# boqian-li/GarmentDreamer

Hardware: AMD Instinct MI355X
Metric: SDS iters/sec (rasterize+UNet+bwd), 100k Gaussians ×8 views @512², 1/2/4/8 GPU (higher is better)
Workload: dtype bf16

## Files before the change

### garmentdreamer_amd/csrc/nn_elementwise.hip

```cpp
#include <hip/hip_runtime.h>
#include <stdint.h>
#include <stdio.h>

#include "../../include/gd_nn.h"
#include "nn_device.h"
#include "nn_host.h"
#include "nn_math.h"

namespace {

using namespace gdnn;


__device__ __forceinline__ float wave_sum(float v)
{
#pragma unroll
    for (int off = 32; off > 0; off >>= 1) v += __shfl_xor(v, off, 64);
    return v;
}

__global__ __launch_bounds__(256) void geglu_kernel(const bf16x8* __restrict__ x, bf16x8* __restrict__ y, int64_t nvec,
                                                    int vin )
{
    for (int64_t i = (int64_t)blockIdx.x * blockDim.x + threadIdx.x; i < nvec; i += (int64_t)gridDim.x * blockDim.x) {
        const int64_t row = i / vin;
        const int c = (int)(i - row * vin);
        const u32x4 h = __builtin_bit_cast(u32x4, x[row * 2 * vin + c]);
        const u32x4 g = __builtin_bit_cast(u32x4, x[row * 2 * vin + vin + c]);
        u32x4 o;
#pragma unroll
        for (int k = 0; k < 4; k++) o.w[k] = gdnn::geglu2(h.w[k], g.w[k]);
        y[i] = __builtin_bit_cast(bf16x8, o);
    }
}

template <int VPL>
__global__ __launch_bounds__(256) void add_layernorm_kernel(const bf16x8* __restrict__ x, const bf16x8* __restrict__ r,
                                                            const bf16x8* __restrict__ w, const bf16x8* __restrict__ b,
                                                            bf16x8* __restrict__ s_out, bf16x8* __restrict__ y,
                                                            int64_t rows, int vpr , float eps)
{
    const int lane = threadIdx.x & 63;
    const int64_t row = (int64_t)blockIdx.x * (blockDim.x >> 6) + (threadIdx.x >> 6);
    if (row >= rows) return;
    const bf16x8* xr = x + row * vpr;
    f2 v[VPL][4];
    f2 sum2 = {0.f, 0.f};
#pragma unroll
    for (int i = 0; i < VPL; i++) {
        const int c = lane + 64 * i;
        if (c < vpr) {
            const u32x4 a = __builtin_bit_cast(u32x4, xr[c]);
            if (r) {
                const u32x4 rr = __builtin_bit_cast(u32x4, r[row * vpr + c]);
                u32x4 so;
#pragma unroll
                for (int k = 0; k < 4; k++) {
                    so.w[k] = pack2(unpack2(a.w[k]) + unpack2(rr.w[k]));
                    v[i][k] = unpack2(so.w[k]);
                }
                if (s_out) s_out[row * vpr + c] = __builtin_bit_cast(bf16x8, so);
            } else {
#pragma unroll
                for (int k = 0; k < 4; k++) v[i][k] = unpack2(a.w[k]);
            }
#pragma unroll
            for (int k = 0; k < 4; k++) sum2 += v[i][k];
        } else {
#pragma unroll
            for (int k = 0; k < 4; k++) v[i][k] = f2{0.f, 0.f};
        }
    }
    const float inv_c = 1.0f / (float)(vpr * 8);
    const float mean = wave_sum(sum2.x + sum2.y) * inv_c;
    f2 sq2 = {0.f, 0.f};
#pragma unroll
    for (int i = 0; i < VPL; i++) {
        if (lane + 64 * i < vpr) {
#pragma unroll
            for (int k = 0; k < 4; k++) {
                const f2 d = v[i][k] - mean;
                sq2 += d * d;
            }
        }
    }
    const float rstd = rsqrtf(wave_sum(sq2.x + sq2.y) * inv_c + eps);
#pragma unroll
    for (int i = 0; i < VPL; i++) {
        const int c = lane + 64 * i;
        if (c < vpr) {
            const u32x4 ww = __builtin_bit_cast(u32x4, w[c]), bb = __builtin_bit_cast(u32x4, b[c]);
            u32x4 o;
#pragma unroll
            for (int k = 0; k < 4; k++) o.w[k] = pack2(((v[i][k] - mean) * rstd) * unpack2(ww.w[k]) + unpack2(bb.w[k]));
            y[row * vpr + c] = __builtin_bit_cast(bf16x8, o);
        }
    }
}

__global__ __launch_bounds__(256) void geglu_backward_kernel(const bf16x8* __restrict__ x, const bf16x8* __restrict__ dy,
                                                             bf16x8* __restrict__ dx, int64_t nvec, int vin)
{
    for (int64_t i = (int64_t)blockIdx.x * blockDim.x + threadIdx.x; i < nvec; i += (int64_t)gridDim.x * blockDim.x) {
        const int64_t row = i / vin;
        const int c = (int)(i - row * vin);
        const u32x4 h = __builtin_bit_cast(u32x4, x[row * 2 * vin + c]);
        const u32x4 g = __builtin_bit_cast(u32x4, x[row * 2 * vin + vin + c]);
        const u32x4 d = __builtin_bit_cast(u32x4, dy[i]);
        u32x4 oh, og;
#pragma unroll
        for (int k = 0; k < 4; k++) {
            const f2 gv = unpack2(g.w[k]), hv = unpack2(h.w[k]), dv = unpack2(d.w[k]);
            const f2 cdf = 0.5f * (1.0f + erf_as2(gv * 0.70710678118654752f));
            const f2 a = (gv * gv) * -0.72134752044448170f;
            const f2 pdf = 0.39894228040143268f * f2{__builtin_amdgcn_exp2f(a.x), __builtin_amdgcn_exp2f(a.y)};
            oh.w[k] = pack2(dv * (gv * cdf));
            og.w[k] = pack2((dv * hv) * (cdf + gv * pdf));
        }
        dx[row * 2 * vin + c] = __builtin_bit_cast(bf16x8, oh);
        dx[row * 2 * vin + vin + c] = __builtin_bit_cast(bf16x8, og);
    }
}

template <int VPL>
__global__ __launch_bounds__(256) void layernorm_backward_kernel(const bf16x8* __restrict__ s, const bf16x8* __restrict__ dy,
                                                                 const bf16x8* __restrict__ w, const bf16x8* __restrict__ ds,
                                                                 bf16x8* __restrict__ dx, int64_t rows, int vpr, float eps)
{
    const int lane = threadIdx.x & 63;
    const int64_t row = (int64_t)blockIdx.x * (blockDim.x >> 6) + (threadIdx.x >> 6);
    if (row >= rows) return;
    f2 v[VPL][4], a[VPL][4];
    f2 sum2 = {0.f, 0.f};
#pragma unroll
    for (int i = 0; i < VPL; i++) {
        const int c = lane + 64 * i;
        if (c < vpr) {
            const u32x4 q = __builtin_bit_cast(u32x4, s[row * vpr + c]);
#pragma unroll
            for (int k = 0; k < 4; k++) { v[i][k] = unpack2(q.w[k]); sum2 += v[i][k]; }
        } else {
#pragma unroll
            for (int k = 0; k < 4; k++) v[i][k] = f2{0.f, 0.f};
        }
    }
    const float inv_c = 1.0f / (float)(vpr * 8);
    const float mean = wave_sum(sum2.x + sum2.y) * inv_c;
    f2 sq2 = {0.f, 0.f};
#pragma unroll
    for (int i = 0; i < VPL; i++)
        if (lane + 64 * i < vpr) {
#pragma unroll
            for (int k = 0; k < 4; k++) { const f2 d = v[i][k] - mean; sq2 += d * d; }
        }
    const float rstd = rsqrtf(wave_sum(sq2.x + sq2.y) * inv_c + eps);
    f2 m1 = {0.f, 0.f}, m2 = {0.f, 0.f};
#pragma unroll
    for (int i = 0; i < VPL; i++) {
        const int c = lane + 64 * i;
        if (c < vpr) {
            const u32x4 g = __builtin_bit_cast(u32x4, dy[row * vpr + c]), ww = __builtin_bit_cast(u32x4, w[c]);
#pragma unroll
            for (int k = 0; k < 4; k++) {
                v[i][k] = (v[i][k] - mean) * rstd;
                a[i][k] = unpack2(g.w[k]) * unpack2(ww.w[k]);
                m1 += a[i][k];
                m2 += a[i][k] * v[i][k];
            }
        } else {
#pragma unroll
            for (int k = 0; k < 4; k++) a[i][k] = f2{0.f, 0.f};
        }
    }
    const float ma = wave_sum(m1.x + m1.y) * inv_c, mb = wave_sum(m2.x + m2.y) * inv_c;
#pragma unroll
    for (int i = 0; i < VPL; i++) {
        const int c = lane + 64 * i;
        if (c < vpr) {
            u32x4 o;
            u32x4 e = {{0u, 0u, 0u, 0u}};
            if (ds) e = __builtin_bit_cast(u32x4, ds[row * vpr + c]);
#pragma unroll
            for (int k = 0; k < 4; k++) o.w[k] = pack2((a[i][k] - ma - v[i][k] * mb) * rstd + unpack2(e.w[k]));
            dx[row * vpr + c] = __builtin_bit_cast(bf16x8, o);
        }
    }
}

template <int R>
__global__ __launch_bounds__(256) void softmax_rows_kernel(const u32x4* x, u32x4* y, int64_t rows, int L8)
{
    const int lane = threadIdx.x & 63;
    const int64_t row = (int64_t)blockIdx.x * 4 + (threadIdx.x >> 6);
    if (row >= rows) return;
    const u32x4* xr = x + row * L8;
    u32x4 v[R];
    float m = -INFINITY;
#pragma unroll
    for (int i = 0; i < R; i++) {
        const int c = lane + 64 * i;
        if (c < L8) {
            v[i] = xr[c];
#pragma unroll
            for (int e = 0; e < 4; e++) { const f2 f = unpack2(v[i].w[e]); m = fmaxf(m, fmaxf(f.x, f.y)); }
        }
    }
#pragma unroll
    for (int off = 32; off > 0; off >>= 1) m = fmaxf(m, __shfl_xor(m, off, 64));
    const float k = 1.4426950408889634f;
    const float mk = m == -INFINITY ? 0.f : m * k;
    float sum = 0.f;
    f2 ex[R][4];
#pragma unroll
    for (int i = 0; i < R; i++) {
        if (lane + 64 * i < L8) {
#pragma unroll
            for (int e = 0; e < 4; e++) {
                const f2 f = unpack2(v[i].w[e]);
                ex[i][e] = f2{__builtin_amdgcn_exp2f(f.x * k - mk), __builtin_amdgcn_exp2f(f.y * k - mk)};
                sum += ex[i][e].x + ex[i][e].y;
            }
        }
    }
    sum = wave_sum(sum);
    const float inv = 1.f / sum;
    u32x4* yr = y + row * L8;
#pragma unroll
    for (int i = 0; i < R; i++) {
        const int c = lane + 64 * i;
        if (c < L8) {
            u32x4 o;
#pragma unroll
            for (int e = 0; e < 4; e++) o.w[e] = pack2(ex[i][e] * inv);
            yr[c] = o;
        }
    }
}

template <int R>
__global__ __launch_bounds__(256) void softmax_rows_backward_kernel(const u32x4* __restrict__ p, const u32x4* dp,
                                                                    u32x4* ds, int64_t rows, int L8)
{
    const int lane = threadIdx.x & 63;
    const int64_t row = (int64_t)blockIdx.x * 4 + (threadIdx.x >> 6);
    if (row >= rows) return;
    const u32x4* pr = p + row * L8;
    const u32x4* gr = dp + row * L8;
    u32x4 vp[R], vg[R];
    f2 acc = f2{0.f, 0.f};
#pragma unroll
    for (int i = 0; i < R; i++) {
        const int c = lane + 64 * i;
        if (c < L8) {
            vp[i] = pr[c];
            vg[i] = gr[c];
        }
    }
#pragma unroll
    for (int i = 0; i < R; i++) {
        if (lane + 64 * i < L8) {
#pragma unroll
            for (int e = 0; e < 4; e++) acc += unpack2(vp[i].w[e]) * unpack2(vg[i].w[e]);
        }
    }
    const float s = wave_sum(acc.x + acc.y);
    u32x4* or_ = ds + row * L8;
#pragma unroll
    for (int i = 0; i < R; i++) {
        const int c = lane + 64 * i;
        if (c < L8) {
            u32x4 o;
#pragma unroll
            for (int e = 0; e < 4; e++) o.w[e] = pack2(unpack2(vp[i].w[e]) * (unpack2(vg[i].w[e]) - s));
            or_[c] = o;
        }
    }
}

template <bool TRANSPOSED>
__global__ __launch_bounds__(256) void conv1x1_c8_kernel(const u32x4* __restrict__ x, const uint16_t* __restrict__ w,
                                                         const uint16_t* __restrict__ bias, u32x4* __restrict__ y, int64_t npix)
{
    float wf[8][8], bf[8];
#pragma unroll
    for (int o = 0; o < 8; o++) {
        bf[o] = (!TRANSPOSED && bias) ? bf2f(bias[o]) : 0.f;
#pragma unroll
        for (int i = 0; i < 8; i++) wf[o][i] = bf2f(TRANSPOSED ? w[i * 8 + o] : w[o * 8 + i]);
    }
    for (int64_t p = (int64_t)blockIdx.x * blockDim.x + threadIdx.x; p < npix; p += (int64_t)gridDim.x * blockDim.x) {
        const u32x4 q = x[p];
        float v[8], o[8];
#pragma unroll
        for (int e = 0; e < 4; e++) { v[2 * e] = __uint_as_float(q.w[e] << 16); v[2 * e + 1] = __uint_as_float(q.w[e] & 0xffff0000u); }
#pragma unroll
        for (int c = 0; c < 8; c++) {
            float a = bf[c];
#pragma unroll
            for (int i = 0; i < 8; i++) a = fmaf(wf[c][i], v[i], a);
            o[c] = a;
        }
        u32x4 out;
#pragma unroll
        for (int e = 0; e < 4; e++) out.w[e] = pack2(f2{o[2 * e], o[2 * e + 1]});
        y[p] = out;
    }
}

}

extern "C" {

const char* gd_nn_elementwise_last_error(void) { return g_err; }

int gd_nn_geglu_forward(void* stream, const void* x, void* y, int64_t rows, int inner)
{
    if (!x || !y) return fail(GD_NN_ERR_INVALID_ARG, "geglu: null pointer");
    if (rows <= 0 || inner <= 0 || inner % 8) return fail(GD_NN_ERR_INVALID_ARG, "geglu: need inner % 8 == 0");
    const int64_t nvec = rows * (inner / 8);
    const int64_t blocks = (nvec + 255) / 256;
    const int grid = (int)(blocks < 16384 ? blocks : 16384);
    hipLaunchKernelGGL(geglu_kernel, dim3(grid), dim3(256), 0, (hipStream_t)stream, (const bf16x8*)x, (bf16x8*)y, nvec,
                       inner / 8);
    return launch_status("geglu: launch failed");
}

int gd_nn_add_layernorm_forward(void* stream, const void* x, const void* residual, const void* weight, const void* bias,
                                float eps, void* sum_out, void* y, int64_t rows, int C)
{
    if (!x || !weight || !bias || !y) return fail(GD_NN_ERR_INVALID_ARG, "add_layernorm: null pointer");
    if (rows <= 0 || C <= 0 || C % 8 || C > 64 * 8 * 4)
        return fail(GD_NN_ERR_INVALID_ARG, "add_layernorm: need C % 8 == 0 and C <= 2048");
    if (sum_out && !residual) return fail(GD_NN_ERR_INVALID_ARG, "add_layernorm: sum_out without residual");
    const int vpr = C / 8;
    const int vpl = (vpr + 63) / 64;
    const int64_t blocks = (rows + 3) / 4;
    if (blocks > 2147483647LL) return fail(GD_NN_ERR_INVALID_ARG, "add_layernorm: too many rows");
#define GD_LN(V_)                                                                                                      \
    hipLaunchKernelGGL(add_layernorm_kernel<V_>, dim3((unsigned)blocks), dim3(256), 0, (hipStream_t)stream,            \
                       (const bf16x8*)x, (const bf16x8*)residual, (const bf16x8*)weight, (const bf16x8*)bias,          \
                       (bf16x8*)sum_out, (bf16x8*)y, rows, vpr, eps)
    if (vpl == 1) GD_LN(1);
    else if (vpl == 2) GD_LN(2);
    else if (vpl == 3) GD_LN(3);
    else GD_LN(4);
#undef GD_LN
    return launch_status("add_layernorm: launch failed");
}

int gd_nn_geglu_backward(void* stream, const void* x, const void* dy, void* dx, int64_t rows, int inner)
{
    if (!x || !dy || !dx) return fail(GD_NN_ERR_INVALID_ARG, "geglu_backward: null pointer");
    if (rows <= 0 || inner <= 0 || inner % 8) return fail(GD_NN_ERR_INVALID_ARG, "geglu_backward: need inner % 8 == 0");
    const int64_t nvec = rows * (inner / 8);
    const int64_t blocks = (nvec + 255) / 256;
    const int grid = (int)(blocks < 16384 ? blocks : 16384);
    hipLaunchKernelGGL(geglu_backward_kernel, dim3(grid), dim3(256), 0, (hipStream_t)stream, (const bf16x8*)x, (const bf16x8*)dy,
                       (bf16x8*)dx, nvec, inner / 8);
    return launch_status("geglu_backward: launch failed");
}

int gd_nn_layernorm_backward(void* stream, const void* s, const void* dy, const void* weight, const void* ds, void* dx,
                             int64_t rows, int C, float eps)
{
    if (!s || !dy || !weight || !dx) return fail(GD_NN_ERR_INVALID_ARG, "layernorm_backward: null pointer");
    if (rows <= 0 || C <= 0 || C % 8 || C > 2048) return fail(GD_NN_ERR_INVALID_ARG, "layernorm_backward: need C % 8 == 0, C <= 2048");
    const int vpr = C / 8, vpl = (vpr + 63) / 64;
    const int64_t blocks = (rows + 3) / 4;
    if (blocks > 2147483647LL) return fail(GD_NN_ERR_INVALID_ARG, "layernorm_backward: too many rows");
#define GD_LNB(V_)                                                                                                     \
    hipLaunchKernelGGL(layernorm_backward_kernel<V_>, dim3((unsigned)blocks), dim3(256), 0, (hipStream_t)stream,       \
                       (const bf16x8*)s, (const bf16x8*)dy, (const bf16x8*)weight, (const bf16x8*)ds, (bf16x8*)dx, rows, vpr, eps)
    if (vpl == 1) GD_LNB(1);
    else if (vpl == 2) GD_LNB(2);
    else if (vpl == 3) GD_LNB(3);
    else GD_LNB(4);
#undef GD_LNB
    return launch_status("layernorm_backward: launch failed");
}

int gd_nn_conv1x1_c8(void* stream, const void* x, const void* weight, const void* bias, void* y, int64_t npix, int transposed)
{
    if (!x || !weight || !y) return fail(GD_NN_ERR_INVALID_ARG, "conv1x1_c8: null pointer");
    if (npix <= 0) return fail(GD_NN_ERR_INVALID_ARG, "conv1x1_c8: need npix > 0");
    const int64_t blocks = (npix + 255) / 256;
    const int grid = (int)(blocks < 16384 ? blocks : 16384);
    if (transposed)
        hipLaunchKernelGGL(conv1x1_c8_kernel<true>, dim3(grid), dim3(256), 0, (hipStream_t)stream, (const u32x4*)x,
                           (const uint16_t*)weight, (const uint16_t*)nullptr, (u32x4*)y, npix);
    else
        hipLaunchKernelGGL(conv1x1_c8_kernel<false>, dim3(grid), dim3(256), 0, (hipStream_t)stream, (const u32x4*)x,
                           (const uint16_t*)weight, (const uint16_t*)bias, (u32x4*)y, npix);
    return launch_status("conv1x1_c8: launch failed");
}

int gd_nn_softmax_rows_forward(void* stream, const void* x, void* y, int64_t rows, int L)
{
    if (!x || !y) return fail(GD_NN_ERR_INVALID_ARG, "softmax_rows: null pointer");
    if (rows <= 0 || L <= 0 || L % 8 || L > 8192) return fail(GD_NN_ERR_INVALID_ARG, "softmax_rows: need rows > 0, L % 8 == 0, L <= 8192");
    const int64_t blocks = (rows + 3) / 4;
    if (blocks > 2147483647LL) return fail(GD_NN_ERR_INVALID_ARG, "softmax_rows: too many rows");
    const int L8 = L / 8, R = (L8 + 63) / 64;
#define GD_SM(R_) hipLaunchKernelGGL(softmax_rows_kernel<R_>, dim3((unsigned)blocks), dim3(256), 0, (hipStream_t)stream, (const u32x4*)x, (u32x4*)y, rows, L8)
    if (R <= 2) GD_SM(2);
    else if (R <= 4) GD_SM(4);
    else if (R <= 8) GD_SM(8);
    else GD_SM(16);
#undef GD_SM
    return launch_status("softmax_rows: launch failed");
}

int gd_nn_softmax_rows_backward(void* stream, const void* p, const void* dp, void* ds, int64_t rows, int L)
{
    if (!p || !dp || !ds) return fail(GD_NN_ERR_INVALID_ARG, "softmax_rows_backward: null pointer");
    if (rows <= 0 || L <= 0 || L % 8 || L > 8192) return fail(GD_NN_ERR_INVALID_ARG, "softmax_rows_backward: need rows > 0, L % 8 == 0, L <= 8192");
    const int64_t blocks = (rows + 3) / 4;
    if (blocks > 2147483647LL) return fail(GD_NN_ERR_INVALID_ARG, "softmax_rows_backward: too many rows");
    const int L8 = L / 8, R = (L8 + 63) / 64;
#define GD_SMB(R_) hipLaunchKernelGGL(softmax_rows_backward_kernel<R_>, dim3((unsigned)blocks), dim3(256), 0, (hipStream_t)stream, (const u32x4*)p, (const u32x4*)dp, (u32x4*)ds, rows, L8)
    if (R <= 2) GD_SMB(2);
    else if (R <= 4) GD_SMB(4);
    else if (R <= 8) GD_SMB(8);
    else GD_SMB(16);
#undef GD_SMB
    return launch_status("softmax_rows_backward: launch failed");
}

}
```

### garmentdreamer_amd/guidance/sd21.py

```python
from __future__ import annotations

import math
from typing import Optional

import torch
import torch.nn as nn
import torch.nn.functional as F

from ..nn_ops import (add_layer_norm, attention_d64, attention_d64_supported, attention_d64_vt, conv1x1, conv3x3, conv3x3_s2, conv3x3_s2_supported, conv3x3_small_cin,
                      conv3x3_supported, geglu, gn_conv3x3, gn_conv3x3_supported, gn_conv_prefers_fused, group_norm_silu,
                      resnet_block_frozen, resnet_block_frozen_supported, upsample2x_conv3x3,
                      upsample2x_conv3x3_supported, linear_320, route_rows, route_scale,
                      linear_320_geglu, linear_320_supported, gemm_geglu, gemm_supported)


import os as _os

_FUSED_QKV = _os.environ.get("GD_FUSED_QKV", "1") != "0"
_VT_GEMM = _os.environ.get("GD_VT_GEMM", "1") != "0"
_LORA_FUSED = _os.environ.get("GD_LORA_FUSED", "1") != "0"
_VAE_ATTN_NODE = _os.environ.get("GD_VAE_ATTN_NODE", "1") != "0"
_CTX_VT = _os.environ.get("GD_CTX_VT", "1") != "0"
_LORA_LINEAR = _os.environ.get("GD_LORA_LINEAR", "1") != "0"
_CONV_BIAS_GRAD = _os.environ.get("GD_CONV_BIAS_GRAD", "1") != "0"
_PINNED_TABLES = _os.environ.get("GD_PAGEABLE_COPIES", "0") != "1"
_TEMB_TRAIN_CAT = _os.environ.get("GD_TEMB_TRAIN_CAT", "1") != "0"
from .. import nn_ops
_FP8_ACTIVE = [None]


def _gn(norm: nn.GroupNorm, x, silu: bool):
    return group_norm_silu(x, norm.weight, norm.bias, norm.num_groups, norm.eps, silu)


def _conv3(conv: nn.Conv2d, x, image_bias=None, residual=None):
    bias = conv.bias if image_bias is None else image_bias
    frozen = not conv.weight.requires_grad and (conv.bias is None or not conv.bias.requires_grad)
    if frozen and conv3x3_supported(x, conv.weight) and conv.stride == (1, 1) and conv.padding == (1, 1):
        if bias is not None and bias.requires_grad and not _CONV_BIAS_GRAD:
            y = conv3x3(x, conv.weight, None, None) + (bias[:, :, None, None] if bias.dim() == 2 else bias[None, :, None, None])
            return y if residual is None else y + residual
        return conv3x3(x, conv.weight, bias, residual)
    nn_ops._note_fallback("sd21._conv3", x, "needs frozen bf16 channels_last weights, stride 1, pad 1, Cin % 64 == 0")
    y = F.conv2d(x, conv.weight, None if image_bias is not None else conv.bias, conv.stride, conv.padding)
    if image_bias is not None:
        y = y + image_bias[:, :, None, None]
    return y if residual is None else y + residual


import os as _os0
_LIN320 = _os0.environ.get("GD_LINEAR320", "1") != "0"
_OWN_GEMM = _os0.environ.get("GD_OWN_GEMM", "1") != "0"
_OWN_GEMM_MIN_ROWS = 1024


def _lib_linear(x, w, b=None):
    if route_scale() > 1 and x.is_cuda:
        padded, take = route_rows(x.reshape(-1, x.shape[-1]))
        return take(F.linear(padded, w, b)).reshape(*x.shape[:-1], w.shape[0])
    return F.linear(x, w, b)


def _lib_addmm(c, a, w_t):
    if route_scale() > 1 and a.is_cuda:
        pa, take = route_rows(a)
        pc, _ = route_rows(c)
        return take(torch.addmm(pc, pa, w_t))
    return torch.addmm(c, a, w_t)


def _lin(mod: nn.Linear, x, bias=None):
    w = mod.weight
    b = mod.bias if bias is None else bias
    if _LIN320 and x.is_cuda and not torch.is_grad_enabled() and not w.requires_grad and w.shape[1] == 320 and \
            linear_320_supported(x, w, b):
        return linear_320(x, w, b)
    return _lib_linear(x, w, b)


def _gn_conv3(norm: nn.GroupNorm, conv: nn.Conv2d, x, image_bias=None, residual=None):
    frozen = not conv.weight.requires_grad and (conv.bias is None or not conv.bias.requires_grad)
    frozen = frozen and (image_bias is None or not image_bias.requires_grad)
    st = _FP8_ACTIVE[0]
    if st is not None and frozen and not torch.is_grad_enabled() and st.wants(conv, x):
        bias = conv.bias if image_bias is None else image_bias
        if st.mode == "run" and id(conv) in st.amax:
            return st.gn_conv(norm, conv, x, bias, residual)
        act = _gn(norm, x, True)
        if st.mode == "calibrate":
            st.observe(conv, act)
        return _conv3(conv, act, image_bias=image_bias, residual=residual)
    if x.is_cuda and frozen and gn_conv_prefers_fused(x, conv.out_channels) and \
            gn_conv3x3_supported(x, norm.weight, conv.weight):
        return gn_conv3x3(x, norm.weight, norm.bias, norm.num_groups, norm.eps, True, conv.weight,
                          conv.bias if image_bias is None else image_bias, residual)
    return _conv3(conv, _gn(norm, x, True), image_bias=image_bias, residual=residual)




class TembProjections:

    __slots__ = ("temb", "image_bias")

    def __init__(self, temb, image_bias):
        self.temb, self.image_bias = temb, image_bias


class ContextProjections:

    __slots__ = ("context", "kv", "vt")

    def __init__(self, context, kv, vt=None):
        self.context, self.kv, self.vt = context, kv, (vt or {})

    @property
    def shape(self):
        return self.context.shape


class ResnetBlock2D(nn.Module):
    def __init__(self, in_ch: int, out_ch: int, temb_ch: Optional[int], eps: float = 1e-5, groups: int = 32):
        super().__init__()
        self.norm1 = nn.GroupNorm(groups, in_ch, eps=eps)
        self.conv1 = nn.Conv2d(in_ch, out_ch, 3, padding=1)
        self.time_emb_proj = nn.Linear(temb_ch, out_ch) if temb_ch is not None else None
        self.norm2 = nn.GroupNorm(groups, out_ch, eps=eps)
        self.conv2 = nn.Conv2d(out_ch, out_ch, 3, padding=1)
        self.conv_shortcut = nn.Conv2d(in_ch, out_ch, 1) if in_ch != out_ch else None

    def forward(self, x, temb=None, next_norm=None):
        if resnet_block_frozen_supported(x, self):
            return resnet_block_frozen(x, self, next_norm)
        image_bias = None
        if isinstance(temb, TembProjections):
            image_bias = temb.image_bias.get(id(self))
            temb = temb.temb
        if image_bias is None and self.time_emb_proj is not None:
            image_bias = self.time_emb_proj(F.silu(temb)) + self.conv1.bias
        h = _gn_conv3(self.norm1, self.conv1, x, image_bias=image_bias)
        if self.conv_shortcut is not None:
            x = conv1x1(x, self.conv_shortcut.weight, self.conv_shortcut.bias)
        return _gn_conv3(self.norm2, self.conv2, h, residual=x)


class LoRALinearLayer(nn.Module):

    def __init__(self, in_features: int, out_features: int, rank: int = 4):
        super().__init__()
        self.down = nn.Linear(in_features, rank, bias=False)
        self.up = nn.Linear(rank, out_features, bias=False)
        nn.init.normal_(self.down.weight, std=1 / rank)
        nn.init.zeros_(self.up.weight)

    def forward(self, x):
        return self.up(self.down(x.to(self.down.weight.dtype))).to(x.dtype)


class Attention(nn.Module):

    def __init__(self, query_dim: int, heads: int, dim_head: int, cross_dim: Optional[int] = None,
                 qkv_bias: bool = False):
        super().__init__()
        inner = heads * dim_head
        self.heads = heads
        self.to_q = nn.Linear(query_dim, inner, bias=qkv_bias)
        self.to_k = nn.Linear(cross_dim or query_dim, inner, bias=qkv_bias)
        self.to_v = nn.Linear(cross_dim or query_dim, inner, bias=qkv_bias)
        self.to_out = nn.ModuleList([nn.Linear(inner, query_dim)])
        self.lora = None
        self.lora_scale = 1.0

    def add_lora(self, rank: int = 4):
        q_in, kv_in, inner = self.to_q.in_features, self.to_k.in_features, self.to_q.out_features
        self.lora = nn.ModuleDict({
            "to_q_lora": LoRALinearLayer(q_in, inner, rank), "to_k_lora": LoRALinearLayer(kv_in, inner, rank),
            "to_v_lora": LoRALinearLayer(kv_in, inner, rank),
            "to_out_lora": LoRALinearLayer(inner, self.to_out[0].out_features, rank)})
        return self.lora

    def forward(self, x, context=None):
        B, N, _ = x.shape
        kv = context_vt = None
        if isinstance(context, ContextProjections):
            kv = context.kv.get(id(self)) if self.lora is None else None
            context_vt = context.vt
            context = context.context
        ctx = x if context is None else context
        if kv is not None:
            q, (k, v) = _lin(self.to_q, x), kv
            vt = context_vt.get(id(self)) if context_vt is not None else None
            if vt is not None and N >= 256 and _CTX_VT and q.shape[-1] == 64 * self.heads and not torch.is_grad_enabled():
                q4, k4 = q.view(B, N, self.heads, 64), k.view(B, k.shape[1], self.heads, 64)
                if nn_ops._attention_d64_layout_ok(q4, k4, k4):
                    return _lin(self.to_out[0], nn_ops.attention_d64_vt_strided(q4, k4, vt, k.shape[1]))
        elif _FUSED_QKV and context is None and self.lora is None and x.is_cuda and self.to_q.bias is None and \
                not self.to_q.weight.requires_grad and not torch.is_grad_enabled():
            src = (self.to_q.weight.data_ptr(), self.to_q.weight._version, self.to_k.weight._version,
                   self.to_v.weight._version, x.dtype)
            if getattr(self, "_wqkv_src", None) != src:
                self._wqk = torch.cat([self.to_q.weight, self.to_k.weight], dim=0).detach().contiguous()
                self._wqkv_src = src
            q, k = (linear_320(x, self._wqk) if _LIN320 and linear_320_supported(x, self._wqk)
                    else _lib_linear(x, self._wqk)).chunk(2, dim=-1)
            q = q.view(B, N, self.heads, -1)
            k = k.view(B, N, self.heads, -1)
            if _VT_GEMM and N % 64 == 0 and N >= 256 and q.shape[-1] == 64 and x.dtype == torch.bfloat16:
                vt = torch.matmul(self.to_v.weight.detach(), x.transpose(1, 2))
                return _lin(self.to_out[0], attention_d64_vt(q, k, vt))
            v = _lin(self.to_v, x)
            q, k = q.reshape(B, N, -1), k.reshape(B, N, -1)
        elif self.lora is not None:
            q = self._lora_lin(self.to_q, x, "to_q_lora")
            k = self._lora_lin(self.to_k, ctx, "to_k_lora")
            v = self._lora_lin(self.to_v, ctx, "to_v_lora")
        else:
            q, k, v = _lin(self.to_q, x), _lin(self.to_k, ctx), _lin(self.to_v, ctx)
        q = q.view(B, N, self.heads, -1)
        k = k.view(B, ctx.shape[1], self.heads, -1)
        v = v.view(B, ctx.shape[1], self.heads, -1)
        if N >= 256 and q.shape[-1] == 64 and nn_ops.attention_d64_train_supported(q, k, v):
            o = nn_ops.attention_d64_train(q, k, v)
        elif N >= 256 and q.shape[-1] == 64 and attention_d64_supported(q, k, v):
            o = attention_d64(q, k, v)
        else:
            o = F.scaled_dot_product_attention(q.transpose(1, 2), k.transpose(1, 2), v.transpose(1, 2))
            o = o.transpose(1, 2).reshape(B, N, -1)
        if self.lora is not None:
            return self._lora_lin(self.to_out[0], o, "to_out_lora")
        return _lin(self.to_out[0], o)

    def _lora_lin(self, mod: nn.Linear, x, name):
        layer = self.lora[name]
        dw, uw = layer.down.weight, layer.up.weight
        w, b = mod.weight, mod.bias
        if _LORA_FUSED and _LORA_LINEAR and x.is_cuda and x.dtype == torch.bfloat16 and w.dtype == torch.bfloat16 and \
                not w.requires_grad and (b is None or not b.requires_grad) and dw.dtype == torch.float32 and \
                uw.dtype == torch.float32 and dw.shape[0] == 4 and uw.shape[1] == 4 and x.shape[-1] % 8 == 0 and \
                w.shape[0] % 8 == 0 and dw.is_contiguous() and uw.is_contiguous():
            return nn_ops.lora_linear(x, w, dw, uw, self.lora_scale, lambda t: _lin(mod, t))
        return self._lora_add(_lin(mod, x), x, name)

    def _lora_add(self, base, x, name):
        layer = self.lora[name]
        dw, uw = layer.down.weight, layer.up.weight
        if _LORA_FUSED and nn_ops.lora_branch_supported(x, base, dw, uw):
            return nn_ops.lora_branch(x, base, dw, uw, self.lora_scale)
        return base + self.lora_scale * layer(x)


class GEGLU(nn.Module):
    def __init__(self, dim_in: int, dim_out: int):
        super().__init__()
        self.proj = nn.Linear(dim_in, dim_out * 2)

    def forward(self, x):
        w = self.proj.weight
        if _LIN320 and x.is_cuda and not torch.is_grad_enabled() and not w.requires_grad and tuple(w.shape) == (2560, 320) and \
                linear_320_supported(x, w, self.proj.bias):
            return linear_320_geglu(x, w, self.proj.bias)
        if _OWN_GEMM and x.is_cuda and not torch.is_grad_enabled() and not w.requires_grad and w.shape[1] != 320 and \
                (x.numel() // x.shape[-1]) * route_scale() >= _OWN_GEMM_MIN_ROWS and gemm_supported(x, w, self.proj.bias, geglu=True):
            return gemm_geglu(x, w, self.proj.bias)
        return geglu(_lin(self.proj, x))


class FeedForward(nn.Module):
    def __init__(self, dim: int, mult: int = 4):
        super().__init__()
        self.net = nn.ModuleList([GEGLU(dim, dim * mult), nn.Identity(), nn.Linear(dim * mult, dim)])

    def forward(self, x):
        return _lin(self.net[2], self.net[0](x))


class BasicTransformerBlock(nn.Module):
    def __init__(self, dim: int, heads: int, dim_head: int, cross_dim: int):
        super().__init__()
        self.norm1 = nn.LayerNorm(dim)
        self.attn1 = Attention(dim, heads, dim_head)
        self.norm2 = nn.LayerNorm(dim)
        self.attn2 = Attention(dim, heads, dim_head, cross_dim=cross_dim)
        self.norm3 = nn.LayerNorm(dim)
        self.ff = FeedForward(dim)

    def forward(self, x, context, defer_ff_bias: bool = False):
        _, n = add_layer_norm(x, None, self.norm1)
        x, n = add_layer_norm(x, self.attn1(n), self.norm2)
        x, n = add_layer_norm(x, self.attn2(n, context), self.norm3)
        if defer_ff_bias:
            g = self.ff.net[0](n)
            return _lib_addmm(x.reshape(-1, x.shape[-1]), g.reshape(-1, g.shape[-1]), self.ff.net[2].weight.t()).view_as(x)
        return x + self.ff(n)


class Transformer2DModel(nn.Module):
    def __init__(self, channels: int, heads: int, dim_head: int, cross_dim: int, groups: int = 32):
        super().__init__()
        self.norm = nn.GroupNorm(groups, channels, eps=1e-6)
        self.proj_in = nn.Linear(channels, channels)
        self.transformer_blocks = nn.ModuleList([BasicTransformerBlock(channels, heads, dim_head, cross_dim)])
        self.proj_out = nn.Linear(channels, channels)

    def _folded_out_bias(self, dtype):
        w, b2 = self.proj_out.weight, self.transformer_blocks[0].ff.net[2].bias
        key = (w.data_ptr(), w._version, b2._version, self.proj_out.bias._version, dtype)
        if getattr(self, "_fold_key", None) != key:
            with torch.no_grad():
                self._fold_bias = (self.proj_out.bias.float() + w.float() @ b2.float()).to(dtype)
            self._fold_key = key
        return self._fold_bias

    def forward(self, x, context):
        B, C, H, W = x.shape
        h = _gn(self.norm, x, False)
        h = h.permute(0, 2, 3, 1).reshape(B, H * W, C)
        h = _lin(self.proj_in, h)
        if len(self.transformer_blocks) == 1 and h.is_cuda and not torch.is_grad_enabled() and \
                not self.proj_out.weight.requires_grad:
            h = self.transformer_blocks[0](h, context, defer_ff_bias=True)
            h = _lin(self.proj_out, h, self._folded_out_bias(h.dtype))
        else:
            for blk in self.transformer_blocks:
                h = blk(h, context)
            h = self.proj_out(h)
        h = h.reshape(B, H, W, C).permute(0, 3, 1, 2)
        return h + x


class Downsample2D(nn.Module):
    def __init__(self, ch: int, padding: int = 1):
        super().__init__()
        self.padding = padding
        self.conv = nn.Conv2d(ch, ch, 3, stride=2, padding=padding)

    def forward(self, x):
        if conv3x3_s2_supported(x, self.conv.weight):
            return conv3x3_s2(x, self.conv.weight, self.conv.bias, self.padding)
        nn_ops._note_fallback("sd21.Downsample2D", x, "needs frozen bf16 weights with Cin % 64 == 0 and Cout % 64 == 0")
        if self.padding == 0:
            x = F.pad(x, (0, 1, 0, 1))
        return self.conv(x)


class Upsample2D(nn.Module):
    def __init__(self, ch: int):
        super().__init__()
        self.conv = nn.Conv2d(ch, ch, 3, padding=1)

    def forward(self, x):
        if upsample2x_conv3x3_supported(x, self.conv.weight) and not self.conv.bias.requires_grad:
            return upsample2x_conv3x3(x, self.conv.weight, self.conv.bias)
        return _conv3(self.conv, F.interpolate(x, scale_factor=2.0, mode="nearest"))


class _DownBlock(nn.Module):
    def __init__(self, in_ch, out_ch, temb_ch, n_layers, heads, cross_dim, attn: bool, down: bool):
        super().__init__()
        self.resnets = nn.ModuleList(
            [ResnetBlock2D(in_ch if i == 0 else out_ch, out_ch, temb_ch) for i in range(n_layers)])
        self.attentions = nn.ModuleList(
            [Transformer2DModel(out_ch, heads, out_ch // heads, cross_dim) for _ in range(n_layers)]) if attn else None
        self.downsamplers = nn.ModuleList([Downsample2D(out_ch)]) if down else None

    def forward(self, x, temb, context, skips):
        for i, res in enumerate(self.resnets):
            x = res(x, temb)
            if self.attentions is not None:
                x = self.attentions[i](x, context)
            skips.append(x)
        if self.downsamplers is not None:
            x = self.downsamplers[0](x)
            skips.append(x)
        return x


class _UpBlock(nn.Module):
    def __init__(self, in_ch, prev_ch, out_ch, temb_ch, n_layers, heads, cross_dim, attn: bool, up: bool):
        super().__init__()
        res = []
        for i in range(n_layers):
            skip_ch = in_ch if i == n_layers - 1 else out_ch
            res_in = prev_ch if i == 0 else out_ch
            res.append(ResnetBlock2D(res_in + skip_ch, out_ch, temb_ch))
        self.resnets = nn.ModuleList(res)
        self.attentions = nn.ModuleList(
            [Transformer2DModel(out_ch, heads, out_ch // heads, cross_dim) for _ in range(n_layers)]) if attn else None
        self.upsamplers = nn.ModuleList([Upsample2D(out_ch)]) if up else None

    def forward(self, x, temb, context, skips):
        for i, res in enumerate(self.resnets):
            x = torch.cat([x, skips.pop()], dim=1)
            x = res(x, temb)
            if self.attentions is not None:
                x = self.attentions[i](x, context)
        if self.upsamplers is not None:
            x = self.upsamplers[0](x)
        return x


class _MidBlockCrossAttn(nn.Module):
    def __init__(self, ch, temb_ch, heads, cross_dim):
        super().__init__()
        self.resnets = nn.ModuleList([ResnetBlock2D(ch, ch, temb_ch), ResnetBlock2D(ch, ch, temb_ch)])
        self.attentions = nn.ModuleList([Transformer2DModel(ch, heads, ch // heads, cross_dim)])

    def forward(self, x, temb, context):
        x = self.resnets[0](x, temb)
        x = self.attentions[0](x, context)
        return self.resnets[1](x, temb)


class TimestepEmbedding(nn.Module):
    def __init__(self, in_ch, out_ch):
        super().__init__()
        self.linear_1 = nn.Linear(in_ch, out_ch)
        self.linear_2 = nn.Linear(out_ch, out_ch)

    def forward(self, x):
        return _lin(self.linear_2, F.silu(_lin(self.linear_1, x)))


def sinusoidal_timestep_embedding(t: torch.Tensor, dim: int) -> torch.Tensor:
    half = dim // 2
    exponent = -math.log(10000.0) * torch.arange(half, dtype=torch.float32, device=t.device) / half
    emb = t.float()[:, None] * torch.exp(exponent)[None, :]
    return torch.cat([torch.cos(emb), torch.sin(emb)], dim=-1)


class UNet2DConditionModel(nn.Module):

    def __init__(self, in_channels=4, out_channels=4, block_out_channels=(320, 640, 1280, 1280), layers_per_block=2,
                 cross_attention_dim=1024, attention_head_dim=(5, 10, 20, 20)):
        super().__init__()
        ch = block_out_channels
        temb_ch = ch[0] * 4
        self.block_out_channels = tuple(ch)
        self.conv_in = nn.Conv2d(in_channels, ch[0], 3, padding=1)
        self.time_embedding = TimestepEmbedding(ch[0], temb_ch)
        self.down_blocks = nn.ModuleList()
        out = ch[0]
        for i, c in enumerate(ch):
            inp, out = out, c
            last = i == len(ch) - 1
            self.down_blocks.append(_DownBlock(inp, out, temb_ch, layers_per_block, attention_head_dim[i],
                                               cross_attention_dim, attn=not last, down=not last))
        self.mid_block = _MidBlockCrossAttn(ch[-1], temb_ch, attention_head_dim[-1], cross_attention_dim)
        self.up_blocks = nn.ModuleList()
        rev = list(reversed(ch))
        rev_heads = list(reversed(attention_head_dim))
        out = rev[0]
        for i, c in enumerate(rev):
            prev, out = out, c
            inp = rev[min(i + 1, len(ch) - 1)]
            last = i == len(ch) - 1
            self.up_blocks.append(_UpBlock(inp, prev, out, temb_ch, layers_per_block + 1, rev_heads[i],
                                           cross_attention_dim, attn=i != 0, up=not last))
        self.conv_norm_out = nn.GroupNorm(32, ch[0], eps=1e-5)
        self.conv_out = nn.Conv2d(ch[0], out_channels, 3, padding=1)

    def extra_embedding(self, batch: int, **kwargs):
        return None

    def _project_context(self, ctx):
        if not ctx.is_cuda or torch.is_grad_enabled():
            return ctx
        atts = [m.attn2 for m in self.modules() if isinstance(m, BasicTransformerBlock)]
        if not atts or any(a.to_k.weight.requires_grad or a.to_k.bias is not None or a.lora is not None for a in atts):
            return ctx
        first = atts[0].to_k.weight
        key = (first.data_ptr(), ctx.dtype, len(atts)) + tuple(t._version for a in atts for t in (a.to_k.weight, a.to_v.weight))
        cache = getattr(self, "_ctx_cat", None)
        if cache is None or cache[0] != key:
            with torch.no_grad():
                w = torch.cat([t for a in atts for t in (a.to_k.weight, a.to_v.weight)], dim=0).to(ctx.dtype).contiguous()
                wv = torch.cat([a.to_v.weight for a in atts], dim=0).to(ctx.dtype).contiguous()
            cache = self._ctx_cat = (key, w, wv)
        with torch.no_grad():
            allp = _lib_linear(ctx, cache[1])
            vt_all = None
            if _CTX_VT and ctx.dtype == torch.bfloat16 and all(a.to_v.out_features == 64 * a.heads for a in atts):
                T = ctx.shape[1]
                Tp = (T + 63) // 64 * 64
                ctx_p = F.pad(ctx, (0, 0, 0, Tp - T)) if Tp != T else ctx
                vt_all = torch.matmul(cache[2], ctx_p.transpose(1, 2))
        kv, vt, off, voff = {}, {}, 0, 0
        for a in atts:
            c = a.to_k.out_features
            kv[id(a)] = (allp[..., off:off + c], allp[..., off + c:off + 2 * c])
            if vt_all is not None:
                vt[id(a)] = vt_all[:, voff:voff + c]
            off += 2 * c
            voff += c
        return ContextProjections(ctx, kv, vt)

    def _project_temb(self, temb):
        train = torch.is_grad_enabled() and temb.requires_grad
        if not temb.is_cuda or (train and not _TEMB_TRAIN_CAT):
            return temb
        blocks = [m for m in self.modules() if isinstance(m, ResnetBlock2D) and m.time_emb_proj is not None]
        if not blocks or any(b.time_emb_proj.weight.requires_grad or b.conv1.bias.requires_grad for b in blocks):
            return temb
        first = blocks[0].time_emb_proj.weight
        key = (first.data_ptr(), temb.dtype, len(blocks)) + tuple(
            t._version for b in blocks for t in (b.time_emb_proj.weight, b.time_emb_proj.bias, b.conv1.bias))
        cache = getattr(self, "_temb_cat", None)
        if cache is None or cache[0] != key:
            with torch.no_grad():
                w = torch.cat([b.time_emb_proj.weight for b in blocks], dim=0).to(temb.dtype).contiguous()
                bias = torch.cat([b.time_emb_proj.bias + b.conv1.bias for b in blocks], dim=0).to(temb.dtype)
            cache = self._temb_cat = (key, w, bias)
        if train:
            parts = torch.split(_lib_linear(F.silu(temb), cache[1], cache[2]), [b.time_emb_proj.out_features for b in blocks], dim=1)
            return TembProjections(temb, {id(b): p for b, p in zip(blocks, parts)})
        with torch.no_grad():
            allp = _lib_linear(F.silu(temb), cache[1], cache[2])
        out, off = {}, 0
        for b in blocks:
            c = b.time_emb_proj.out_features
            out[id(b)] = allp[:, off:off + c]
            off += c
        return TembProjections(temb, out)

    fp8 = None

    def enable_fp8(self, state=None):
        from ..nn_ops import Fp8State
        self.fp8 = state if state is not None else Fp8State()
        return self.fp8

    def forward(self, sample, timestep, encoder_hidden_states, **kwargs):
        if self.fp8 is not None and not torch.is_grad_enabled() and sample.is_cuda:
            _FP8_ACTIVE[0] = self.fp8
            try:
                return self._forward(sample, timestep, encoder_hidden_states, **kwargs)
            finally:
                _FP8_ACTIVE[0] = None
        return self._forward(sample, timestep, encoder_hidden_states, **kwargs)

    def _forward(self, sample, timestep, encoder_hidden_states, **kwargs):
        dtype = self.conv_in.weight.dtype
        if timestep.dim() == 0:
            timestep = timestep[None].expand(sample.shape[0])
        temb = self.time_embedding(sinusoidal_timestep_embedding(timestep, self.block_out_channels[0]).to(dtype))
        extra = self.extra_embedding(sample.shape[0], **kwargs)
        if extra is not None:
            temb = temb + extra.to(dtype)
        temb = self._project_temb(temb)
        x = conv3x3_small_cin(sample.to(dtype).contiguous(memory_format=torch.channels_last), self.conv_in.weight,
                              self.conv_in.bias)
        ctx = self._project_context(encoder_hidden_states.to(dtype))
        skips = [x]
        for blk in self.down_blocks:
            x = blk(x, temb, ctx, skips)
        x = self.mid_block(x, temb, ctx)
        for blk in self.up_blocks:
            x = blk(x, temb, ctx, skips)
        return _conv3(self.conv_out, _gn(self.conv_norm_out, x, True))


class LoraUNet2DConditionModel(UNet2DConditionModel):

    def __init__(self, rank: int = 4, **kw):
        super().__init__(**kw)
        temb_ch = self.block_out_channels[0] * 4
        self.camera_emb = nn.Sequential(nn.Linear(16, temb_ch), nn.SiLU(), nn.Linear(temb_ch, temb_ch))
        self.lambertian_emb = nn.Parameter(torch.randn(1, temb_ch))
        self.textureless_emb = nn.Parameter(torch.randn(1, temb_ch))
        self.normal_emb = nn.Parameter(torch.randn(1, temb_ch))
        self.lora_layers = nn.ModuleList()
        for m in self.modules():
            if isinstance(m, Attention):
                self.lora_layers.append(m.add_lora(rank))

    def adapters_to_fp32(self):
        self.lora_layers.float()
        return self

    def trainables_to_fp32(self):
        self.adapters_to_fp32()
        self.camera_emb.float()
        for p in (self.lambertian_emb, self.textureless_emb, self.normal_emb):
            p.data = p.data.float()
        return self

    def freeze_base(self):
        for p in self.parameters():
            p.requires_grad_(False)
        train = list(self.lora_layers.parameters()) + list(self.camera_emb.parameters()) + \
            [self.lambertian_emb, self.textureless_emb, self.normal_emb]
        for p in train:
            p.requires_grad_(True)
        return train

    def forward(self, sample, timestep, encoder_hidden_states, **kwargs):
        if torch.is_grad_enabled() and sample.is_cuda:
            with nn_ops.lora_grad_group():
                return super().forward(sample, timestep, encoder_hidden_states, **kwargs)
        return super().forward(sample, timestep, encoder_hidden_states, **kwargs)

    def extra_embedding(self, batch: int, c=None, shading: str = "albedo"):
        dev, dt = self.camera_emb[0].weight.device, self.camera_emb[0].weight.dtype
        if c is None:
            c = torch.zeros(batch, 16, device=dev)
        emb = self.camera_emb(c.to(device=dev, dtype=dt))
        if shading == "textureless":
            emb = emb + self.textureless_emb
        elif shading == "lambertian":
            emb = emb + self.lambertian_emb
        elif shading == "normal":
            emb = emb + self.normal_emb
        else:
            assert shading == "albedo"
        return emb




class _VAEAttention(nn.Module):

    def __init__(self, ch: int):
        super().__init__()
        self.group_norm = nn.GroupNorm(32, ch, eps=1e-6)
        self.to_q = nn.Linear(ch, ch)
        self.to_k = nn.Linear(ch, ch)
        self.to_v = nn.Linear(ch, ch)
        self.to_out = nn.ModuleList([nn.Linear(ch, ch)])

    def _qkv_scaled(self, dtype, scale):
        ws = (self.to_q.weight, self.to_k.weight, self.to_v.weight, self.to_q.bias, self.to_k.bias, self.to_v.bias)
        key = (ws[0].data_ptr(), dtype) + tuple(t._version for t in ws)
        if getattr(self, "_qkv_key", None) != key:
            with torch.no_grad():
                w = torch.cat([ws[0].float() * scale, ws[1].float(), ws[2].float()], dim=0).to(dtype).contiguous()
                b = torch.cat([ws[3].float() * scale, ws[4].float(), ws[5].float()], dim=0).to(dtype)
            self._qkv_cache, self._qkv_key = (w, b), key
        return self._qkv_cache

    def forward(self, x):
        B, C, H, W = x.shape
        h = _gn(self.group_norm, x, False).permute(0, 2, 3, 1).reshape(B, H * W, C)
        if x.is_cuda:
            o = None
            if _FUSED_QKV and not (self.to_q.weight.requires_grad or self.to_k.weight.requires_grad or self.to_v.weight.requires_grad):
                qkv = _lib_linear(h, *self._qkv_scaled(h.dtype, C ** -0.5))
                if _VAE_ATTN_NODE and nn_ops.single_head_attention_supported(qkv):
                    o = nn_ops.single_head_attention(qkv)
                else:
                    q, k, v = qkv.chunk(3, dim=-1)
            else:
                q, k, v = _lin(self.to_q, h) * (C ** -0.5), _lin(self.to_k, h), _lin(self.to_v, h)
            if o is None:
                p = torch.softmax(torch.bmm(q, k.transpose(1, 2)), dim=-1)
                o = torch.bmm(p, v)
        else:
            q, k, v = self.to_q(h), self.to_k(h), self.to_v(h)
            o = F.scaled_dot_product_attention(q[:, None], k[:, None], v[:, None])[:, 0]
        o = _lin(self.to_out[0], o).reshape(B, H, W, C).permute(0, 3, 1, 2)
        return x + o


class _VAEDownBlock(nn.Module):
    def __init__(self, in_ch, out_ch, n_layers, down: bool):
        super().__init__()
        self.resnets = nn.ModuleList(
            [ResnetBlock2D(in_ch if i == 0 else out_ch, out_ch, None, eps=1e-6) for i in range(n_layers)])
        self.downsamplers = nn.ModuleList([Downsample2D(out_ch, padding=0)]) if down else None

    def forward(self, x, next_norm=None):
        for i, r in enumerate(self.resnets):
            last = i + 1 == len(self.resnets)
            x = r(x, next_norm=(next_norm if self.downsamplers is None else None) if last else self.resnets[i + 1].norm1)
        if self.downsamplers is not None:
            x = self.downsamplers[0](x)
        return x


class _VAEMidBlock(nn.Module):
    def __init__(self, ch):
        super().__init__()
        self.resnets = nn.ModuleList([ResnetBlock2D(ch, ch, None, eps=1e-6), ResnetBlock2D(ch, ch, None, eps=1e-6)])
        self.attentions = nn.ModuleList([_VAEAttention(ch)])

    def forward(self, x):
        return self.resnets[1](self.attentions[0](self.resnets[0](x)))


class Encoder(nn.Module):
    def __init__(self, in_channels=3, block_out_channels=(128, 256, 512, 512), layers_per_block=2, latent_channels=4):
        super().__init__()
        ch = block_out_channels
        self.conv_in = nn.Conv2d(in_channels, ch[0], 3, padding=1)
        self.down_blocks = nn.ModuleList()
        out = ch[0]
        for i, c in enumerate(ch):
            inp, out = out, c
            self.down_blocks.append(_VAEDownBlock(inp, out, layers_per_block, down=i != len(ch) - 1))
        self.mid_block = _VAEMidBlock(ch[-1])
        self.conv_norm_out = nn.GroupNorm(32, ch[-1], eps=1e-6)
        self.conv_out = nn.Conv2d(ch[-1], 2 * latent_channels, 3, padding=1)

    def forward(self, x):
        x = conv3x3_small_cin(x.contiguous(memory_format=torch.channels_last), self.conv_in.weight, self.conv_in.bias,
                              next_norm=self.down_blocks[0].resnets[0].norm1)
        for i, b in enumerate(self.down_blocks):
            x = b(x, next_norm=self.mid_block.resnets[0].norm1 if i + 1 == len(self.down_blocks) else None)
        x = self.mid_block(x)
        return _conv3(self.conv_out, _gn(self.conv_norm_out, x, True))


# ... 247 lines not shown
```

### garmentdreamer_amd/guidance/stable_diffusion_guidance.py

```python
from __future__ import annotations

from dataclasses import dataclass, field
from typing import Any, Optional

import torch
import torch.nn as nn
import torch.nn.functional as F

from .. import _runtime_env, nn_ops
from . import sd21


def C(value: Any, epoch: int, global_step: int) -> float:
    if isinstance(value, (int, float)):
        return value
    value = list(value)
    if len(value) == 3:
        value = [0] + value
    assert len(value) == 4
    start_step, start_value, end_value, end_step = value
    current = global_step if isinstance(end_step, int) else epoch
    return start_value + (end_value - start_value) * max(min(1.0, (current - start_step) / (end_step - start_step)), 0.0)


class StableDiffusionGuidance(nn.Module):
    @dataclass
    class Config:
        pretrained_model_name_or_path: str = "stabilityai/stable-diffusion-2-1-base"
        enable_memory_efficient_attention: bool = False
        enable_sequential_cpu_offload: bool = False
        enable_attention_slicing: bool = False
        enable_channels_last_format: bool = True
        guidance_scale: float = 100.0
        grad_clip: Optional[Any] = None
        half_precision_weights: bool = True
        min_step_percent: float = 0.02
        max_step_percent: float = 0.98
        max_step_percent_annealed: float = 0.5
        anneal_start_step: Optional[int] = None
        use_sjc: bool = False
        var_red: bool = True
        weighting_strategy: str = "sds"
        token_merging: bool = False
        token_merging_params: Optional[dict] = field(default_factory=dict)
        view_dependent_prompting: bool = True
        max_items_eval: int = 4
        unet_weights: Optional[str] = None
        vae_weights: Optional[str] = None
        init_seed: int = 0
        use_hip_graphs: bool = False
        fp8_unet: bool = False
        fp8_calibration_steps: int = 3

    def __init__(self, cfg: Optional[dict] = None, device="cuda", unet: Optional[nn.Module] = None,
                 vae: Optional[nn.Module] = None):
        super().__init__()
        cfg = cfg or {}
        self.cfg = cfg if isinstance(cfg, self.Config) else self.Config(**cfg)
        self.device = torch.device(device)
        self.configure(unet, vae)

    def configure(self, unet=None, vae=None) -> None:
        self.weights_dtype = torch.bfloat16 if self.cfg.half_precision_weights else torch.float32
        if unet is None:
            with torch.device(self.device):
                unet = sd21.UNet2DConditionModel()
            if self.cfg.unet_weights:
                sd21.load_diffusers_weights(unet, self.cfg.unet_weights)
            else:
                sd21.init_random_(unet, self.cfg.init_seed)
        self._vae_self_built = vae is None
        self._own_decoder = ()
        if vae is None:
            with torch.device(self.device):
                vae = sd21.AutoencoderKLEncoder()
            if self.cfg.vae_weights:
                sd21.load_diffusers_weights(vae, self.cfg.vae_weights)
            else:
                sd21.init_random_(vae, self.cfg.init_seed + 1)
        fmt = torch.channels_last if self.cfg.enable_channels_last_format else torch.contiguous_format
        self.unet = unet.to(device=self.device, dtype=self.weights_dtype).to(memory_format=fmt).eval()
        self.vae = vae.to(device=self.device, dtype=self.weights_dtype).to(memory_format=fmt).eval()
        for p in self.vae.parameters():
            p.requires_grad_(False)
        for p in self.unet.parameters():
            p.requires_grad_(False)
        self.scheduler = sd21.DDIMScheduler()
        self.num_train_timesteps = self.scheduler.config.num_train_timesteps
        self.set_min_max_steps()
        self.alphas = self.scheduler.alphas_cumprod.to(self.device)
        if self.cfg.use_sjc:
            self.us = torch.sqrt((1 - self.alphas) / self.alphas)
        self.grad_clip_val: Optional[float] = None
        self._unet_graphs = {}
        self._vae_graphs = {}
        self._fp8_calibrated = False
        self._fp8_calib_done = 0
        if self.cfg.fp8_unet and self.weights_dtype == torch.bfloat16 and self.device.type == "cuda":
            self.unet.enable_fp8()
        if self.cfg.use_hip_graphs and not _runtime_env.graph_replay_safe():
            import warnings
            warnings.warn(f"{_runtime_env.FLAG}=0 was not in place before the HIP runtime started; hipGraph replay of "
                          "the UNet / VAE is off for this process (eager launches). Import garmentdreamer_amd before "
                          "the first torch.cuda call, or export the flag.")
            self.cfg.use_hip_graphs = False

    def set_min_max_steps(self, min_step_percent=0.02, max_step_percent=0.98):
        self.min_step = int(self.num_train_timesteps * min_step_percent)
        self.max_step = int(self.num_train_timesteps * max_step_percent)

    def forward_unet(self, latents, t, encoder_hidden_states):
        input_dtype = latents.dtype
        t_dtype = torch.float32 if self.weights_dtype == torch.bfloat16 else self.weights_dtype
        x, tt, ctx = latents.to(self.weights_dtype), t.to(t_dtype), encoder_hidden_states.to(self.weights_dtype)
        fp8 = getattr(self.unet, "fp8", None)
        if fp8 is not None and not self._fp8_calibrated and not torch.is_grad_enabled():
            out = self.unet(x, tt, encoder_hidden_states=ctx).to(input_dtype)
            self._fp8_calib_done += 1
            if self._fp8_calib_done >= max(1, int(self.cfg.fp8_calibration_steps)):
                fp8.mode = "run"
                self._fp8_calibrated = True
            return out
        if self.cfg.use_hip_graphs and x.is_cuda and not torch.is_grad_enabled():
            try:
                return self._graphed_unet(x, tt, ctx).to(input_dtype)
            except RuntimeError as e:
                self._graphs_failed(e)
        return self.unet(x, tt, encoder_hidden_states=ctx).to(input_dtype)

    def may_capture(self, batch_size: int) -> bool:
        if not self.cfg.use_hip_graphs:
            return False
        have_u = any(k[0][0] in (2 * batch_size, 4 * batch_size) for k in self._unet_graphs)
        have_v = any(k[0] == batch_size for k in self._vae_graphs)
        return not (have_u and have_v)

    def _graphs_failed(self, err):
        import warnings
        warnings.warn(f"hipGraph capture failed ({err}); continuing with eager kernel launches")
        self.cfg.use_hip_graphs = False
        self._unet_graphs.clear()
        self._vae_graphs.clear()
        torch.cuda.synchronize()
        from .. import nn_ops
        nn_ops.reset_workspaces()

    def _graphed_unet(self, x, t, ctx):
        key = (tuple(x.shape), tuple(ctx.shape))
        entry = self._unet_graphs.get(key)
        if entry is None:
            sx, st, sc = x.clone(), t.clone(), ctx.clone()
            side = torch.cuda.Stream(device=x.device)
            side.wait_stream(torch.cuda.current_stream(x.device))
            with torch.cuda.stream(side), torch.no_grad():
                for _ in range(2):
                    self.unet(sx, st, encoder_hidden_states=sc)
            torch.cuda.current_stream(x.device).wait_stream(side)
            g = torch.cuda.CUDAGraph()
            with _runtime_env.capture_guard(), torch.cuda.graph(g), torch.no_grad():
                out = self.unet(sx, st, encoder_hidden_states=sc)
            entry = self._unet_graphs[key] = (g, sx, st, sc, out)
        g, sx, st, sc, out = entry
        sx.copy_(x)
        st.copy_(t)
        sc.copy_(ctx)
        g.replay()
        return out.clone()

    def _graphed_vae_moments(self, imgs):
        key = tuple(imgs.shape)
        fn = self._vae_graphs.get(key)
        if fn is None:
            vae = self.vae

            class _Moments(nn.Module):
                def forward(self, x):
                    return vae.quant_conv(vae.encoder(x))

            sample = torch.rand(imgs.shape, device=imgs.device, dtype=imgs.dtype, requires_grad=True)
            with _runtime_env.capture_guard():
                fn = self._vae_graphs[key] = torch.cuda.make_graphed_callables(_Moments(), (sample,))
        return fn(imgs)

    def encode_images(self, imgs, vae_noise: Optional[torch.Tensor] = None):
        return self._encode_prepared((imgs * 2.0 - 1.0).to(self.weights_dtype), vae_noise, imgs.dtype)

    def _encode_prepared(self, x, vae_noise, out_dtype):
        with nn_ops.route_batch(1, x.shape[0]):
            if self.cfg.use_hip_graphs and x.is_cuda and torch.is_grad_enabled() and x.requires_grad:
                xc = x.contiguous(memory_format=torch.channels_last)
                try:
                    posterior = sd21.DiagonalGaussianDistribution(self._graphed_vae_moments(xc))
                except RuntimeError as e:
                    self._graphs_failed(e)
                    posterior = self.vae.encode(x).latent_dist
            else:
                posterior = self.vae.encode(x).latent_dist
        noise = None if vae_noise is None else vae_noise.to(self.weights_dtype)
        latents = posterior.sample(noise) * self.vae.config.scaling_factor
        return latents.to(out_dtype)

    def compute_grad_sds(self, latents, t, prompt_utils, elevation, azimuth, camera_distances,
                         noise: Optional[torch.Tensor] = None):
        use_perp_neg = bool(getattr(prompt_utils, "use_perp_neg", False))
        batch_size = elevation.shape[0]
        neg_guidance_weights = None
        if use_perp_neg:
            text_embeddings, neg_guidance_weights = prompt_utils.get_text_embeddings_perp_neg(
                elevation, azimuth, camera_distances, self.cfg.view_dependent_prompting)
            with torch.no_grad():
                if noise is None:
                    noise = torch.randn_like(latents)
                latents_noisy = self.scheduler.add_noise(latents, noise, t)
                with nn_ops.route_batch(4, 4 * batch_size):
                    noise_pred = self.forward_unet(torch.cat([latents_noisy] * 4, dim=0), torch.cat([t] * 4),
                                                   encoder_hidden_states=text_embeddings)
            noise_pred_text = noise_pred[:batch_size]
            noise_pred_uncond = noise_pred[batch_size:batch_size * 2]
            noise_pred_neg = noise_pred[batch_size * 2:]
            e_pos = noise_pred_text - noise_pred_uncond
            accum_grad = 0
            n_negative_prompts = neg_guidance_weights.shape[-1]
            for i in range(n_negative_prompts):
                e_i_neg = noise_pred_neg[i::n_negative_prompts] - noise_pred_uncond
                accum_grad = accum_grad + neg_guidance_weights[:, i].view(-1, 1, 1, 1).to(e_pos) * \
                    perpendicular_component(e_i_neg, e_pos)
            noise_pred = noise_pred_uncond + self.cfg.guidance_scale * (e_pos + accum_grad)
        else:
            text_embeddings = prompt_utils.get_text_embeddings(elevation, azimuth, camera_distances,
                                                               self.cfg.view_dependent_prompting)
            with torch.no_grad():
                if noise is None:
                    noise = torch.randn_like(latents)
                latents_noisy = self.scheduler.add_noise(latents, noise, t)
                latent_model_input = torch.cat([latents_noisy] * 2, dim=0)
                with nn_ops.route_batch(2, 2 * batch_size):
                    noise_pred = self.forward_unet(latent_model_input, torch.cat([t] * 2),
                                                   encoder_hidden_states=text_embeddings)
            noise_pred_text, noise_pred_uncond = noise_pred.chunk(2)
            noise_pred = noise_pred_text + self.cfg.guidance_scale * (noise_pred_text - noise_pred_uncond)

        if self.cfg.weighting_strategy == "sds":
            w = (1 - self.alphas[t]).view(-1, 1, 1, 1)
        elif self.cfg.weighting_strategy == "uniform":
            w = 1
        elif self.cfg.weighting_strategy == "fantasia3d":
            w = (self.alphas[t] ** 0.5 * (1 - self.alphas[t])).view(-1, 1, 1, 1)
        else:
            raise ValueError(f"Unknown weighting strategy: {self.cfg.weighting_strategy}")
        grad = w * (noise_pred - noise)
        guidance_eval_utils = {"use_perp_neg": use_perp_neg, "neg_guidance_weights": neg_guidance_weights,
                               "text_embeddings": text_embeddings, "t_orig": t, "latents_noisy": latents_noisy,
                               "noise_pred": noise_pred}
        return grad, guidance_eval_utils

    def compute_grad_sjc(self, latents, t, prompt_utils, elevation, azimuth, camera_distances,
                         noise: Optional[torch.Tensor] = None):
        use_perp_neg = bool(getattr(prompt_utils, "use_perp_neg", False))
        batch_size = elevation.shape[0]
        sigma = self.us[t].view(-1, 1, 1, 1)
        neg_guidance_weights = None
        if use_perp_neg:
            text_embeddings, neg_guidance_weights = prompt_utils.get_text_embeddings_perp_neg(
                elevation, azimuth, camera_distances, self.cfg.view_dependent_prompting)
            reps = 4
        else:
            text_embeddings = prompt_utils.get_text_embeddings(elevation, azimuth, camera_distances,
                                                               self.cfg.view_dependent_prompting)
            reps = 2
        with torch.no_grad():
            if noise is None:
                noise = torch.randn_like(latents)
            y = latents
            zs = y + sigma * noise
            scaled_zs = zs / torch.sqrt(1 + sigma ** 2)
            with nn_ops.route_batch(reps, reps * batch_size):
                noise_pred = self.forward_unet(torch.cat([scaled_zs] * reps, dim=0), torch.cat([t] * reps),
                                               encoder_hidden_states=text_embeddings)
        if use_perp_neg:
            noise_pred_text = noise_pred[:batch_size]
            noise_pred_uncond = noise_pred[batch_size:batch_size * 2]
            noise_pred_neg = noise_pred[batch_size * 2:]
            e_pos = noise_pred_text - noise_pred_uncond
            accum_grad = 0
            n_negative_prompts = neg_guidance_weights.shape[-1]
            for i in range(n_negative_prompts):
                e_i_neg = noise_pred_neg[i::n_negative_prompts] - noise_pred_uncond
                accum_grad = accum_grad + neg_guidance_weights[:, i].view(-1, 1, 1, 1).to(e_pos) * \
                    perpendicular_component(e_i_neg, e_pos)
            noise_pred = noise_pred_uncond + self.cfg.guidance_scale * (e_pos + accum_grad)
        else:
            noise_pred_text, noise_pred_uncond = noise_pred.chunk(2)
            noise_pred = noise_pred_text + self.cfg.guidance_scale * (noise_pred_text - noise_pred_uncond)
        Ds = zs - sigma * noise_pred
        grad = -(Ds - y) / sigma if self.cfg.var_red else -(Ds - zs) / sigma
        guidance_eval_utils = {"use_perp_neg": use_perp_neg, "neg_guidance_weights": neg_guidance_weights,
                               "text_embeddings": text_embeddings, "t_orig": t, "latents_noisy": scaled_zs,
                               "noise_pred": noise_pred}
        return grad, guidance_eval_utils

    def __call__(self, rgb, prompt_utils, elevation, azimuth, camera_distances, rgb_as_latents=False,
                 guidance_eval=False, noise: Optional[torch.Tensor] = None, timesteps: Optional[torch.Tensor] = None,
                 vae_noise: Optional[torch.Tensor] = None, **kwargs):
        batch_size = rgb.shape[0]
        rgb_BCHW = rgb.permute(0, 3, 1, 2)
        if rgb_as_latents:
            latents = F.interpolate(rgb_BCHW, (64, 64), mode="bilinear", align_corners=False)
        elif self.weights_dtype == torch.bfloat16 and nn_ops.vae_prologue_supported(rgb_BCHW):
            latents = self._encode_prepared(nn_ops.vae_prologue(rgb_BCHW, 512, 512), vae_noise, rgb.dtype)
        else:
            rgb_BCHW_512 = F.interpolate(rgb_BCHW, (512, 512), mode="bilinear", align_corners=False)
            latents = self.encode_images(rgb_BCHW_512, vae_noise)

        if timesteps is None:
            t = torch.randint(self.min_step, self.max_step + 1, [batch_size], dtype=torch.long, device=self.device)
        else:
            t = timesteps.to(device=self.device, dtype=torch.long)

        compute_grad = self.compute_grad_sjc if self.cfg.use_sjc else self.compute_grad_sds
        grad, guidance_eval_utils = compute_grad(latents, t, prompt_utils, elevation, azimuth, camera_distances, noise)
        grad = torch.nan_to_num(grad)
        if self.grad_clip_val is not None:
            grad = grad.clamp(-self.grad_clip_val, self.grad_clip_val)
        target = (latents - grad).detach()
        loss_sds = 0.5 * F.mse_loss(latents, target, reduction="sum") / batch_size
        guidance_out = {"loss_sds": loss_sds, "grad_norm": grad.norm(), "min_step": self.min_step,
                        "max_step": self.max_step}
        if guidance_eval:
            guidance_eval_out = self.guidance_eval(**guidance_eval_utils, generator=kwargs.get("eval_generator"))
            texts = []
            for n, e, a, c in zip(guidance_eval_out["noise_levels"], elevation, azimuth, camera_distances):
                texts.append(f"n{n:.02f}\ne{e.item():.01f}\na{a.item():.01f}\nc{c.item():.02f}")
            guidance_eval_out.update({"texts": texts})
            guidance_out.update({"eval": guidance_eval_out})
        return guidance_out

    def _decoder_vae(self):
        if hasattr(self.vae, "decode"):
            return self.vae
        if not self._vae_self_built:
            raise RuntimeError("guidance_eval needs a VAE with a decoder (pass vae=<object with .decode>); the supplied VAE "
                               "has the encoder half only")
        if not self._own_decoder:
            self._own_decoder = (_build_decoder(self.device, self.weights_dtype, self.cfg.vae_weights, self.cfg.init_seed + 2,
                                                self.cfg.enable_channels_last_format),)
        return self._own_decoder[0]

    def decode_latents(self, latents, latent_height: int = 64, latent_width: int = 64):
        vae = self._decoder_vae()
        input_dtype = latents.dtype
        latents = F.interpolate(latents, (latent_height, latent_width), mode="bilinear", align_corners=False)
        if isinstance(vae, sd21._VAEDecoderMixin):
            return vae.decode_to_image(latents).to(input_dtype)
        latents = 1 / vae.config.scaling_factor * latents
        image = vae.decode(latents.to(self.weights_dtype)).sample
        image = (image * 0.5 + 0.5).clamp(0, 1)
        return image.to(input_dtype)

    @torch.no_grad()
    def get_noise_pred(self, latents_noisy, t, text_embeddings, use_perp_neg=False, neg_guidance_weights=None):
        batch_size = latents_noisy.shape[0]
        reps = 4 if use_perp_neg else 2
        from .. import nn_ops
        with nn_ops.route_batch(reps, reps * batch_size):
            noise_pred = self.forward_unet(torch.cat([latents_noisy] * reps, dim=0),
                                           torch.cat([t.reshape(1)] * reps).to(self.device),
                                           encoder_hidden_states=text_embeddings)
        if use_perp_neg:
            noise_pred_text = noise_pred[:batch_size]
            noise_pred_uncond = noise_pred[batch_size:batch_size * 2]
            noise_pred_neg = noise_pred[batch_size * 2:]
            e_pos = noise_pred_text - noise_pred_uncond
            accum_grad = 0
            n_negative_prompts = neg_guidance_weights.shape[-1]
            for i in range(n_negative_prompts):
                e_i_neg = noise_pred_neg[i::n_negative_prompts] - noise_pred_uncond
                accum_grad = accum_grad + neg_guidance_weights[:, i].view(-1, 1, 1, 1).to(e_pos) * \
                    perpendicular_component(e_i_neg, e_pos)
            return noise_pred_uncond + self.cfg.guidance_scale * (e_pos + accum_grad)
        noise_pred_text, noise_pred_uncond = noise_pred.chunk(2)
        return noise_pred_text + self.cfg.guidance_scale * (noise_pred_text - noise_pred_uncond)

    @torch.no_grad()
    def guidance_eval(self, t_orig, text_embeddings, latents_noisy, noise_pred, use_perp_neg=False,
                      neg_guidance_weights=None, generator=None):
        self.scheduler.set_timesteps(50)
        timesteps_dev = self.scheduler.timesteps.to(self.device)
        bs = min(self.cfg.max_items_eval, latents_noisy.shape[0]) if self.cfg.max_items_eval > 0 else latents_noisy.shape[0]
        large_enough_idxs = timesteps_dev.expand([bs, -1]) > t_orig[:bs].unsqueeze(-1)
        idxs = torch.min(large_enough_idxs, dim=1)[1]
        t = timesteps_dev[idxs]
        fracs = list((t / self.scheduler.config.num_train_timesteps).cpu().numpy())
        imgs_noisy = self.decode_latents(latents_noisy[:bs]).permute(0, 2, 3, 1)
        latents_1step, pred_1orig = [], []
        for b in range(bs):
            step_output = self.scheduler.step(noise_pred[b:b + 1], t[b], latents_noisy[b:b + 1], eta=1, generator=generator)
            latents_1step.append(step_output["prev_sample"])
            pred_1orig.append(step_output["pred_original_sample"])
        latents_1step = torch.cat(latents_1step)
        pred_1orig = torch.cat(pred_1orig)
        imgs_1step = self.decode_latents(latents_1step).permute(0, 2, 3, 1)
        imgs_1orig = self.decode_latents(pred_1orig).permute(0, 2, 3, 1)
        latents_final = []
        for b, i in enumerate(idxs):
            latents = latents_1step[b:b + 1]
            sel = [b, b + len(idxs), b + 2 * len(idxs), b + 3 * len(idxs)] if use_perp_neg else [b, b + len(idxs)]
            text_emb = text_embeddings[sel, ...]
            neg_guid = neg_guidance_weights[b:b + 1] if use_perp_neg else None
            for tt in self.scheduler.timesteps[int(i) + 1:]:
                npred = self.get_noise_pred(latents, tt, text_emb, use_perp_neg, neg_guid)
                latents = self.scheduler.step(npred, tt, latents, eta=1, generator=generator)["prev_sample"]
            latents_final.append(latents)
        latents_final = torch.cat(latents_final)
        imgs_final = self.decode_latents(latents_final).permute(0, 2, 3, 1)
        return {"bs": bs, "noise_levels": fracs, "imgs_noisy": imgs_noisy, "imgs_1step": imgs_1step,
                "imgs_1orig": imgs_1orig, "imgs_final": imgs_final}

    def update_step(self, epoch: int, global_step: int, on_load_weights: bool = False):
        if self.cfg.grad_clip is not None:
            self.grad_clip_val = C(self.cfg.grad_clip, epoch, global_step)
        self.set_min_max_steps(min_step_percent=C(self.cfg.min_step_percent, epoch, global_step),
                               max_step_percent=C(self.cfg.max_step_percent, epoch, global_step))


def _build_decoder(device, dtype, weights: Optional[str], seed: int, channels_last: bool = True):
    with torch.device(device):
        dec = sd21.AutoencoderKLDecoder()
    if weights:
        sd21.load_diffusers_weights(dec, weights)
    else:
        sd21.init_random_(dec, seed)
    fmt = torch.channels_last if channels_last else torch.contiguous_format
    dec = dec.to(device=device, dtype=dtype).to(memory_format=fmt).eval()
    for p in dec.parameters():
        p.requires_grad_(False)
    return dec


def perpendicular_component(x, y):
    eps = torch.ones_like(x[:, 0, 0, 0]) * 1e-6
    return x - (torch.mul(x, y).sum(dim=[1, 2, 3]) / torch.maximum(torch.mul(y, y).sum(dim=[1, 2, 3]), eps)).view(-1, 1, 1, 1) * y


class PromptEmbeddings:

    use_perp_neg = False
    perp_neg_f_sb = (1, 0.5, -0.606)
    perp_neg_f_fsb = (1, 0.5, +0.967)
    perp_neg_f_fs = (4, 0.5, -2.426)
    perp_neg_f_sf = (4, 0.5, -2.426)

    def __init__(self, text_embeddings_vd, uncond_text_embeddings_vd, front_threshold=45.0, back_threshold=45.0,
                 overhead_threshold=60.0):
        self.text_embeddings_vd = text_embeddings_vd
        self.uncond_text_embeddings_vd = uncond_text_embeddings_vd
        self.text_embeddings = text_embeddings_vd[:1]
        self.uncond_text_embeddings = uncond_text_embeddings_vd[:1]
        self.front_threshold, self.back_threshold, self.overhead_threshold = front_threshold, back_threshold, \
            overhead_threshold

    @classmethod
    def random(cls, device, dtype=torch.float32, seed: int = 0):
        g = torch.Generator().manual_seed(seed)
        e = torch.randn(2, 4, 77, 1024, generator=g).to(device=device, dtype=dtype)
        return cls(e[0], e[1])

    def get_text_embeddings(self, elevation, azimuth, camera_distances, view_dependent_prompting=True):
        batch_size = elevation.shape[0]
        if view_dependent_prompting:
            azi = (azimuth + 180) % 360 - 180
            idx = torch.zeros_like(elevation, dtype=torch.long)
            idx[(azi > -self.front_threshold) & (azi < self.front_threshold)] = 1
            idx[(azi > 180 - self.back_threshold) | (azi < -180 + self.back_threshold)] = 2
            idx[elevation > self.overhead_threshold] = 3
            dev = self.text_embeddings_vd.device
            if idx.device != dev:
                if dev.type == "cuda" and not idx.is_cuda and sd21._PINNED_TABLES:
                    idx = idx.pin_memory()
                idx = idx.to(dev, non_blocking=True)
            text, uncond = self.text_embeddings_vd[idx], self.uncond_text_embeddings_vd[idx]
        else:
            text = self.text_embeddings.expand(batch_size, -1, -1)
            uncond = self.uncond_text_embeddings.expand(batch_size, -1, -1)
        return torch.cat([text, uncond], dim=0)

    def _direction_idx(self, elevation, azimuth):
        azi = (azimuth + 180) % 360 - 180
        idx = torch.zeros_like(elevation, dtype=torch.long)
        idx[(azi > -self.front_threshold) & (azi < self.front_threshold)] = 1
        idx[(azi > 180 - self.back_threshold) | (azi < -180 + self.back_threshold)] = 2
        idx[elevation > self.overhead_threshold] = 3
        return idx, azi

    def get_text_embeddings_perp_neg(self, elevation, azimuth, camera_distances, view_dependent_prompting=True):
        assert view_dependent_prompting, "Perp-Neg only works with view-dependent prompting"
        B = elevation.shape[0]
        idx, azi = self._direction_idx(elevation, azimuth)
        side, front, back, overhead = (self.text_embeddings_vd[i] for i in range(4))
        decay = lambda f, r: f[0] * torch.exp(-f[1] * r) + f[2]
        pos, neg, wts, unc = [], [], [], []
        for i in range(B):
            d, a = int(idx[i]), azi[i]
            u = self.uncond_text_embeddings_vd[d]
            unc.append(u)
            if d == 3:
                pos.append(overhead)
                neg += [u, u]
                wts += [torch.zeros((), device=elevation.device), torch.zeros((), device=elevation.device)]
            elif torch.abs(a) < 90:
                r = 1 - torch.abs(a) / 90
                pos.append(r * front + (1 - r) * side)
                neg += [front, side]
                wts += [-decay(self.perp_neg_f_fs, r), -decay(self.perp_neg_f_sf, 1 - r)]
            else:
                r = 2.0 - torch.abs(a) / 90
                pos.append(r * side + (1 - r) * back)
                neg += [side, front]
                wts += [-decay(self.perp_neg_f_sb, r), -decay(self.perp_neg_f_fsb, r)]
        emb = torch.cat([torch.stack(pos), torch.stack(unc), torch.stack(neg)], dim=0)
        w = torch.stack([torch.as_tensor(x, dtype=torch.float32) for x in wts]).to(elevation.device).reshape(B, 2)
# ... 2 lines not shown
```

### garmentdreamer_amd/nn_ops.py

```python
from __future__ import annotations

import ctypes as C
import os
import weakref

import torch
import torch.nn.functional as F

_HERE = os.path.dirname(os.path.abspath(__file__))
_LIB_PATH = os.path.join(_HERE, "libgd_nn.so")
_LIB_OVERRIDDEN = False
_lib = None


def use_library(path: str) -> None:
    global _LIB_PATH, _LIB_OVERRIDDEN
    if _lib is not None:
        raise RuntimeError("libgd_nn.so is already loaded")
    _LIB_PATH, _LIB_OVERRIDDEN = os.path.abspath(path), True


_vp, _i, _f = C.c_void_p, C.c_int, C.c_float
SIGNATURES = {
    "gd_nn_groupnorm_silu_forward": (_i, [_vp, _vp, _vp, _vp, _vp, _i, _i, _i, _i, _f, _i, _vp, _vp]),
    "gd_nn_groupnorm_silu_fused_supported": (_i, [_i, _i, _i, _i]),
    "gd_nn_groupnorm_silu_fused_forward": (_i, [_vp, _vp, _vp, _vp, _vp, _i, _i, _i, _i, _f, _i]),
    "gd_nn_groupnorm_silu_fused_forward_stats": (_i, [_vp, _vp, _vp, _vp, _vp, _i, _i, _i, _i, _f, _i, _vp]),
    "gd_nn_groupnorm_silu_fused_backward": (_i, [_vp, _vp, _vp, _vp, _vp, _vp, _vp, _i, _i, _i, _i, _i]),
    "gd_nn_groupnorm_silu_fused_backward_supported": (_i, [_i, _i, _i, _i]),
    "gd_nn_groupnorm_silu_backward": (_i, [_vp, _vp, _vp, _vp, _vp, _vp, _vp, _i, _i, _i, _i, _i, _vp, _vp, _vp]),
    "gd_nn_groupnorm_ws_bytes": (C.c_size_t, [_i, _i]),
    "gd_nn_conv3x3_forward": (_i, [_vp, _vp, _vp, _vp, _i, _vp, _vp, _i, _i, _i, _i, _i]),
    "gd_nn_conv3x3_ws_bytes": (C.c_size_t, [_i, _i, _i, _i, _i]),
    "gd_nn_conv3x3_forward_ws": (_i, [_vp, _vp, _vp, _vp, _i, _vp, _vp, _i, _i, _i, _i, _i, _vp, C.c_size_t]),
    "gd_nn_conv_force_split": (_i, [_i]),
    "gd_nn_conv_set_route_scale": (_i, [_i]),
    "gd_nn_conv3x3_flip_weights": (_i, [_vp, _vp, _vp, _i, _i]),
    "gd_nn_conv3x3_first_dgrad_supported": (_i, [_i, _i, _i, _i, _i]),
    "gd_nn_conv3x3_first_dgrad_weights": (_i, [_vp, _vp, _vp, _i, _i]),
    "gd_nn_conv3x3_first_dgrad": (_i, [_vp, _vp, _vp, _vp, _i, _i, _i, _i, _i]),
    "gd_nn_groupnorm_stats": (_i, [_vp, _vp, _i, _i, _i, _i, _f, _vp, _vp]),
    "gd_nn_groupnorm_silu_forward_fp8": (_i, [_vp, _vp, _vp, _vp, _vp, _i, _i, _i, _i, _f, _i, _vp, _vp, _f]),
    "gd_nn_conv3x3_gn_forward": (_i, [_vp, _vp, _vp, _vp, _vp, _i, _i, _vp, _vp, _i, _vp, _vp, _i, _i, _i, _i, _i]),
    "gd_nn_linear_320_supported": (_i, [C.c_int64, _i, _i]),
    "gd_nn_linear_320_forward": (_i, [_vp, _vp, _vp, _vp, _vp, C.c_int64]),
    "gd_nn_linear_k320_forward": (_i, [_vp, _vp, _vp, _vp, _vp, C.c_int64, _i]),
    "gd_nn_linear_k320_geglu_forward": (_i, [_vp, _vp, _vp, _vp, _vp, C.c_int64, _i]),
    "gd_nn_linear_320_last_error": (C.c_char_p, []),
    "gd_nn_conv3x3_stat_rows": (C.c_size_t, [_i, _i, _i, _i, _i]),
    "gd_nn_conv3x3_first_stat_rows": (C.c_size_t, [_i, _i, _i, _i, _i]),
    "gd_nn_conv3x3_first_forward_stats": (_i, [_vp, _vp, _vp, _vp, _vp, _i, _i, _i, _i, _i, _vp]),
    "gd_nn_conv3x3_gn_forward_stats": (_i, [_vp, _vp, _vp, _vp, _vp, _i, _i, _vp, _vp, _i, _vp, _vp, _i, _i, _i, _i, _i,
                                            _vp]),
    "gd_nn_conv3x3_forward_stats": (_i, [_vp, _vp, _vp, _vp, _i, _vp, _vp, _i, _i, _i, _i, _i, _vp]),
    "gd_nn_conv3x3_wino_supported": (_i, [_i, _i, _i, _i, _i]),
    "gd_nn_conv3x3_wino_weights": (_i, [_vp, _vp, _vp, _i, _i]),
    "gd_nn_conv3x3_wino_weights_bytes": (C.c_size_t, [_i, _i]),
    "gd_nn_conv3x3_wino_forward": (_i, [_vp, _vp, _vp, _vp, _i, _vp, _vp, _i, _i, _i, _i, _i, _vp]),
    "gd_nn_conv3x3_wino_gn_forward": (_i, [_vp, _vp, _vp, _vp, _vp, _i, _i, _vp, _vp, _i, _vp, _vp, _i, _i, _i, _i, _i, _vp]),
    "gd_nn_conv3x3_wide_supported": (_i, [_i, _i, _i, _i, _i]),
    "gd_nn_conv3x3_wide_weights": (_i, [_vp, _vp, _vp, _i, _i]),
    "gd_nn_conv3x3_wide_weights_bytes": (C.c_size_t, [_i, _i]),
    "gd_nn_conv3x3_wide_forward": (_i, [_vp, _vp, _vp, _vp, _i, _vp, _vp, _i, _i, _i, _i, _i, _vp]),
    "gd_nn_conv3x3_wide_gn_forward": (_i, [_vp, _vp, _vp, _vp, _vp, _i, _i, _vp, _vp, _i, _vp, _vp, _i, _i, _i, _i, _i, _vp]),
    "gd_nn_groupnorm_finish_partials": (_i, [_vp, _vp, _i, C.c_size_t, _i, _i, _i, _f, _vp]),
    "gd_nn_conv3x3_first_forward": (_i, [_vp, _vp, _vp, _vp, _vp, _i, _i, _i, _i, _i]),
    "gd_nn_conv3x3_s2_forward": (_i, [_vp, _vp, _vp, _vp, _vp, _i, _i, _i, _i, _i, _i]),
    "gd_nn_conv3x3_s2_dgrad": (_i, [_vp, _vp, _vp, _vp, _i, _i, _i, _i, _i, _i]),
    "gd_nn_conv3x3_s2_ws_bytes": (C.c_size_t, [_i, _i, _i, _i, _i, _i, _i]),
    "gd_nn_conv3x3_s2_forward_ws": (_i, [_vp, _vp, _vp, _vp, _vp, _i, _i, _i, _i, _i, _i, _vp, C.c_size_t]),
    "gd_nn_conv3x3_s2_dgrad_ws": (_i, [_vp, _vp, _vp, _vp, _i, _i, _i, _i, _i, _i, _vp, C.c_size_t]),
    "gd_nn_conv3x3_up2_forward": (_i, [_vp, _vp, _vp, _vp, _vp, _vp, _i, _i, _i, _i, _i]),
    "gd_nn_conv_force_variant": (_i, [_i]),
    "gd_nn_linear_forward": (_i, [_vp, _vp, _vp, _vp, _vp, _vp, C.c_int64, _i, _i]),
    "gd_nn_gemm_supported": (_i, [C.c_int64, _i, _i, _i]),
    "gd_nn_gemm_forward": (_i, [_vp, _vp, _vp, _vp, _vp, _vp, C.c_int64, _i, _i]),
    "gd_nn_gemm_geglu_forward": (_i, [_vp, _vp, _vp, _vp, _vp, C.c_int64, _i, _i]),
    "gd_nn_gemm_last_error": (C.c_char_p, []),
    "gd_nn_conv_profile_enable": (_i, [_i]),
    "gd_nn_conv_profile_reset": (_i, []),
    "gd_nn_conv_profile_read": (_i, [C.POINTER(C.c_double), C.POINTER(C.c_int64), C.POINTER(C.c_double)]),
    "gd_nn_conv_profile_read_bytes": (_i, [C.POINTER(C.c_double)]),
    "gd_nn_geglu_forward": (_i, [_vp, _vp, _vp, C.c_int64, _i]),
    "gd_nn_geglu_backward": (_i, [_vp, _vp, _vp, _vp, C.c_int64, _i]),
    "gd_nn_conv1x1_c8": (_i, [_vp, _vp, _vp, _vp, _vp, C.c_int64, _i]),
    "gd_nn_softmax_rows_forward": (_i, [_vp, _vp, _vp, C.c_int64, _i]),
    "gd_nn_softmax_rows_backward": (_i, [_vp, _vp, _vp, _vp, C.c_int64, _i]),
    "gd_nn_layernorm_backward": (_i, [_vp, _vp, _vp, _vp, _vp, _vp, C.c_int64, _i, C.c_float]),
    "gd_nn_add_layernorm_forward": (_i, [_vp, _vp, _vp, _vp, _vp, _f, _vp, _vp, C.c_int64, _i]),
    "gd_nn_attention_ws_bytes": (C.c_size_t, [_i, _i, _i]),
    "gd_nn_attention_d64_forward": (_i, [_vp, _vp, _vp, _vp, _vp, _vp, _i, _i, _i, _i, C.c_int64, _i, C.c_int64, _i,
                                         C.c_int64, _i, C.c_int64, _i, _f, _i]),
    "gd_nn_attention_d64_forward_lse": (_i, [_vp, _vp, _vp, _vp, _vp, _vp, _vp, _i, _i, _i, _i, C.c_int64, _i, C.c_int64, _i,
                                             C.c_int64, _i, C.c_int64, _i, _f, _i]),
    "gd_nn_attention_bwd_ws_bytes": (C.c_size_t, [_i, _i, _i, _i]),
    "gd_nn_attention_d64_backward": (_i, [_vp] * 11 + [_i, _i, _i, _i] + [C.c_int64, _i] * 8 + [_f, _i]),
    "gd_nn_attention_d64_forward_vt": (_i, [_vp, _vp, _vp, _vp, _vp, _i, _i, _i, _i, C.c_int64, _i, C.c_int64, _i, C.c_int64, _i,
                                            _f]),
    "gd_nn_attention_d64_forward_vt_strided": (_i, [_vp, _vp, _vp, _vp, _vp, _i, _i, _i, _i, C.c_int64, _i, C.c_int64, _i, C.c_int64,
                                                    C.c_int64, _i, _f, _i]),
    "gd_nn_attention_last_error": (C.c_char_p, []),
    "gd_nn_vae_prologue_forward": (_i, [_vp, _vp, _vp, _i, _i, _i, _i, _i]),
    "gd_nn_vae_prologue_backward": (_i, [_vp, _vp, _vp, _i, _i, _i, _i, _i, _i]),
    "gd_nn_sparsity_forward": (_i, [_vp, _vp, _vp, C.c_int64, _vp]),
    "gd_nn_sparsity_backward": (_i, [_vp, _vp, _vp, _vp, C.c_int64, _vp]),
    "gd_nn_prologue_last_error": (C.c_char_p, []),
    "gd_nn_fp8_quantize": (_i, [_vp, _vp, _vp, C.c_int64, _f]),
    "gd_nn_fp8_pack_weights": (_i, [_vp, _vp, _vp, C.c_int64, _i, _i, _f]),
    "gd_nn_fp8_linear_forward": (_i, [_vp, _vp, _vp, _vp, _vp, _vp, C.c_int64, _i, _i, _i, _f]),
    "gd_nn_fp8_conv3x3_forward": (_i, [_vp, _vp, _vp, _vp, _i, _vp, _vp, _i, _i, _i, _i, _i, _i, _f]),
    "gd_nn_fp8_last_error": (C.c_char_p, []),
    "gd_nn_conv_last_error": (C.c_char_p, []),
    "gd_nn_elementwise_last_error": (C.c_char_p, []),
    "gd_nn_lora_rowdot": (_i, [_vp, _vp, _vp, _vp, C.c_int64, _i, C.c_float, _i]),
    "gd_nn_lora_rank4_add": (_i, [_vp, _vp, _vp, _vp, _vp, C.c_int64, _i, _i]),
    "gd_nn_lora_row_fused": (_i, [_vp, _vp, _vp, _vp, _vp, _vp, _vp, C.c_int64, _i, _i, C.c_float, _i]),
    "gd_nn_lora_colreduce_scratch_floats": (C.c_size_t, [C.c_int64, _i]),
    "gd_nn_lora_colreduce": (_i, [_vp, _vp, _vp, _vp, _vp, C.c_int64, _i, C.c_float, _i]),
    "gd_nn_lora_colreduce_pair_scratch_floats": (C.c_size_t, [C.c_int64, _i, _i]),
    "gd_nn_lora_colreduce_pair": (_i, [_vp, _vp, _vp, _vp, _vp, _vp, _vp, _vp, C.c_int64, _i, _i]),
    "gd_nn_lora_colreduce_pair_into": (_i, [_vp, _vp, _vp, _vp, _vp, _vp, _vp, _vp, C.c_int64, _i, _i, _i]),
    "gd_nn_lora_colreduce_group_entry_bytes": (C.c_size_t, []),
    "gd_nn_lora_colreduce_group_desc": (_i, [_vp, _vp, _vp, _vp, _vp, _vp, _vp, _vp, C.c_int64, _i, _i, _i, C.POINTER(C.c_int)]),
    "gd_nn_lora_colreduce_group_launch": (_i, [_vp, _vp, _i, _i, _i, _i]),
    "gd_nn_lora_last_error": (C.c_char_p, []),
    "gd_nn_vae_decoder_stem_supported": (_i, [_i, _i, _i, _i]),
    "gd_nn_vae_decoder_stem": (_i, [_vp, _vp, _i, _f, _vp, _vp, _vp, _vp, _vp, _i, _i, _i, _i]),
    "gd_nn_vae_decoder_head_supported": (_i, [_i, _i, _i, _i, _i]),
    "gd_nn_vae_decoder_head": (_i, [_vp, _vp, _vp, _vp, _vp, _i, _vp, _vp, _vp, _i, _i, _i, _i, _i]),
    "gd_nn_vae_decoder_last_error": (C.c_char_p, []),
    "gd_nn_last_error": (C.c_char_p, []),
}


def lib():
    global _lib
    if _lib is None:
        if not os.path.exists(_LIB_PATH):
            raise RuntimeError(f"{_LIB_PATH} not found: build with `python -m garmentdreamer_amd._build`; "
                               "the HIP guidance kernels have no fallback on GPU tensors")
        L = C.CDLL(_LIB_PATH)
        for name, (res, args) in SIGNATURES.items():
            try:
                fn = getattr(L, name)
            except AttributeError:
                if _LIB_OVERRIDDEN:
                    continue
                raise
            fn.restype, fn.argtypes = res, args
        _lib = L
    return _lib


def _check(ret, what, err="gd_nn_last_error"):
    if ret < 0:
        raise RuntimeError(f"{what} failed ({ret}): {getattr(lib(), err)().decode()}")


_gn_ws_cache = {}
_WS_TAG = [None]


class workspace_tag:

    def __init__(self, tag):
        self.tag = tag

    def __enter__(self):
        self.prev, _WS_TAG[0] = _WS_TAG[0], self.tag
        return self

    def __exit__(self, *exc):
        _WS_TAG[0] = self.prev
        return False


def _gn_workspace(x, N, groups):
    stream = torch.cuda.current_stream(x.device)
    key = (x.device.index, stream.cuda_stream, _WS_TAG[0])
    need = lib().gd_nn_groupnorm_ws_bytes(N, groups)
    ws = _gn_ws_cache.get(key)
    if ws is None or ws.numel() < need:
        ws = _gn_ws_cache[key] = torch.zeros(max(need, 1 << 16), dtype=torch.uint8, device=x.device)
    return ws


def reset_workspaces():
    _gn_ws_cache.clear()


_FALLBACKS = {}
_STRICT = False


def set_strict_library(on: bool) -> None:
    global _STRICT
    _STRICT = bool(on)


def library_fallbacks(reset: bool = False) -> dict:
    out = dict(_FALLBACKS)
    if reset:
        _FALLBACKS.clear()
    return out


def _note_fallback(op: str, x, why: str) -> None:
    if not (torch.is_tensor(x) and x.is_cuda and x.dtype == torch.bfloat16):
        return
    key = f"{op}: {why}"
    if _STRICT:
        raise RuntimeError(f"nn_ops strict mode: {key} on a bf16 GPU tensor of shape {tuple(x.shape)} would run on the PyTorch library op")
    _FALLBACKS[key] = _FALLBACKS.get(key, 0) + 1


def _is_nhwc_bf16(x):
    return x.is_cuda and x.dtype == torch.bfloat16 and x.dim() == 4 and x.is_contiguous(memory_format=torch.channels_last)


class _GroupNormSiLU(torch.autograd.Function):
    @staticmethod
    def forward(ctx, x, weight, bias, groups, eps, silu):
        N, Cc, H, W = x.shape
        L = lib()
        y = torch.empty_like(x, memory_format=torch.channels_last)
        ws = _gn_workspace(x, N, groups)
        mr = torch.empty(N * groups * 2, dtype=torch.float32, device=x.device)
        w, b = weight.contiguous(), bias.contiguous()
        with torch.cuda.device(x.device):
            stream = torch.cuda.current_stream(x.device).cuda_stream
            _check(L.gd_nn_groupnorm_silu_forward(stream, x.data_ptr(), y.data_ptr(), w.data_ptr(), b.data_ptr(), N,
                                                  H * W, Cc, groups, float(eps), int(silu), ws.data_ptr(),
                                                  mr.data_ptr()), "gd_nn_groupnorm_silu_forward")
        ctx.save_for_backward(x, w, b, mr)
        ctx.groups, ctx.silu = groups, silu
        return y

    @staticmethod
    def backward(ctx, dy):
        x, w, b, mr = ctx.saved_tensors
        N, Cc, H, W = x.shape
        L = lib()
        dy = dy.contiguous(memory_format=torch.channels_last)
        if dy.dtype != torch.bfloat16:
            dy = dy.to(torch.bfloat16)
        dx = torch.empty_like(x, memory_format=torch.channels_last)
        ws = _gn_workspace(x, N, ctx.groups)
        sums = torch.empty(N * ctx.groups * 2, dtype=torch.float32, device=x.device)
        with torch.cuda.device(x.device):
            stream = torch.cuda.current_stream(x.device).cuda_stream
            _check(L.gd_nn_groupnorm_silu_backward(stream, x.data_ptr(), dy.data_ptr(), w.data_ptr(), b.data_ptr(),
                                                   mr.data_ptr(), dx.data_ptr(), N, H * W, Cc, ctx.groups,
                                                   int(ctx.silu), ws.data_ptr(), sums.data_ptr(), None),
                   "gd_nn_groupnorm_silu_backward")
        return dx, None, None, None, None, None


_GN_FUSED_SMALL = os.environ.get("GD_NN_GN_SMALL", "1") != "0"


def _gn_fused_small(x, weight, bias, groups, eps, silu):
    N, Cc, H, W = x.shape
    y = torch.empty_like(x, memory_format=torch.channels_last)
    w, b = weight.contiguous(), bias.contiguous()
    with torch.cuda.device(x.device):
        _check(lib().gd_nn_groupnorm_silu_fused_forward(torch.cuda.current_stream(x.device).cuda_stream, x.data_ptr(),
                                                        y.data_ptr(), w.data_ptr(), b.data_ptr(), N, H * W, Cc, groups,
                                                        float(eps), int(silu)), "gd_nn_groupnorm_silu_fused_forward")
    return y


_GN_FUSED_TRAIN = os.environ.get("GD_NN_GN_SMALL_TRAIN", "1") != "0"


class _GroupNormSiLUSmall(torch.autograd.Function):

    @staticmethod
    def forward(ctx, x, weight, bias, groups, eps, silu):
        N, Cc, H, W = x.shape
        y = torch.empty_like(x, memory_format=torch.channels_last)
        mr = torch.empty(N * groups * 2, dtype=torch.float32, device=x.device)
        w, b = weight.contiguous(), bias.contiguous()
        with torch.cuda.device(x.device):
            _check(lib().gd_nn_groupnorm_silu_fused_forward_stats(
                torch.cuda.current_stream(x.device).cuda_stream, x.data_ptr(), y.data_ptr(), w.data_ptr(), b.data_ptr(), N,
                H * W, Cc, groups, float(eps), int(silu), mr.data_ptr()), "gd_nn_groupnorm_silu_fused_forward_stats")
        ctx.save_for_backward(x, w, b, mr)
        ctx.groups, ctx.silu = groups, silu
        return y

    @staticmethod
    def backward(ctx, dy):
        x, w, b, mr = ctx.saved_tensors
        N, Cc, H, W = x.shape
        dy = dy.contiguous(memory_format=torch.channels_last)
        if dy.dtype != torch.bfloat16:
            dy = dy.to(torch.bfloat16)
        dx = torch.empty_like(x, memory_format=torch.channels_last)
        L = lib()
        with torch.cuda.device(x.device):
            stream = torch.cuda.current_stream(x.device).cuda_stream
            if L.gd_nn_groupnorm_silu_fused_backward_supported(N, H * W, Cc, ctx.groups):
                _check(L.gd_nn_groupnorm_silu_fused_backward(stream, x.data_ptr(), dy.data_ptr(), w.data_ptr(), b.data_ptr(),
                                                             mr.data_ptr(), dx.data_ptr(), N, H * W, Cc, ctx.groups,
                                                             int(ctx.silu)), "gd_nn_groupnorm_silu_fused_backward")
            else:
                ws = _gn_workspace(x, N, ctx.groups)
                sums = torch.empty(N * ctx.groups * 2, dtype=torch.float32, device=x.device)
                _check(L.gd_nn_groupnorm_silu_backward(stream, x.data_ptr(), dy.data_ptr(), w.data_ptr(), b.data_ptr(),
                                                       mr.data_ptr(), dx.data_ptr(), N, H * W, Cc, ctx.groups,
                                                       int(ctx.silu), ws.data_ptr(), sums.data_ptr(), None),
                       "gd_nn_groupnorm_silu_backward")
        return dx, None, None, None, None, None


def group_norm_silu(x, weight, bias, groups: int, eps: float, silu: bool = True):
    if x.is_cuda:
        if weight.requires_grad or bias.requires_grad:
            raise RuntimeError("group_norm_silu HIP kernel computes input gradients only (frozen weights)")
        if x.dtype == torch.bfloat16 and x.dim() == 4 and x.shape[1] % 8 == 0:
            if not x.is_contiguous(memory_format=torch.channels_last):
                x = x.contiguous(memory_format=torch.channels_last)
            small = lib().gd_nn_groupnorm_silu_fused_supported(x.shape[0], x.shape[2] * x.shape[3], x.shape[1], groups)
            if torch.is_grad_enabled() and x.requires_grad:
                if small and _GN_FUSED_TRAIN:
                    return _GroupNormSiLUSmall.apply(x, weight, bias, groups, eps, silu)
            elif small and _GN_FUSED_SMALL:
                return _gn_fused_small(x, weight, bias, groups, eps, silu)
            return _GroupNormSiLU.apply(x, weight, bias, groups, eps, silu)
        _note_fallback("group_norm_silu", x, "needs a 4-D tensor with C % 8 == 0")
    y = F.group_norm(x, groups, weight, bias, eps)
    return F.silu(y) if silu else y



def _bias_and_stride(bias):
    if bias is None:
        return None, 0
    if bias.dim() == 1:
        return bias.contiguous(), 0
    if bias.stride(1) != 1 or bias.stride(0) % 8 or bias.storage_offset() % 8:
        bias = bias.contiguous()
    return bias, bias.stride(0)


_WINO = os.environ.get("GD_NN_WINO", "1") != "0"

_ROUTE_SCALE = 1
_ROUTE_RANK = 0
_ROUTE_BATCH = None
_ROUTE_OWNER = None


def set_route_scale(k: int, rank: int = 0, owner=None) -> None:
    global _ROUTE_SCALE, _ROUTE_RANK, _ROUTE_OWNER
    k, rank = int(k), int(rank)
    if not 0 <= rank < max(k, 1):
        raise ValueError(f"rank {rank} outside 0..{k - 1}")
    if lib().gd_nn_conv_set_route_scale(k) != 0:
        raise ValueError(f"route scale must be >= 1, got {k}")
    _ROUTE_SCALE, _ROUTE_RANK = k, rank
    _ROUTE_OWNER = weakref.ref(owner) if owner is not None else None


def release_route_scale(owner) -> None:
    cur = _ROUTE_OWNER() if _ROUTE_OWNER is not None else None
    if cur is owner:
        set_route_scale(1, 0)


def route_scale() -> int:
    return _ROUTE_SCALE


class route_batch:

    def __init__(self, groups: int, samples: int):
        self.value = (int(groups), int(samples))

    def __enter__(self):
        global _ROUTE_BATCH
        self.prev, _ROUTE_BATCH = _ROUTE_BATCH, self.value
        return self

    def __exit__(self, *exc):
        global _ROUTE_BATCH
        _ROUTE_BATCH = self.prev
        return False


def route_rows(rows):
    k, r = _ROUTE_SCALE, _ROUTE_RANK
    M, K = rows.shape
    G, B = _ROUTE_BATCH if _ROUTE_BATCH is not None else (1, 0)
    if B <= 0 or B % G or M % B:
        G, B = 1, 1
    c, T = B // G, M // B
    padded = rows.new_zeros((G, c, k, T, K))
    padded[:, :, r] = rows.view(G, c, T, K)

    def take(out):
        return out.view(G, c, k, T, out.shape[-1])[:, :, r].reshape(M, out.shape[-1])
    return padded.view(k * M, K), take


def _conv_route(N, H, W, Cin, Cout, gn=False):
    if not _WINO or Cin % 32 or Cout % 8 or Cout < 64 or H < 16 or W < 16:
        return None
    tiles_n = (Cout + 127) // 128
    if Cout <= 128 and (not gn or Cin <= 128) or (not gn and Cout == 640 and W == 32 and Cin >= 320):
        if N * _ROUTE_SCALE * ((H + 15) // 16) * ((W + 31) // 32) * tiles_n >= (256 if Cout <= 128 else 160) and \
                lib().gd_nn_conv3x3_wide_supported(N, H, W, Cin, Cout):
            return "wide"
    if gn or (Cin < 320 and Cout > 128):
        return None
    if N * _ROUTE_SCALE * ((H + 15) // 16) * ((W + 15) // 16) * tiles_n >= 128 and lib().gd_nn_conv3x3_wino_supported(N, H, W, Cin, Cout):
        return "wino"
    return None


def _conv_launch(x, w_khwc, bias, residual, out_channels):
    N, Cin, H, W = x.shape
    route = _conv_route(N, H, W, Cin, out_channels)
    if route == "wino":
        return _wino_launch(x, w_khwc, bias, residual, out_channels)
    if route == "wide":
        return _wide_launch(x, w_khwc, bias, residual, out_channels)
    L = lib()
    y = torch.empty((N, out_channels, H, W), dtype=torch.bfloat16, device=x.device,
                    memory_format=torch.channels_last)
    bias, stride = _bias_and_stride(bias)
    ws_bytes = L.gd_nn_conv3x3_ws_bytes(N, H, W, Cin, out_channels)
    ws = torch.empty(ws_bytes, dtype=torch.uint8, device=x.device) if ws_bytes else None
    with torch.cuda.device(x.device):
        stream = torch.cuda.current_stream(x.device).cuda_stream
        ret = L.gd_nn_conv3x3_forward_ws(stream, x.data_ptr(), w_khwc.data_ptr(),
                                         None if bias is None else bias.data_ptr(), stride,
                                         None if residual is None else residual.data_ptr(), y.data_ptr(), N, H, W, Cin,
                                         out_channels, None if ws is None else ws.data_ptr(), ws_bytes)
    if ret < 0:
        raise RuntimeError(f"gd_nn_conv3x3_forward failed ({ret}): {L.gd_nn_conv_last_error().decode()}")
    return y


def _patch_launch(x, w_khwc, bias, residual, out_channels):
    N, Cin, H, W = x.shape
    L = lib()
    y = torch.empty((N, out_channels, H, W), dtype=torch.bfloat16, device=x.device, memory_format=torch.channels_last)
    bias, stride = _bias_and_stride(bias)
    with torch.cuda.device(x.device):
        ret = L.gd_nn_conv3x3_gn_forward(torch.cuda.current_stream(x.device).cuda_stream, x.data_ptr(), None, None, None,
                                         0, 0, w_khwc.data_ptr(), None if bias is None else bias.data_ptr(), stride,
                                         None if residual is None else residual.data_ptr(), y.data_ptr(), N, H, W, Cin,
                                         out_channels)
    if ret < 0:
        raise RuntimeError(f"gd_nn_conv3x3_gn_forward failed ({ret}): {L.gd_nn_conv_last_error().decode()}")
    return y


def _wino(weight):
    u = getattr(weight, "_gd_wino", None)
    key = (weight.data_ptr(), weight._version)
    if u is None or u.device != weight.device or getattr(weight, "_gd_wino_key", None) != key:
        Cout, Cin = weight.shape[0], weight.shape[1]
        u = torch.empty(lib().gd_nn_conv3x3_wino_weights_bytes(Cout, Cin) // 2, dtype=torch.bfloat16, device=weight.device)
        with torch.cuda.device(weight.device):
            ret = lib().gd_nn_conv3x3_wino_weights(torch.cuda.current_stream(weight.device).cuda_stream,
                                                   weight.data_ptr(), u.data_ptr(), Cout, Cin)
        _check(ret, "gd_nn_conv3x3_wino_weights", "gd_nn_conv_last_error")
        weight._gd_wino, weight._gd_wino_key = u, key
    return u


def _wino_launch(x, w_khwc, bias, residual, out_channels, stat_part=None):
    N, Cin, H, W = x.shape
    L = lib()
    y = torch.empty((N, out_channels, H, W), dtype=torch.bfloat16, device=x.device, memory_format=torch.channels_last)
    bias, stride = _bias_and_stride(bias)
    u = _wino(w_khwc)
    with torch.cuda.device(x.device):
        ret = L.gd_nn_conv3x3_wino_forward(torch.cuda.current_stream(x.device).cuda_stream, x.data_ptr(), u.data_ptr(),
                                           None if bias is None else bias.data_ptr(), stride,
                                           None if residual is None else residual.data_ptr(), y.data_ptr(), N, H, W, Cin,
                                           out_channels, None if stat_part is None else stat_part.data_ptr())
    _check(ret, "gd_nn_conv3x3_wino_forward", "gd_nn_conv_last_error")
    return y


def _wide(weight):
    u = getattr(weight, "_gd_wide", None)
    key = (weight.data_ptr(), weight._version)
    if u is None or u.device != weight.device or getattr(weight, "_gd_wide_key", None) != key:
        Cout, Cin = weight.shape[0], weight.shape[1]
        u = torch.empty(lib().gd_nn_conv3x3_wide_weights_bytes(Cout, Cin) // 2, dtype=torch.bfloat16, device=weight.device)
        with torch.cuda.device(weight.device):
            ret = lib().gd_nn_conv3x3_wide_weights(torch.cuda.current_stream(weight.device).cuda_stream,
                                                   weight.data_ptr(), u.data_ptr(), Cout, Cin)
        _check(ret, "gd_nn_conv3x3_wide_weights", "gd_nn_conv_last_error")
        weight._gd_wide, weight._gd_wide_key = u, key
    return u


def _wide_launch(x, w_khwc, bias, residual, out_channels, stat_part=None, gn=None):
    N, Cin, H, W = x.shape
    L = lib()
    y = torch.empty((N, out_channels, H, W), dtype=torch.bfloat16, device=x.device, memory_format=torch.channels_last)
    bias, stride = _bias_and_stride(bias)
    u = _wide(w_khwc)
    with torch.cuda.device(x.device):
        st = torch.cuda.current_stream(x.device).cuda_stream
        tail = (u.data_ptr(), None if bias is None else bias.data_ptr(), stride, None if residual is None else residual.data_ptr(),
                y.data_ptr(), N, H, W, Cin, out_channels, None if stat_part is None else stat_part.data_ptr())
        if gn is None:
            ret = L.gd_nn_conv3x3_wide_forward(st, x.data_ptr(), *tail)
        else:
            mr, gw, gb, groups, silu = gn
            ret = L.gd_nn_conv3x3_wide_gn_forward(st, x.data_ptr(), mr.data_ptr(), gw.data_ptr(), gb.data_ptr(), groups,
                                                  int(silu), *tail)
    _check(ret, "gd_nn_conv3x3_wide_forward", "gd_nn_conv_last_error")
    return y


def _wino_gn_launch(x, mean_rstd, gn_weight, gn_bias, groups, silu, w_khwc, bias, residual, out_channels, stat_part=None):
    N, Cin, H, W = x.shape
    L = lib()
    y = torch.empty((N, out_channels, H, W), dtype=torch.bfloat16, device=x.device, memory_format=torch.channels_last)
    bias, stride = _bias_and_stride(bias)
    u = _wino(w_khwc)
    with torch.cuda.device(x.device):
        ret = L.gd_nn_conv3x3_wino_gn_forward(torch.cuda.current_stream(x.device).cuda_stream, x.data_ptr(),
                                              mean_rstd.data_ptr(), gn_weight.data_ptr(), gn_bias.data_ptr(), groups,
                                              int(silu), u.data_ptr(), None if bias is None else bias.data_ptr(), stride,
                                              None if residual is None else residual.data_ptr(), y.data_ptr(), N, H, W, Cin,
                                              out_channels, None if stat_part is None else stat_part.data_ptr())
    _check(ret, "gd_nn_conv3x3_wino_gn_forward", "gd_nn_conv_last_error")
# ... 545 lines not shown
        raise RuntimeError(f"gd_nn_geglu_forward failed ({ret}): {L.gd_nn_elementwise_last_error().decode()}")
    return x, y


class _GegluTrain(torch.autograd.Function):

    @staticmethod
    def forward(ctx, x):
        inner = x.shape[-1] // 2
        xc, y = _geglu_fwd(x, inner)
        ctx.save_for_backward(xc)
        return y

    @staticmethod
    def backward(ctx, dy):
        (x,) = ctx.saved_tensors
        inner = x.shape[-1] // 2
        dy = dy.contiguous()
        dx = torch.empty_like(x)
        L = lib()
        with torch.cuda.device(x.device):
            ret = L.gd_nn_geglu_backward(torch.cuda.current_stream(x.device).cuda_stream, x.data_ptr(), dy.data_ptr(),
                                         dx.data_ptr(), x.numel() // (2 * inner), inner)
        if ret < 0:
            raise RuntimeError(f"gd_nn_geglu_backward failed ({ret}): {L.gd_nn_elementwise_last_error().decode()}")
        return dx


def softmax_rows_(s):
    L = s.shape[-1]
    with torch.cuda.device(s.device):
        ret = lib().gd_nn_softmax_rows_forward(torch.cuda.current_stream(s.device).cuda_stream, s.data_ptr(), s.data_ptr(),
                                               s.numel() // L, L)
    if ret < 0:
        raise RuntimeError(f"gd_nn_softmax_rows_forward failed ({ret}): {lib().gd_nn_elementwise_last_error().decode()}")
    return s


def softmax_rows_backward_(p, dp):
    L = p.shape[-1]
    with torch.cuda.device(p.device):
        ret = lib().gd_nn_softmax_rows_backward(torch.cuda.current_stream(p.device).cuda_stream, p.data_ptr(), dp.data_ptr(),
                                                dp.data_ptr(), p.numel() // L, L)
    if ret < 0:
        raise RuntimeError(f"gd_nn_softmax_rows_backward failed ({ret}): {lib().gd_nn_elementwise_last_error().decode()}")
    return dp


class _SingleHeadAttention(torch.autograd.Function):

    @staticmethod
    def forward(ctx, qkv):
        Cc = qkv.shape[-1] // 3
        q, k, v = qkv[..., :Cc], qkv[..., Cc:2 * Cc], qkv[..., 2 * Cc:]
        p = softmax_rows_(torch.bmm(q, k.transpose(1, 2)))
        ctx.save_for_backward(qkv, p)
        return torch.bmm(p, v)

    @staticmethod
    def backward(ctx, do):
        qkv, p = ctx.saved_tensors
        Cc = qkv.shape[-1] // 3
        q, k, v = qkv[..., :Cc], qkv[..., Cc:2 * Cc], qkv[..., 2 * Cc:]
        do = do.contiguous()
        ds = softmax_rows_backward_(p, torch.bmm(do, v.transpose(1, 2)))
        dqkv = torch.empty_like(qkv)
        torch.bmm(ds, k, out=dqkv[..., :Cc])
        torch.bmm(ds.transpose(1, 2), q, out=dqkv[..., Cc:2 * Cc])
        torch.bmm(p.transpose(1, 2), do, out=dqkv[..., 2 * Cc:])
        return dqkv


def single_head_attention_supported(qkv) -> bool:
    return (qkv.is_cuda and qkv.dtype == torch.bfloat16 and qkv.dim() == 3 and qkv.is_contiguous() and qkv.shape[-1] % 24 == 0
            and qkv.shape[1] % 8 == 0 and qkv.shape[1] <= 8192)


def single_head_attention(qkv):
    return _SingleHeadAttention.apply(qkv)


def _conv1x1_c8_launch(x, weight, bias, transposed):
    y = torch.empty_like(x, memory_format=torch.channels_last)
    L = lib()
    with torch.cuda.device(x.device):
        ret = L.gd_nn_conv1x1_c8(torch.cuda.current_stream(x.device).cuda_stream, x.data_ptr(), weight.data_ptr(),
                                 None if bias is None else bias.data_ptr(), y.data_ptr(), x.numel() // 8, int(transposed))
    if ret < 0:
        raise RuntimeError(f"gd_nn_conv1x1_c8 failed ({ret}): {L.gd_nn_elementwise_last_error().decode()}")
    return y


class _Conv1x1C8(torch.autograd.Function):

    @staticmethod
    def forward(ctx, x, weight, bias):
        ctx.save_for_backward(weight)
        return _conv1x1_c8_launch(x, weight, bias, False)

    @staticmethod
    def backward(ctx, dy):
        (weight,) = ctx.saved_tensors
        return _conv1x1_c8_launch(dy.contiguous(memory_format=torch.channels_last), weight, None, True), None, None


def conv1x1_c8_supported(x, weight, bias) -> bool:
    return (x.is_cuda and x.dim() == 4 and x.shape[1] == 8 and x.dtype == torch.bfloat16 and tuple(weight.shape) == (8, 8, 1, 1)
            and weight.dtype == torch.bfloat16 and weight.is_contiguous() and not weight.requires_grad
            and (bias is None or (bias.dtype == torch.bfloat16 and bias.is_contiguous() and not bias.requires_grad))
            and x.data_ptr() % 16 == 0 and x.numel() > 0)


def conv1x1_c8(x, weight, bias=None):
    if not x.is_contiguous(memory_format=torch.channels_last):
        x = x.contiguous(memory_format=torch.channels_last)
    return _Conv1x1C8.apply(x, weight, bias)


_ATTN_TRAIN = os.environ.get("GD_ATTN_TRAIN", "1") != "0"
_ATTN_BWD = os.environ.get("GD_ATTN_BWD", "1") != "0"
_ATTN_BWD_MIN_KEYS = int(os.environ.get("GD_ATTN_BWD_MIN_KEYS", "1"))
_ROW_TRAIN = os.environ.get("GD_ROW_TRAIN", "1") != "0"


def geglu(x):
    inner = x.shape[-1] // 2
    if x.is_cuda and x.dtype == torch.bfloat16 and inner % 8 == 0 and x.shape[-1] == 2 * inner:
        if _rowwise_ok(x):
            return _geglu_fwd(x, inner)[1]
        if _ROW_TRAIN:
            return _GegluTrain.apply(x)
    h, gate = x.chunk(2, dim=-1)
    return h * F.gelu(gate)


def _ln_backward(s, dy, weight, ds, eps):
    Cc = s.shape[-1]
    dx = torch.empty_like(s)
    L = lib()
    with torch.cuda.device(s.device):
        ret = L.gd_nn_layernorm_backward(torch.cuda.current_stream(s.device).cuda_stream, s.data_ptr(), dy.data_ptr(),
                                         weight.data_ptr(), None if ds is None else ds.data_ptr(), dx.data_ptr(),
                                         s.numel() // Cc, Cc, float(eps))
    if ret < 0:
        raise RuntimeError(f"gd_nn_layernorm_backward failed ({ret}): {L.gd_nn_elementwise_last_error().decode()}")
    return dx


def _add_ln_fwd(x, residual, weight, bias, eps, want_sum):
    Cc = x.shape[-1]
    x = x.contiguous()
    if residual is not None:
        residual = residual.contiguous()
    s = torch.empty_like(x) if (residual is not None and want_sum) else None
    y = torch.empty_like(x)
    L = lib()
    with torch.cuda.device(x.device):
        ret = L.gd_nn_add_layernorm_forward(
            torch.cuda.current_stream(x.device).cuda_stream, x.data_ptr(),
            None if residual is None else residual.data_ptr(), weight.data_ptr(), bias.data_ptr(),
            float(eps), None if s is None else s.data_ptr(), y.data_ptr(), x.numel() // Cc, Cc)
    if ret < 0:
        raise RuntimeError(f"gd_nn_add_layernorm_forward failed ({ret}): {L.gd_nn_elementwise_last_error().decode()}")
    return (x if residual is None else s), y


class _AddLayerNormTrain(torch.autograd.Function):

    @staticmethod
    def forward(ctx, x, residual, weight, bias, eps):
        s, y = _add_ln_fwd(x, residual, weight, bias, eps, True)
        ctx.save_for_backward(s, weight)
        ctx.eps = eps
        ctx.has_res = residual is not None
        ctx.set_materialize_grads(False)
        if residual is None:
            return y
        return s, y

    @staticmethod
    def backward(ctx, *grads):
        s, weight = ctx.saved_tensors
        gs, gy = (None, grads[0]) if not ctx.has_res else grads
        if gy is None:
            d = gs
        else:
            d = _ln_backward(s, gy.contiguous(), weight, None if gs is None else gs.contiguous(), ctx.eps)
        return d, (d if ctx.has_res else None), None, None, None


def add_layer_norm(x, residual, norm, want_sum: bool = True):
    Cc = x.shape[-1]
    ok = Cc % 8 == 0 and Cc <= 2048 and norm.weight.dtype == torch.bfloat16 and x.is_cuda and x.dtype == torch.bfloat16 and \
        (residual is None or (residual.is_cuda and residual.dtype == torch.bfloat16))
    if ok and _rowwise_ok(x, residual, norm.weight, norm.bias):
        return _add_ln_fwd(x, residual, norm.weight, norm.bias, norm.eps, want_sum)
    if ok and _ROW_TRAIN and torch.is_grad_enabled() and not norm.weight.requires_grad and not norm.bias.requires_grad:
        if residual is None:
            return x, _AddLayerNormTrain.apply(x, None, norm.weight, norm.bias, float(norm.eps))
        return _AddLayerNormTrain.apply(x, residual, norm.weight, norm.bias, float(norm.eps))
    s = x if residual is None else x + residual
    return s, norm(s)



def _attention_d64_layout_ok(q, k, v) -> bool:
    ok = lambda t: (t.is_cuda and t.dtype == torch.bfloat16 and t.dim() == 4 and t.shape[-1] == 64 and t.stride(-1) == 1
                    and t.stride(2) == 64 and t.stride(1) % 8 == 0)
    return ok(q) and ok(k) and ok(v) and k.shape == v.shape and q.shape[0] == k.shape[0] and q.shape[2] == k.shape[2]


def attention_d64_supported(q, k, v) -> bool:
    return _attention_d64_layout_ok(q, k, v) and \
        not (torch.is_grad_enabled() and (q.requires_grad or k.requires_grad or v.requires_grad))


def attention_d64_train_supported(q, k, v) -> bool:
    return _ATTN_TRAIN and torch.is_grad_enabled() and (q.requires_grad or k.requires_grad or v.requires_grad) and \
        _attention_d64_layout_ok(q, k, v)


def attention_d64(q, k, v):
    B, S, H, _ = q.shape
    kv_len = k.shape[1]
    Skv = (kv_len + 63) // 64 * 64
    L = lib()
    o = torch.empty((B, S, H * 64), dtype=torch.bfloat16, device=q.device)
    ws = torch.empty(L.gd_nn_attention_ws_bytes(B, Skv, H), dtype=torch.uint8, device=q.device)
    with torch.cuda.device(q.device):
        ret = L.gd_nn_attention_d64_forward(torch.cuda.current_stream(q.device).cuda_stream, q.data_ptr(), k.data_ptr(),
                                            v.data_ptr(), o.data_ptr(), ws.data_ptr(), B, S, Skv, H, q.stride(0), q.stride(1),
                                            k.stride(0), k.stride(1), v.stride(0), v.stride(1), o.stride(0), o.stride(1),
                                            64 ** -0.5, kv_len)
    if ret < 0:
        raise RuntimeError(f"gd_nn_attention_d64_forward failed ({ret}): {L.gd_nn_attention_last_error().decode()}")
    return o


class _AttentionD64Train(torch.autograd.Function):

    @staticmethod
    def forward(ctx, q, k, v):
        B, S, H, _ = q.shape
        kv_len = k.shape[1]
        Skv = (kv_len + 63) // 64 * 64
        L = lib()
        o = torch.empty((B, S, H * 64), dtype=torch.bfloat16, device=q.device)
        lse = torch.empty((B, H, S), dtype=torch.float32, device=q.device)
        ws = torch.empty(L.gd_nn_attention_ws_bytes(B, Skv, H), dtype=torch.uint8, device=q.device)
        with torch.cuda.device(q.device):
            ret = L.gd_nn_attention_d64_forward_lse(torch.cuda.current_stream(q.device).cuda_stream, q.data_ptr(), k.data_ptr(),
                                                    v.data_ptr(), o.data_ptr(), lse.data_ptr(), ws.data_ptr(), B, S, Skv, H,
                                                    q.stride(0), q.stride(1), k.stride(0), k.stride(1), v.stride(0), v.stride(1),
                                                    o.stride(0), o.stride(1), 64 ** -0.5, kv_len)
        if ret < 0:
            raise RuntimeError(f"gd_nn_attention_d64_forward_lse failed ({ret}): {L.gd_nn_attention_last_error().decode()}")
        ctx.save_for_backward(q, k, v, o, lse)
        return o

    @staticmethod
    def backward(ctx, do):
        q, k, v, o, lse = ctx.saved_tensors
        B, S, H, _ = q.shape
        kv_len = k.shape[1]
        if _ATTN_BWD and S % 64 == 0 and kv_len >= _ATTN_BWD_MIN_KEYS:
            Skv = (kv_len + 63) // 64 * 64
            do = do.contiguous()
            L = lib()
            dq = torch.empty((B, S, H, 64), dtype=torch.bfloat16, device=q.device)
            dk = torch.empty((B, kv_len, H, 64), dtype=torch.bfloat16, device=q.device)
            dv = torch.empty((B, kv_len, H, 64), dtype=torch.bfloat16, device=q.device)
            ws = torch.empty(L.gd_nn_attention_bwd_ws_bytes(B, S, Skv, H), dtype=torch.uint8, device=q.device)
            with torch.cuda.device(q.device):
                ret = L.gd_nn_attention_d64_backward(
                    torch.cuda.current_stream(q.device).cuda_stream, q.data_ptr(), k.data_ptr(), v.data_ptr(), o.data_ptr(),
                    do.data_ptr(), lse.data_ptr(), dq.data_ptr(), dk.data_ptr(), dv.data_ptr(), ws.data_ptr(), B, S, Skv, H,
                    q.stride(0), q.stride(1), k.stride(0), k.stride(1), v.stride(0), v.stride(1), o.stride(0), o.stride(1),
                    do.stride(0), do.stride(1), dq.stride(0), dq.stride(1), dk.stride(0), dk.stride(1), dv.stride(0),
                    dv.stride(1), 64 ** -0.5, kv_len)
            if ret < 0:
                raise RuntimeError(f"gd_nn_attention_d64_backward failed ({ret}): {L.gd_nn_attention_last_error().decode()}")
            return dq, dk, dv
        z = torch.zeros((), dtype=torch.long, device=q.device)
        dq, dk, dv = torch.ops.aten._scaled_dot_product_flash_attention_backward(
            do.reshape(B, S, H, 64).transpose(1, 2), q.transpose(1, 2), k.transpose(1, 2), v.transpose(1, 2),
            o.view(B, S, H, 64).transpose(1, 2), lse, None, None, S, k.shape[1], 0.0, False, z, z, scale=64 ** -0.5)
        return dq.transpose(1, 2), dk.transpose(1, 2), dv.transpose(1, 2)


def attention_d64_train(q, k, v):
    return _AttentionD64Train.apply(q, k, v)


def attention_d64_vt(q, k, vt):
    B, S, H, _ = q.shape
    Skv = k.shape[1]
    assert vt.shape == (B, H * 64, Skv) and vt.is_contiguous() and vt.dtype == torch.bfloat16 and Skv % 64 == 0
    L = lib()
    o = torch.empty((B, S, H * 64), dtype=torch.bfloat16, device=q.device)
    with torch.cuda.device(q.device):
        ret = L.gd_nn_attention_d64_forward_vt(torch.cuda.current_stream(q.device).cuda_stream, q.data_ptr(), k.data_ptr(),
                                               vt.data_ptr(), o.data_ptr(), B, S, Skv, H, q.stride(0), q.stride(1),
                                               k.stride(0), k.stride(1), o.stride(0), o.stride(1), 64 ** -0.5)
    if ret < 0:
        raise RuntimeError(f"gd_nn_attention_d64_forward_vt failed ({ret}): {L.gd_nn_attention_last_error().decode()}")
    return o


def attention_d64_vt_strided(q, k, vt, kv_len: int):
    B, S, H, _ = q.shape
    Skv = vt.shape[2]
    assert vt.shape[:2] == (B, H * 64) and vt.stride(2) == 1 and vt.stride(1) == Skv and vt.dtype == torch.bfloat16 and Skv % 64 == 0
    L = lib()
    o = torch.empty((B, S, H * 64), dtype=torch.bfloat16, device=q.device)
    with torch.cuda.device(q.device):
        ret = L.gd_nn_attention_d64_forward_vt_strided(torch.cuda.current_stream(q.device).cuda_stream, q.data_ptr(), k.data_ptr(),
                                                       vt.data_ptr(), o.data_ptr(), B, S, Skv, H, q.stride(0), q.stride(1),
                                                       k.stride(0), k.stride(1), vt.stride(0), o.stride(0), o.stride(1),
                                                       64 ** -0.5, int(kv_len))
    if ret < 0:
        raise RuntimeError(f"gd_nn_attention_d64_forward_vt_strided failed ({ret}): {L.gd_nn_attention_last_error().decode()}")
    return o


class _VaePrologue(torch.autograd.Function):

    @staticmethod
    def forward(ctx, x, OH, OW):
        N, Cc, H, W = x.shape
        y = torch.empty((N, 3, OH, OW), dtype=torch.bfloat16, device=x.device, memory_format=torch.channels_last)
        L = lib()
        with torch.cuda.device(x.device):
            _check(L.gd_nn_vae_prologue_forward(torch.cuda.current_stream(x.device).cuda_stream, x.data_ptr(), y.data_ptr(),
                                                N, H, W, OH, OW), "gd_nn_vae_prologue_forward", "gd_nn_prologue_last_error")
        ctx.shape = (N, H, W, OH, OW)
        return y

    @staticmethod
    def backward(ctx, dy):
        N, H, W, OH, OW = ctx.shape
        if dy.dtype != torch.bfloat16:
            dy = dy.to(torch.bfloat16)
        base = dy._base if dy._base is not None and dy.storage_offset() == 0 else None
        if (base is not None and base.dtype == torch.bfloat16 and base.dim() == 4 and dy.shape[1] == 3
                and base.shape[0] == N and base.shape[1] >= 3 and base.shape[2:] == dy.shape[2:]
                and base.is_contiguous(memory_format=torch.channels_last) and dy.stride() == base.stride()
                and dy.data_ptr() == base.data_ptr()):
            src, CG = base, base.shape[1]
        else:
            src, CG = dy.contiguous(memory_format=torch.channels_last), 3
        dx = torch.empty((N, 3, H, W), dtype=torch.float32, device=dy.device)
        L = lib()
        with torch.cuda.device(dy.device):
            _check(L.gd_nn_vae_prologue_backward(torch.cuda.current_stream(dy.device).cuda_stream, src.data_ptr(),
                                                 dx.data_ptr(), N, H, W, OH, OW, CG), "gd_nn_vae_prologue_backward", "gd_nn_prologue_last_error")
        return dx, None, None


def vae_prologue_supported(x) -> bool:
    return x.is_cuda and x.dtype == torch.float32 and x.dim() == 4 and x.shape[1] == 3 and x.is_contiguous()


def vae_prologue(x, OH: int = 512, OW: int = 512):
    return _VaePrologue.apply(x, OH, OW)


VAE_HEAD_RAW, VAE_HEAD_IMAGE = 0, 1
_HEAD_MODES = {"raw": VAE_HEAD_RAW, "image": VAE_HEAD_IMAGE}


def _frozen_bf16(*ts) -> bool:
    return all(t is None or (t.is_cuda and t.dtype == torch.bfloat16 and not t.requires_grad) for t in ts)


def vae_decode_stem_supported(latents, pq_weight, pq_bias, weight, bias) -> bool:
    if not (latents.is_cuda and latents.dim() == 4 and latents.shape[1] == 4 and latents.dtype in (torch.float32, torch.bfloat16)):
        return False
    if torch.is_grad_enabled() and latents.requires_grad:
        return False
    if not (_frozen_bf16(pq_weight, pq_bias, weight, bias) and tuple(pq_weight.shape) == (4, 4, 1, 1)
            and weight.dim() == 4 and tuple(weight.shape[1:]) == (4, 3, 3)):
        return False
    N, _, h, w = latents.shape
    return bool(lib().gd_nn_vae_decoder_stem_supported(N, h, w, weight.shape[0]))


def vae_decode_stem(latents, inv_scale: float, pq_weight, pq_bias, weight, bias):
    if vae_decode_stem_supported(latents, pq_weight, pq_bias, weight, bias):
        lat = latents.contiguous()
        N, _, h, w = lat.shape
        Cout = weight.shape[0]
        wc = weight.contiguous(memory_format=torch.channels_last)
        y = torch.empty((N, Cout, h, w), dtype=torch.bfloat16, device=lat.device, memory_format=torch.channels_last)
        with torch.cuda.device(lat.device):
            _check(lib().gd_nn_vae_decoder_stem(torch.cuda.current_stream(lat.device).cuda_stream, lat.data_ptr(),
                                                int(lat.dtype == torch.bfloat16), float(inv_scale),
                                                pq_weight.contiguous().data_ptr(),
                                                None if pq_bias is None else pq_bias.contiguous().data_ptr(), wc.data_ptr(),
                                                None if bias is None else bias.contiguous().data_ptr(), y.data_ptr(), N, h, w,
                                                Cout), "gd_nn_vae_decoder_stem", "gd_nn_vae_decoder_last_error")
        return y
    _note_fallback("vae_decode_stem", weight, "needs [N, 4, h, w] fp32/bf16 GPU latents, frozen bf16 weights, Cout % 64 == 0 <= 512")
    z = (latents * inv_scale).to(weight.dtype)
    return F.conv2d(F.conv2d(z, pq_weight, pq_bias), weight, bias, padding=1)


def vae_decode_head_supported(x, norm_weight, norm_bias, groups: int, weight, bias) -> bool:
    if not (x.is_cuda and x.dtype == torch.bfloat16 and x.dim() == 4) or (torch.is_grad_enabled() and x.requires_grad):
        return False
    if not (_frozen_bf16(norm_weight, norm_bias, weight, bias) and weight.dim() == 4
            and tuple(weight.shape) == (3, x.shape[1], 3, 3) and norm_weight.numel() == x.shape[1]):
        return False
    N, C, H, W = x.shape
    return bool(lib().gd_nn_vae_decoder_head_supported(N, H, W, C, int(groups)))


def vae_decode_head(x, norm_weight, norm_bias, groups: int, eps: float, weight, bias, mode: str = "image", mean_rstd=None):
    m = _HEAD_MODES[mode]
    if vae_decode_head_supported(x, norm_weight, norm_bias, groups, weight, bias):
        x = x.contiguous(memory_format=torch.channels_last)
        N, C, H, W = x.shape
        L = lib()
        out = torch.empty((N, 3, H, W), dtype=torch.bfloat16 if m == VAE_HEAD_RAW else torch.float32, device=x.device,
                          memory_format=torch.channels_last)
        wc = weight.contiguous(memory_format=torch.channels_last)
        with torch.cuda.device(x.device):
            stream = torch.cuda.current_stream(x.device).cuda_stream
            if mean_rstd is None:
                mean_rstd = torch.empty(N * groups * 2, dtype=torch.float32, device=x.device)
                _check(L.gd_nn_groupnorm_stats(stream, x.data_ptr(), N, H * W, C, groups, float(eps),
                                               _gn_workspace(x, N, groups).data_ptr(), mean_rstd.data_ptr()),
                       "gd_nn_groupnorm_stats")
            elif mean_rstd.dtype != torch.float32 or mean_rstd.numel() != N * groups * 2 or not mean_rstd.is_contiguous():
                raise ValueError("vae_decode_head: mean_rstd must be contiguous fp32 [N * groups * 2]")
            _check(L.gd_nn_vae_decoder_head(stream, x.data_ptr(), mean_rstd.data_ptr(), norm_weight.contiguous().data_ptr(),
                                            norm_bias.contiguous().data_ptr(), int(groups), wc.data_ptr(),
                                            None if bias is None else bias.contiguous().data_ptr(), out.data_ptr(), m, N, H,
                                            W, C), "gd_nn_vae_decoder_head", "gd_nn_vae_decoder_last_error")
        return out
    _note_fallback("vae_decode_head", x, "needs bf16 GPU activations with C % 64 == 0 <= 256 and frozen bf16 C -> 3 weights")
    r = F.conv2d(F.silu(F.group_norm(x, groups, norm_weight, norm_bias, eps)), weight, bias, padding=1)
    if m == VAE_HEAD_RAW:
        return r
    return (r.float() * 0.5 + 0.5).clamp(0, 1).contiguous(memory_format=torch.channels_last)


class _SparsityHead(torch.autograd.Function):

    @staticmethod
    def forward(ctx, depth, dmax):
        d = depth.contiguous()
        m = dmax.detach().reshape(1).to(torch.float32)
        sums = torch.empty(2, dtype=torch.float64, device=d.device)
        n = d.numel()
        L = lib()
        with torch.cuda.device(d.device):
            _check(L.gd_nn_sparsity_forward(torch.cuda.current_stream(d.device).cuda_stream, d.data_ptr(), m.data_ptr(), n,
                                            sums.data_ptr()), "gd_nn_sparsity_forward", "gd_nn_prologue_last_error")
        ctx.save_for_backward(d, m, sums)
        return (sums[0] / n).to(torch.float32)

    @staticmethod
    def backward(ctx, g):
        d, m, sums = ctx.saved_tensors
        n = d.numel()
        g32 = g.reshape(1).to(torch.float32).contiguous()
        dd = torch.empty_like(d)
        L = lib()
        with torch.cuda.device(d.device):
            _check(L.gd_nn_sparsity_backward(torch.cuda.current_stream(d.device).cuda_stream, d.data_ptr(), m.data_ptr(),
                                             g32.data_ptr(), n, dd.data_ptr()), "gd_nn_sparsity_backward", "gd_nn_prologue_last_error")
        dmax_grad = (-(sums[1] / n).to(torch.float32) / (m[0] + 1e-5)) * g32[0]
        return dd, dmax_grad.reshape(())

# ... 449 lines not shown
```

### include/gd_nn.h

```cpp
#ifndef GD_NN_H_INCLUDED
#define GD_NN_H_INCLUDED

#include <stddef.h>
#include <stdint.h>

#ifdef __cplusplus
extern "C" {
#endif

#define GD_NN_OK 0
#define GD_NN_ERR_INVALID_ARG (-1)
#define GD_NN_ERR_HIP (-2)

int gd_nn_groupnorm_silu_forward(void* stream, const void* x, void* y, const void* gamma, const void* beta, int N,
                                 int HW, int C, int G, float eps, int apply_silu, double* stats_ws,
                                 float* mean_rstd);

int gd_nn_groupnorm_silu_backward(void* stream, const void* x, const void* dy, const void* gamma,
                                  const void* beta, const float* mean_rstd, void* dx, int N, int HW, int C, int G,
                                  int apply_silu, double* stats_ws, float* group_sums ,
                                  const void* add);

size_t gd_nn_groupnorm_ws_bytes(int N, int G);

int gd_nn_conv3x3_forward(void* stream, const void* x, const void* weight, const void* bias, int bias_img_stride,
                          const void* residual, void* y, int N, int H, int W, int Cin, int Cout);

int gd_nn_conv3x3_flip_weights(void* stream, const void* weight, void* flipped, int Cout, int Cin);

int gd_nn_conv3x3_first_dgrad_supported(int N, int H, int W, int Cin, int Cout);
int gd_nn_conv3x3_first_dgrad_weights(void* stream, const void* weight, void* wpack, int Cout, int Cin);
int gd_nn_conv3x3_first_dgrad(void* stream, const void* dy, const void* wpack, void* dx4, int N, int H, int W, int Cin, int Cout);

int gd_nn_conv_force_variant(int v);

int gd_nn_linear_forward(void* stream, const void* x, const void* weight, const void* bias, const void* residual, void* y,
                         int64_t M, int K, int Nout);
int gd_nn_gemm_supported(int64_t M, int K, int N, int geglu);
int gd_nn_gemm_forward(void* stream, const void* x, const void* weight, const void* bias, const void* residual, void* y,
                       int64_t M, int K, int N);
int gd_nn_gemm_geglu_forward(void* stream, const void* x, const void* weight, const void* bias, void* y, int64_t M, int K,
                             int inner);
const char* gd_nn_gemm_last_error(void);
int gd_nn_conv_profile_enable(int on);
int gd_nn_conv_profile_reset(void);
int gd_nn_conv_profile_read(double* total_ms, int64_t* launches, double* total_flops);
int gd_nn_conv_profile_read_bytes(double* total_bytes);

size_t gd_nn_conv3x3_ws_bytes(int N, int H, int W, int Cin, int Cout);
int gd_nn_conv3x3_forward_ws(void* stream, const void* x, const void* weight, const void* bias, int bias_img_stride,
                             const void* residual, void* y, int N, int H, int W, int Cin, int Cout, void* ws,
                             size_t ws_bytes);
int gd_nn_conv_force_split(int s);
int gd_nn_conv_set_route_scale(int k);

int gd_nn_groupnorm_silu_fused_supported(int N, int HW, int C, int G);
int gd_nn_groupnorm_silu_fused_forward(void* stream, const void* x, void* y, const void* gamma, const void* beta, int N,
                                       int HW, int C, int G, float eps, int apply_silu);
int gd_nn_groupnorm_silu_fused_forward_stats(void* stream, const void* x, void* y, const void* gamma, const void* beta, int N,
                                             int HW, int C, int G, float eps, int apply_silu, float* mean_rstd);
int gd_nn_groupnorm_silu_fused_backward_supported(int N, int HW, int C, int G);
int gd_nn_groupnorm_silu_fused_backward(void* stream, const void* x, const void* dy, const void* gamma, const void* beta,
                                        const float* mean_rstd, void* dx, int N, int HW, int C, int G, int apply_silu);

int gd_nn_groupnorm_stats(void* stream, const void* x, int N, int HW, int C, int G, float eps, double* stats_ws,
                          float* mean_rstd);

int gd_nn_conv3x3_gn_forward(void* stream, const void* x, const float* mean_rstd, const void* gamma, const void* beta,
                             int groups, int apply_silu, const void* weight, const void* bias, int bias_img_stride,
                             const void* residual, void* y, int N, int H, int W, int Cin, int Cout);

size_t gd_nn_conv3x3_stat_rows(int N, int H, int W, int Cout, int gn_entry);
int gd_nn_conv3x3_gn_forward_stats(void* stream, const void* x, const float* mean_rstd, const void* gamma,
                                   const void* beta, int groups, int apply_silu, const void* weight, const void* bias,
                                   int bias_img_stride, const void* residual, void* y, int N, int H, int W, int Cin,
                                   int Cout, float* stat_part);
int gd_nn_conv3x3_forward_stats(void* stream, const void* x, const void* weight, const void* bias, int bias_img_stride,
                                const void* residual, void* y, int N, int H, int W, int Cin, int Cout, float* stat_part);
int gd_nn_conv3x3_wino_supported(int N, int H, int W, int Cin, int Cout);
size_t gd_nn_conv3x3_wino_weights_bytes(int Cout, int Cin);
int gd_nn_conv3x3_wino_weights(void* stream, const void* weight, void* u, int Cout, int Cin);
int gd_nn_conv3x3_wino_forward(void* stream, const void* x, const void* u, const void* bias, int bias_img_stride,
                               const void* residual, void* y, int N, int H, int W, int Cin, int Cout, float* stat_part);
int gd_nn_conv3x3_wino_gn_forward(void* stream, const void* x, const float* mean_rstd, const void* gamma, const void* beta,
                                  int groups, int apply_silu, const void* u, const void* bias, int bias_img_stride,
                                  const void* residual, void* y, int N, int H, int W, int Cin, int Cout, float* stat_part);
int gd_nn_conv3x3_wide_supported(int N, int H, int W, int Cin, int Cout);
size_t gd_nn_conv3x3_wide_weights_bytes(int Cout, int Cin);
int gd_nn_conv3x3_wide_weights(void* stream, const void* weight, void* u, int Cout, int Cin);
int gd_nn_conv3x3_wide_forward(void* stream, const void* x, const void* u, const void* bias, int bias_img_stride,
                               const void* residual, void* y, int N, int H, int W, int Cin, int Cout, float* stat_part);
int gd_nn_conv3x3_wide_gn_forward(void* stream, const void* x, const float* mean_rstd, const void* gamma, const void* beta,
                                  int groups, int apply_silu, const void* u, const void* bias, int bias_img_stride,
                                  const void* residual, void* y, int N, int H, int W, int Cin, int Cout, float* stat_part);
size_t gd_nn_conv3x3_first_stat_rows(int N, int H, int W, int Cin, int Cout);
int gd_nn_conv3x3_first_forward_stats(void* stream, const void* x, const void* weight, const void* bias, void* y, int N,
                                      int H, int W, int Cin, int Cout, float* stat_part);
int gd_nn_groupnorm_finish_partials(void* stream, const float* stat_part, int N, size_t rows, int C, int G, int HW,
                                    float eps, float* mean_rstd);

int gd_nn_linear_320_supported(int64_t M, int K, int N);
int gd_nn_linear_k320_forward(void* stream, const void* x, const void* weight, const void* bias, void* y, int64_t M, int N);
int gd_nn_linear_320_forward(void* stream, const void* x, const void* weight, const void* bias, void* y, int64_t M);
int gd_nn_linear_k320_geglu_forward(void* stream, const void* x, const void* weight, const void* bias, void* y, int64_t M,
                                    int inner);
const char* gd_nn_linear_320_last_error(void);

int gd_nn_conv3x3_first_forward(void* stream, const void* x, const void* weight, const void* bias, void* y, int N, int H,
                                int W, int Cin, int Cout);

int gd_nn_conv3x3_s2_forward(void* stream, const void* x, const void* weight, const void* bias, void* y, int N, int Hin,
                             int Win, int Cin, int Cout, int pad_lo);

int gd_nn_conv3x3_up2_forward(void* stream, const void* x, const void* w_even_rows, const void* w_odd_rows,
                              const void* bias, void* y, int N, int H, int W, int Cin, int Cout);

int gd_nn_conv3x3_s2_dgrad(void* stream, const void* dy, const void* weight_flipped, void* dx, int N, int Hin, int Win,
                           int Cin, int Cout, int pad_lo);

size_t gd_nn_conv3x3_s2_ws_bytes(int N, int Hin, int Win, int Cin, int Cout, int pad_lo, int dgrad);
int gd_nn_conv3x3_s2_forward_ws(void* stream, const void* x, const void* weight, const void* bias, void* y, int N,
                                int Hin, int Win, int Cin, int Cout, int pad_lo, void* ws, size_t ws_bytes);
int gd_nn_conv3x3_s2_dgrad_ws(void* stream, const void* dy, const void* weight_flipped, void* dx, int N, int Hin, int Win,
                              int Cin, int Cout, int pad_lo, void* ws, size_t ws_bytes);

int gd_nn_geglu_forward(void* stream, const void* x, void* y, int64_t rows, int inner);
int gd_nn_geglu_backward(void* stream, const void* x, const void* dy, void* dx, int64_t rows, int inner);
int gd_nn_layernorm_backward(void* stream, const void* s, const void* dy, const void* weight, const void* ds, void* dx,
                             int64_t rows, int C, float eps);

int gd_nn_add_layernorm_forward(void* stream, const void* x, const void* residual, const void* weight, const void* bias,
                                float eps, void* sum_out, void* y, int64_t rows, int C);

size_t gd_nn_attention_ws_bytes(int B, int Skv, int H);
int gd_nn_attention_d64_forward(void* stream, const void* q, const void* k, const void* v, void* o, void* vt_ws, int B, int S,
                                int Skv, int H, int64_t q_bs, int q_rs, int64_t k_bs, int k_rs, int64_t v_bs, int v_rs,
                                int64_t o_bs, int o_rs, float scale, int kv_len);
int gd_nn_attention_d64_forward_lse(void* stream, const void* q, const void* k, const void* v, void* o, float* lse, void* vt_ws,
                                    int B, int S, int Skv, int H, int64_t q_bs, int q_rs, int64_t k_bs, int k_rs, int64_t v_bs,
                                    int v_rs, int64_t o_bs, int o_rs, float scale, int kv_len);
size_t gd_nn_attention_bwd_ws_bytes(int B, int S, int Skv, int H);
int gd_nn_attention_d64_backward(void* stream, const void* q, const void* k, const void* v, const void* o, const void* dout,
                                 const float* lse, void* dq, void* dk, void* dv, void* ws, int B, int S, int Skv, int H,
                                 int64_t q_bs, int q_rs, int64_t k_bs, int k_rs, int64_t v_bs, int v_rs, int64_t o_bs, int o_rs,
                                 int64_t do_bs, int do_rs, int64_t dq_bs, int dq_rs, int64_t dk_bs, int dk_rs, int64_t dv_bs,
                                 int dv_rs, float scale, int kv_len);
int gd_nn_attention_d64_forward_vt(void* stream, const void* q, const void* k, const void* vt, void* o, int B, int S, int Skv,
                                   int H, int64_t q_bs, int q_rs, int64_t k_bs, int k_rs, int64_t o_bs, int o_rs, float scale);
int gd_nn_attention_d64_forward_vt_strided(void* stream, const void* q, const void* k, const void* vt, void* o, int B, int S,
                                           int Skv, int H, int64_t q_bs, int q_rs, int64_t k_bs, int k_rs, int64_t vt_bs,
                                           int64_t o_bs, int o_rs, float scale, int kv_len);
const char* gd_nn_attention_last_error(void);

int gd_nn_vae_prologue_forward(void* stream, const float* x, void* y, int N, int H, int W, int OH, int OW);
int gd_nn_vae_prologue_backward(void* stream, const void* dy, float* dx, int N, int H, int W, int OH, int OW, int CG);

int gd_nn_sparsity_forward(void* stream, const float* depth, const float* dmax, int64_t n, double* sums2);
int gd_nn_sparsity_backward(void* stream, const float* depth, const float* dmax, const float* grad_out, int64_t n,
                            float* d_depth);
const char* gd_nn_prologue_last_error(void);

int gd_nn_fp8_quantize(void* stream, const void* x_bf16, void* y_fp8, int64_t n, float inv_scale);
int gd_nn_groupnorm_silu_forward_fp8(void* stream, const void* x, void* y_fp8, const void* gamma, const void* beta, int N,
                                     int HW, int C, int G, float eps, int apply_silu, double* stats_ws, float* mean_rstd,
                                     float inv_scale);
int gd_nn_fp8_pack_weights(void* stream, const void* w_bf16, void* w_fp8, int64_t rows, int K, int Kp, float inv_scale);
int gd_nn_fp8_linear_forward(void* stream, const void* x_fp8, const void* w_fp8, const void* bias, const void* residual,
                             void* y, int64_t M, int K, int Kp, int Nout, float dq);
int gd_nn_fp8_conv3x3_forward(void* stream, const void* x_fp8, const void* w_fp8, const void* bias, int bias_img_stride,
                              const void* residual, void* y, int N, int H, int W, int Cin, int CinP, int Cout, float dq);
const char* gd_nn_fp8_last_error(void);

const char* gd_nn_conv_last_error(void);
int gd_nn_conv1x1_c8(void* stream, const void* x, const void* weight, const void* bias, void* y, int64_t npix, int transposed);
int gd_nn_softmax_rows_forward(void* stream, const void* x, void* y, int64_t rows, int L);
int gd_nn_softmax_rows_backward(void* stream, const void* p, const void* dp, void* ds, int64_t rows, int L);
const char* gd_nn_elementwise_last_error(void);
int gd_nn_lora_rowdot(void* stream, const void* a, const float* w, float* h, int64_t M, int K, float scale, int w_is_k_by_4);
int gd_nn_lora_rank4_add(void* stream, const float* h, const float* w, const void* base, void* y, int64_t M, int N, int w_is_n_by_4);
int gd_nn_lora_row_fused(void* stream, const void* a, const float* w1, const float* w2, const void* base, float* h, void* y,
                         int64_t M, int K, int N, float scale, int backward);
size_t gd_nn_lora_colreduce_scratch_floats(int64_t M, int J);
int gd_nn_lora_colreduce(void* stream, const void* a, const float* v, float* scratch, float* g, int64_t M, int J, float scale,
                         int g_is_j_by_4);
size_t gd_nn_lora_colreduce_pair_scratch_floats(int64_t M, int N, int K);
int gd_nn_lora_colreduce_pair(void* stream, const void* dy, const float* hs, const void* x, const float* dh, float* scratch,
                              float* d_up, float* d_down, int64_t M, int N, int K);
int gd_nn_lora_colreduce_pair_into(void* stream, const void* dy, const float* hs, const void* x, const float* dh, float* scratch,
                                   float* d_up, float* d_down, int64_t M, int N, int K, int accumulate);
size_t gd_nn_lora_colreduce_group_entry_bytes(void);
int gd_nn_lora_colreduce_group_desc(void* entry, const void* dy, const float* hs, const void* x, const float* dh, float* scratch,
                                    float* d_up, float* d_down, int64_t M, int N, int K, int accumulate, int* grid_xyz);
int gd_nn_lora_colreduce_group_launch(void* stream, const void* table_host, int n_entries, int grid1_x, int grid1_y, int grid2_x);
const char* gd_nn_lora_last_error(void);

int gd_nn_vae_decoder_stem_supported(int N, int h, int w, int Cout);
int gd_nn_vae_decoder_stem(void* stream, const void* latents, int latents_bf16, float inv_scale, const void* pq_weight,
                           const void* pq_bias, const void* weight, const void* bias, void* y, int N, int h, int w, int Cout);

#define GD_NN_VAE_HEAD_RAW 0
#define GD_NN_VAE_HEAD_IMAGE 1
int gd_nn_vae_decoder_head_supported(int N, int H, int W, int C, int G);
int gd_nn_vae_decoder_head(void* stream, const void* x, const float* mean_rstd, const void* gamma, const void* beta, int G,
                           const void* weight, const void* bias, void* out, int mode, int N, int H, int W, int C);
const char* gd_nn_vae_decoder_last_error(void);

const char* gd_nn_last_error(void);

#ifdef __cplusplus
}
#endif
#endif
```

Baseline: 22.74.

## Share batch-identical UNet work across CFG reps and fuse joins with GroupNorm stats

Adds a reps mechanism so the first resnet, norm, proj_in and self-attention of a down block run once on shared images and are then broadcast across classifier-free-guidance copies. A broadcasting add-layernorm kernel reads the shared input per row. New join kernels fuse residual add or skip concat with per-block GroupNorm partial statistics, so the next GroupNorm can skip its stats pass. This cuts duplicated compute and memory passes, but adds complex broadcasting bookkeeping and extra repeat/launch calls where the sharing does not apply.

New measurement: 23.00, median of 6. 1.01x the previous value.

```diff
diff --git a/garmentdreamer_amd/csrc/nn_elementwise.hip b/garmentdreamer_amd/csrc/nn_elementwise.hip
--- a/garmentdreamer_amd/csrc/nn_elementwise.hip
+++ b/garmentdreamer_amd/csrc/nn_elementwise.hip
@@ -38,12 +38,13 @@
 __global__ __launch_bounds__(256) void add_layernorm_kernel(const bf16x8* __restrict__ x, const bf16x8* __restrict__ r,
                                                             const bf16x8* __restrict__ w, const bf16x8* __restrict__ b,
                                                             bf16x8* __restrict__ s_out, bf16x8* __restrict__ y,
-                                                            int64_t rows, int vpr , float eps)
+                                                            int64_t rows, int vpr , float eps,
+                                                            int64_t x_rows )
 {
     const int lane = threadIdx.x & 63;
     const int64_t row = (int64_t)blockIdx.x * (blockDim.x >> 6) + (threadIdx.x >> 6);
     if (row >= rows) return;
-    const bf16x8* xr = x + row * vpr;
+    const bf16x8* xr = x + (row < x_rows ? row : row % x_rows) * vpr;
     f2 v[VPL][4];
     f2 sum2 = {0.f, 0.f};
 #pragma unroll
@@ -305,6 +306,108 @@
         for (int e = 0; e < 4; e++) out.w[e] = pack2(f2{o[2 * e], o[2 * e + 1]});
         y[p] = out;
     }
+}
+
+constexpr int kJoinUnroll = 4;
+constexpr int kJoinMaxThreads = 320;
+
+template <bool CONCAT, bool STATS>
+__global__ __launch_bounds__(kJoinMaxThreads) void join_gn_partials_kernel(const bf16x8* __restrict__ a,
+                                                                           const bf16x8* __restrict__ b,
+                                                                           bf16x8* __restrict__ out, float2* __restrict__ part,
+                                                                           int HW, int vpa, int vpp, int rows, int ppb, int Nb)
+{
+    __shared__ float4 s_red[kJoinMaxThreads];
+    const int n = blockIdx.y, nb = n % Nb;
+    const int tv = threadIdx.x % vpp, tr = threadIdx.x / vpp;
+    const int p0 = blockIdx.x * ppb, p1 = min(HW, p0 + ppb);
+    const bool from_b = CONCAT && tv >= vpa;
+    const int vps = CONCAT ? (from_b ? vpp - vpa : vpa) : vpp;
+    const int sv = from_b ? tv - vpa : tv;
+    const bf16x8* src = from_b ? b + (size_t)nb * HW * vps : a + (size_t)n * HW * vps;
+    const bf16x8* bn = b + (size_t)nb * HW * vpp;
+    bf16x8* on = out + (size_t)n * HW * vpp;
+    f2 s[2] = {f2{0.f, 0.f}, f2{0.f, 0.f}}, ss[2] = {f2{0.f, 0.f}, f2{0.f, 0.f}};
+    auto body = [&](const bf16x8& va, const bf16x8& vb, int p) {
+        u32x4 o = __builtin_bit_cast(u32x4, va);
+        if (!CONCAT) {
+            const u32x4 wb = __builtin_bit_cast(u32x4, vb);
+#pragma unroll
+            for (int k = 0; k < 4; k++) o.w[k] = pack2(unpack2(o.w[k]) + unpack2(wb.w[k]));
+        }
+        on[(size_t)p * vpp + tv] = __builtin_bit_cast(bf16x8, o);
+        if (STATS) {
+#pragma unroll
+            for (int k = 0; k < 4; k++) {
+                const f2 f = unpack2(o.w[k]);
+                s[k >> 1] += f;
+                ss[k >> 1] += f * f;
+            }
+        }
+    };
+    int p = p0 + tr;
+    for (; p + (kJoinUnroll - 1) * rows < p1; p += kJoinUnroll * rows) {
+        bf16x8 va[kJoinUnroll], vb[kJoinUnroll];
+#pragma unroll
+        for (int u = 0; u < kJoinUnroll; u++) {
+            va[u] = src[(size_t)(p + u * rows) * vps + sv];
+            if (!CONCAT) vb[u] = bn[(size_t)(p + u * rows) * vpp + tv];
+        }
+#pragma unroll
+        for (int u = 0; u < kJoinUnroll; u++) body(va[u], CONCAT ? va[u] : vb[u], p + u * rows);
+    }
+    for (; p < p1; p += rows) {
+        const bf16x8 va = src[(size_t)p * vps + sv];
+        body(va, CONCAT ? va : bn[(size_t)p * vpp + tv], p);
+    }
+    if (!STATS) return;
+    s_red[threadIdx.x] = float4{s[0].x + s[0].y, ss[0].x + ss[0].y, s[1].x + s[1].y, ss[1].x + ss[1].y};
+    __syncthreads();
+    for (int q = threadIdx.x; q < 2 * vpp; q += blockDim.x) {
+        float sa = 0.f, sb = 0.f;
+        for (int r = 0; r < rows; r++) {
+            const float4 v = s_red[r * vpp + (q >> 1)];
+            sa += (q & 1) ? v.z : v.x;
+            sb += (q & 1) ? v.w : v.y;
+        }
+        part[((size_t)n * (2 * vpp) + q) * gridDim.x + blockIdx.x] = float2{sa, sb};
+    }
+}
+
+bool join_geo(int N, int HW, int C, int* vpp, int* rows, int* ppb, int* nblk)
+{
+    if (N <= 0 || N > 65535 || HW <= 0 || C <= 0 || C % 8 || C / 8 > kJoinMaxThreads) return false;
+    *vpp = C / 8;
+    *rows = *vpp >= 256 ? 1 : 256 / *vpp;
+    int p = 128;
+    while (p > *rows && (long)((HW + p - 1) / p) * N < 2048) p >>= 1;
+    if (p < *rows) p = *rows;
+    *ppb = p;
+    *nblk = (HW + p - 1) / p;
+    return true;
+}
+
+bool aligned16(const void* p) { return ((uintptr_t)p & 15) == 0; }
+
+template <bool CONCAT>
+int join_launch(void* stream, const void* a, const void* b, void* out, float* part, int N, int Nb, int HW, int C0, int C1)
+{
+    const int C = CONCAT ? C0 + C1 : C0;
+    int vpp, rows, ppb, nblk;
+    if (!a || !b || !out) return fail(GD_NN_ERR_INVALID_ARG, "join: null pointer");
+    if (!aligned16(a) || !aligned16(b) || !aligned16(out)) return fail(GD_NN_ERR_INVALID_ARG, "join: tensors must be 16-byte aligned");
+    if (C0 <= 0 || C0 % 8 || (CONCAT && (C1 <= 0 || C1 % 8)) || !join_geo(N, HW, C, &vpp, &rows, &ppb, &nblk))
+        return fail(GD_NN_ERR_INVALID_ARG, "join: need channel counts that are multiples of 8, C <= 2560, N <= 65535");
+    if (Nb <= 0 || Nb > N || N % Nb) return fail(GD_NN_ERR_INVALID_ARG, "join: the images of b must divide N");
+    if ((int64_t)N * HW * C >= (int64_t)1 << 40) return fail(GD_NN_ERR_INVALID_ARG, "join: tensor too large");
+    const dim3 grid(nblk, N), block(rows * vpp);
+    if (part)
+        hipLaunchKernelGGL((join_gn_partials_kernel<CONCAT, true>), grid, block, 0, (hipStream_t)stream, (const bf16x8*)a,
+                           (const bf16x8*)b, (bf16x8*)out, (float2*)part, HW, C0 / 8, vpp, rows, ppb, Nb);
+    else
+        hipLaunchKernelGGL((join_gn_partials_kernel<CONCAT, false>), grid, block, 0, (hipStream_t)stream, (const bf16x8*)a,
+                           (const bf16x8*)b, (bf16x8*)out, (float2*)nullptr, HW, C0 / 8, vpp, rows, ppb, Nb);
+    return launch_status("join: launch failed");
 }
 
 }
@@ -328,10 +431,19 @@
 int gd_nn_add_layernorm_forward(void* stream, const void* x, const void* residual, const void* weight, const void* bias,
                                 float eps, void* sum_out, void* y, int64_t rows, int C)
 {
+    return gd_nn_add_layernorm_forward_bcast(stream, x, residual, weight, bias, eps, sum_out, y, rows, C, rows);
+}
+
+int gd_nn_add_layernorm_forward_bcast(void* stream, const void* x, const void* residual, const void* weight,
+                                      const void* bias, float eps, void* sum_out, void* y, int64_t rows, int C,
+                                      int64_t x_rows)
+{
     if (!x || !weight || !bias || !y) return fail(GD_NN_ERR_INVALID_ARG, "add_layernorm: null pointer");
     if (rows <= 0 || C <= 0 || C % 8 || C > 64 * 8 * 4)
         return fail(GD_NN_ERR_INVALID_ARG, "add_layernorm: need C % 8 == 0 and C <= 2048");
     if (sum_out && !residual) return fail(GD_NN_ERR_INVALID_ARG, "add_layernorm: sum_out without residual");
+    if (x_rows <= 0 || x_rows > rows || rows % x_rows || (x_rows != rows && !residual))
+        return fail(GD_NN_ERR_INVALID_ARG, "add_layernorm: x_rows must divide rows (and a shared x needs a residual)");
     const int vpr = C / 8;
     const int vpl = (vpr + 63) / 64;
     const int64_t blocks = (rows + 3) / 4;
@@ -339,13 +451,31 @@
 #define GD_LN(V_)                                                                                                      \
     hipLaunchKernelGGL(add_layernorm_kernel<V_>, dim3((unsigned)blocks), dim3(256), 0, (hipStream_t)stream,            \
                        (const bf16x8*)x, (const bf16x8*)residual, (const bf16x8*)weight, (const bf16x8*)bias,          \
-                       (bf16x8*)sum_out, (bf16x8*)y, rows, vpr, eps)
+                       (bf16x8*)sum_out, (bf16x8*)y, rows, vpr, eps, x_rows)
     if (vpl == 1) GD_LN(1);
     else if (vpl == 2) GD_LN(2);
     else if (vpl == 3) GD_LN(3);
     else GD_LN(4);
 #undef GD_LN
     return launch_status("add_layernorm: launch failed");
+}
+
+size_t gd_nn_join_stat_rows(int N, int HW, int C)
+{
+    int vpp, rows, ppb, nblk;
+    return join_geo(N, HW, C, &vpp, &rows, &ppb, &nblk) ? (size_t)nblk : 0;
+}
+
+int gd_nn_add_gn_partials(void* stream, const void* a, const void* b, void* out, float* stat_part, int N, int Nb, int HW,
+                          int C)
+{
+    return join_launch<false>(stream, a, b, out, stat_part, N, Nb, HW, C, 0);
+}
+
+int gd_nn_concat_gn_partials(void* stream, const void* a, const void* b, void* out, float* stat_part, int N, int Nb, int HW,
+                             int C0, int C1)
+{
+    return join_launch<true>(stream, a, b, out, stat_part, N, Nb, HW, C0, C1);
 }
 
 int gd_nn_geglu_backward(void* stream, const void* x, const void* dy, void* dx, int64_t rows, int inner)
diff --git a/garmentdreamer_amd/guidance/sd21.py b/garmentdreamer_amd/guidance/sd21.py
--- a/garmentdreamer_amd/guidance/sd21.py
+++ b/garmentdreamer_amd/guidance/sd21.py
@@ -30,7 +30,8 @@
 
 
 def _gn(norm: nn.GroupNorm, x, silu: bool):
-    return group_norm_silu(x, norm.weight, norm.bias, norm.num_groups, norm.eps, silu)
+    mr = nn_ops.gn_stats_of(x, norm.num_groups, norm.eps) if x.is_cuda else None
+    return group_norm_silu(x, norm.weight, norm.bias, norm.num_groups, norm.eps, silu, mean_rstd=mr)
 
 
 def _conv3(conv: nn.Conv2d, x, image_bias=None, residual=None):
@@ -179,21 +180,29 @@
             "to_out_lora": LoRALinearLayer(inner, self.to_out[0].out_features, rank)})
         return self.lora
 
-    def forward(self, x, context=None):
+    def forward(self, x, context=None, reps: int = 1):
         B, N, _ = x.shape
         kv = context_vt = None
         if isinstance(context, ContextProjections):
             kv = context.kv.get(id(self)) if self.lora is None else None
             context_vt = context.vt
             context = context.context
+        if reps > 1 and kv is None:
+            x = x.repeat(reps, 1, 1)
+            B, reps = B * reps, 1
         ctx = x if context is None else context
         if kv is not None:
-            q, (k, v) = _lin(self.to_q, x), kv
+            with nn_ops.route_batch_shared(reps):
+                q = _lin(self.to_q, x)
+            k, v = kv
             vt = context_vt.get(id(self)) if context_vt is not None else None
             if vt is not None and N >= 256 and _CTX_VT and q.shape[-1] == 64 * self.heads and not torch.is_grad_enabled():
-                q4, k4 = q.view(B, N, self.heads, 64), k.view(B, k.shape[1], self.heads, 64)
-                if nn_ops._attention_d64_layout_ok(q4, k4, k4):
+                q4, k4 = q.view(B, N, self.heads, 64), k.view(B * reps, k.shape[1], self.heads, 64)
+                if nn_ops._attention_d64_layout_ok(q4, k4[:B], k4[:B]):
                     return _lin(self.to_out[0], nn_ops.attention_d64_vt_strided(q4, k4, vt, k.shape[1]))
+            if reps > 1:
+                q = q.repeat(reps, 1, 1)
+                B = B * reps
         elif _FUSED_QKV and context is None and self.lora is None and x.is_cuda and self.to_q.bias is None and \
                 not self.to_q.weight.requires_grad and not torch.is_grad_enabled():
             src = (self.to_q.weight.data_ptr(), self.to_q.weight._version, self.to_k.weight._version,
@@ -284,10 +293,11 @@
         self.norm3 = nn.LayerNorm(dim)
         self.ff = FeedForward(dim)
 
-    def forward(self, x, context, defer_ff_bias: bool = False):
-        _, n = add_layer_norm(x, None, self.norm1)
-        x, n = add_layer_norm(x, self.attn1(n), self.norm2)
-        x, n = add_layer_norm(x, self.attn2(n, context), self.norm3)
+    def forward(self, x, context, defer_ff_bias: bool = False, reps: int = 1):
+        with nn_ops.route_batch_shared(reps):
+            _, n = add_layer_norm(x, None, self.norm1)
+            x, n = add_layer_norm(x, self.attn1(n), self.norm2)
+        x, n = add_layer_norm(x, self.attn2(n, context, reps=reps), self.norm3)
         if defer_ff_bias:
             g = self.ff.net[0](n)
             return _lib_addmm(x.reshape(-1, x.shape[-1]), g.reshape(-1, g.shape[-1]), self.ff.net[2].weight.t()).view_as(x)
@@ -311,21 +321,24 @@
             self._fold_key = key
         return self._fold_bias
 
-    def forward(self, x, context):
+    def forward(self, x, context, next_norm=None, reps: int = 1):
         B, C, H, W = x.shape
-        h = _gn(self.norm, x, False)
-        h = h.permute(0, 2, 3, 1).reshape(B, H * W, C)
-        h = _lin(self.proj_in, h)
+        with nn_ops.route_batch_shared(reps):
+            h = _gn(self.norm, x, False)
+            h = h.permute(0, 2, 3, 1).reshape(B, H * W, C)
+            h = _lin(self.proj_in, h)
         if len(self.transformer_blocks) == 1 and h.is_cuda and not torch.is_grad_enabled() and \
                 not self.proj_out.weight.requires_grad:
-            h = self.transformer_blocks[0](h, context, defer_ff_bias=True)
+            h = self.transformer_blocks[0](h, context, defer_ff_bias=True, reps=reps)
             h = _lin(self.proj_out, h, self._folded_out_bias(h.dtype))
         else:
-            for blk in self.transformer_blocks:
-                h = blk(h, context)
+            for i, blk in enumerate(self.transformer_blocks):
+                h = blk(h, context, reps=reps if i == 0 else 1)
             h = self.proj_out(h)
-        h = h.reshape(B, H, W, C).permute(0, 3, 1, 2)
-        return h + x
+        h = h.reshape(B * reps, H, W, C).permute(0, 3, 1, 2)
+        if h.is_cuda and not torch.is_grad_enabled():
+            return nn_ops.add_join(h, x, next_norm)
+        return h + (x if reps == 1 else x.repeat(reps, 1, 1, 1))
 
 
 class Downsample2D(nn.Module):
@@ -363,11 +376,19 @@
             [Transformer2DModel(out_ch, heads, out_ch // heads, cross_dim) for _ in range(n_layers)]) if attn else None
         self.downsamplers = nn.ModuleList([Downsample2D(out_ch)]) if down else None
 
-    def forward(self, x, temb, context, skips):
+    def forward(self, x, temb, context, skips, reps: int = 1, temb_shared=None):
+        n = len(self.resnets)
         for i, res in enumerate(self.resnets):
-            x = res(x, temb)
+            if reps > 1 and i == 0:
+                with nn_ops.route_batch_shared(reps):
+                    x = res(x, temb_shared)
+                if self.attentions is None:
+                    x = x.repeat(reps, 1, 1, 1)
+            else:
+                x = res(x, temb)
             if self.attentions is not None:
-                x = self.attentions[i](x, context)
+                x = self.attentions[i](x, context, next_norm=self.resnets[i + 1].norm1 if i + 1 < n else None,
+                                       reps=reps if i == 0 else 1)
             skips.append(x)
         if self.downsamplers is not None:
             x = self.downsamplers[0](x)
@@ -388,12 +409,19 @@
             [Transformer2DModel(out_ch, heads, out_ch // heads, cross_dim) for _ in range(n_layers)]) if attn else None
         self.upsamplers = nn.ModuleList([Upsample2D(out_ch)]) if up else None
 
-    def forward(self, x, temb, context, skips):
+    def forward(self, x, temb, context, skips, next_norm=None):
+        n = len(self.resnets)
         for i, res in enumerate(self.resnets):
-            x = torch.cat([x, skips.pop()], dim=1)
+            skip = skips.pop()
+            if x.is_cuda and not torch.is_grad_enabled():
+                x = nn_ops.concat_join(x, skip, res.norm1)
+            else:
+                x = torch.cat([x, skip if skip.shape[0] == x.shape[0] else skip.repeat(x.shape[0] // skip.shape[0], 1, 1, 1)],
+                              dim=1)
             x = res(x, temb)
             if self.attentions is not None:
-                x = self.attentions[i](x, context)
+                x = self.attentions[i](x, context,
+                                       next_norm=next_norm if i + 1 == n and self.upsamplers is None else None)
         if self.upsamplers is not None:
             x = self.upsamplers[0](x)
         return x
@@ -494,13 +522,14 @@
             voff += c
         return ContextProjections(ctx, kv, vt)
 
-    def _project_temb(self, temb):
+    def _project_temb(self, temb, reps: int = 1):
         train = torch.is_grad_enabled() and temb.requires_grad
+        plain = (temb, temb.repeat(reps, 1)) if reps > 1 else temb
         if not temb.is_cuda or (train and not _TEMB_TRAIN_CAT):
-            return temb
+            return plain
         blocks = [m for m in self.modules() if isinstance(m, ResnetBlock2D) and m.time_emb_proj is not None]
         if not blocks or any(b.time_emb_proj.weight.requires_grad or b.conv1.bias.requires_grad for b in blocks):
-            return temb
+            return plain
         first = blocks[0].time_emb_proj.weight
         key = (first.data_ptr(), temb.dtype, len(blocks)) + tuple(
             t._version for b in blocks for t in (b.time_emb_proj.weight, b.time_emb_proj.bias, b.conv1.bias))
@@ -515,12 +544,17 @@
             return TembProjections(temb, {id(b): p for b, p in zip(blocks, parts)})
         with torch.no_grad():
             allp = _lib_linear(F.silu(temb), cache[1], cache[2])
-        out, off = {}, 0
-        for b in blocks:
-            c = b.time_emb_proj.out_features
-            out[id(b)] = allp[:, off:off + c]
-            off += c
-        return TembProjections(temb, out)
+
+        def slices(t, allp):
+            out, off = {}, 0
+            for b in blocks:
+                c = b.time_emb_proj.out_features
+                out[id(b)] = allp[:, off:off + c]
+                off += c
+            return TembProjections(t, out)
+        if reps > 1:
+            return slices(temb, allp), slices(temb.repeat(reps, 1), allp.repeat(reps, 1))
+        return slices(temb, allp)
 
     fp8 = None
 
@@ -529,33 +563,58 @@
         self.fp8 = state if state is not None else Fp8State()
         return self.fp8
 
-    def forward(self, sample, timestep, encoder_hidden_states, **kwargs):
+    supports_shared_reps = True
+
+    def forward(self, sample, timestep, encoder_hidden_states, shared_reps: int = 1, **kwargs):
         if self.fp8 is not None and not torch.is_grad_enabled() and sample.is_cuda:
             _FP8_ACTIVE[0] = self.fp8
             try:
-                return self._forward(sample, timestep, encoder_hidden_states, **kwargs)
+                return self._forward(sample, timestep, encoder_hidden_states, shared_reps, **kwargs)
             finally:
                 _FP8_ACTIVE[0] = None
-        return self._forward(sample, timestep, encoder_hidden_states, **kwargs)
-
-    def _forward(self, sample, timestep, encoder_hidden_states, **kwargs):
+        return self._forward(sample, timestep, encoder_hidden_states, shared_reps, **kwargs)
+
+    def _shared_prefix_ok(self, sample) -> bool:
+        return (sample.is_cuda and not torch.is_grad_enabled() and not self.conv_in.weight.requires_grad
+                and type(self).extra_embedding is UNet2DConditionModel.extra_embedding
+                and self.down_blocks[0].attentions is not None)
+
+    def _forward(self, sample, timestep, encoder_hidden_states, shared_reps: int = 1, **kwargs):
         dtype = self.conv_in.weight.dtype
+        reps = int(shared_reps)
+        if reps < 1 or encoder_hidden_states.shape[0] != sample.shape[0] * reps:
+            raise ValueError(f"shared_reps={reps}: {sample.shape[0]} samples need {sample.shape[0] * max(reps, 1)} contexts, "
+                             f"got {encoder_hidden_states.shape[0]}")
+        if reps > 1 and not self._shared_prefix_ok(sample):
+            sample = torch.cat([sample] * reps, dim=0)
+            if timestep.dim() > 0:
+                timestep = torch.cat([timestep] * reps)
+            reps = 1
         if timestep.dim() == 0:
             timestep = timestep[None].expand(sample.shape[0])
-        temb = self.time_embedding(sinusoidal_timestep_embedding(timestep, self.block_out_channels[0]).to(dtype))
-        extra = self.extra_embedding(sample.shape[0], **kwargs)
-        if extra is not None:
-            temb = temb + extra.to(dtype)
-        temb = self._project_temb(temb)
-        x = conv3x3_small_cin(sample.to(dtype).contiguous(memory_format=torch.channels_last), self.conv_in.weight,
-                              self.conv_in.bias)
+        with nn_ops.route_batch_shared(reps):
+            temb = self.time_embedding(sinusoidal_timestep_embedding(timestep, self.block_out_channels[0]).to(dtype))
+            extra = self.extra_embedding(sample.shape[0], **kwargs)
+            if extra is not None:
+                temb = temb + extra.to(dtype)
+            temb_shared = None
+            if reps > 1:
+                temb_shared, temb = self._project_temb(temb, reps)
+            else:
+                temb = self._project_temb(temb)
+            x = conv3x3_small_cin(sample.to(dtype).contiguous(memory_format=torch.channels_last), self.conv_in.weight,
+                                  self.conv_in.bias)
         ctx = self._project_context(encoder_hidden_states.to(dtype))
         skips = [x]
-        for blk in self.down_blocks:
-            x = blk(x, temb, ctx, skips)
+        for i, blk in enumerate(self.down_blocks):
+            if i == 0 and reps > 1:
+                x = blk(x, temb, ctx, skips, reps=reps, temb_shared=temb_shared)
+            else:
+                x = blk(x, temb, ctx, skips)
         x = self.mid_block(x, temb, ctx)
-        for blk in self.up_blocks:
-            x = blk(x, temb, ctx, skips)
+        last = len(self.up_blocks) - 1
+        for i, blk in enumerate(self.up_blocks):
+            x = blk(x, temb, ctx, skips, next_norm=self.conv_norm_out if i == last else None)
         return _conv3(self.conv_out, _gn(self.conv_norm_out, x, True))
 
 
diff --git a/garmentdreamer_amd/guidance/stable_diffusion_guidance.py b/garmentdreamer_amd/guidance/stable_diffusion_guidance.py
--- a/garmentdreamer_amd/guidance/stable_diffusion_guidance.py
+++ b/garmentdreamer_amd/guidance/stable_diffusion_guidance.py
@@ -9,6 +9,9 @@
 
 from .. import _runtime_env, nn_ops
 from . import sd21
+
+import os as _os
+_SHARED_PREFIX = _os.environ.get("GD_SHARED_PREFIX", "1") != "0"
 
 
 def C(value: Any, epoch: int, global_step: int) -> float:
@@ -109,13 +112,17 @@
         self.min_step = int(self.num_train_timesteps * min_step_percent)
         self.max_step = int(self.num_train_timesteps * max_step_percent)
 
-    def forward_unet(self, latents, t, encoder_hidden_states):
+    def _shared_reps(self, reps: int) -> dict:
+        return {"shared_reps": reps} if _SHARED_PREFIX and reps > 1 and getattr(self.unet, "supports_shared_reps", False) else {}
+
+    def forward_unet(self, latents, t, encoder_hidden_states, shared_reps: int = 1):
+        kw = {"shared_reps": int(shared_reps)} if shared_reps > 1 else {}
         input_dtype = latents.dtype
         t_dtype = torch.float32 if self.weights_dtype == torch.bfloat16 else self.weights_dtype
         x, tt, ctx = latents.to(self.weights_dtype), t.to(t_dtype), encoder_hidden_states.to(self.weights_dtype)
         fp8 = getattr(self.unet, "fp8", None)
         if fp8 is not None and not self._fp8_calibrated and not torch.is_grad_enabled():
-            out = self.unet(x, tt, encoder_hidden_states=ctx).to(input_dtype)
+            out = self.unet(x, tt, encoder_hidden_states=ctx, **kw).to(input_dtype)
             self._fp8_calib_done += 1
             if self._fp8_calib_done >= max(1, int(self.cfg.fp8_calibration_steps)):
                 fp8.mode = "run"
@@ -123,15 +130,15 @@
             return out
         if self.cfg.use_hip_graphs and x.is_cuda and not torch.is_grad_enabled():
             try:
-                return self._graphed_unet(x, tt, ctx).to(input_dtype)
+                return self._graphed_unet(x, tt, ctx, **kw).to(input_dtype)
             except RuntimeError as e:
                 self._graphs_failed(e)
-        return self.unet(x, tt, encoder_hidden_states=ctx).to(input_dtype)
+        return self.unet(x, tt, encoder_hidden_states=ctx, **kw).to(input_dtype)
 
     def may_capture(self, batch_size: int) -> bool:
         if not self.cfg.use_hip_graphs:
             return False
-        have_u = any(k[0][0] in (2 * batch_size, 4 * batch_size) for k in self._unet_graphs)
+        have_u = any(k[1][0] in (2 * batch_size, 4 * batch_size) for k in self._unet_graphs)
         have_v = any(k[0] == batch_size for k in self._vae_graphs)
         return not (have_u and have_v)
 
@@ -145,8 +152,8 @@
         from .. import nn_ops
         nn_ops.reset_workspaces()
 
-    def _graphed_unet(self, x, t, ctx):
-        key = (tuple(x.shape), tuple(ctx.shape))
+    def _graphed_unet(self, x, t, ctx, **kw):
+        key = (tuple(x.shape), tuple(ctx.shape)) + tuple(sorted(kw.items()))
         entry = self._unet_graphs.get(key)
         if entry is None:
             sx, st, sc = x.clone(), t.clone(), ctx.clone()
@@ -154,11 +161,11 @@
             side.wait_stream(torch.cuda.current_stream(x.device))
             with torch.cuda.stream(side), torch.no_grad():
                 for _ in range(2):
-                    self.unet(sx, st, encoder_hidden_states=sc)
+                    self.unet(sx, st, encoder_hidden_states=sc, **kw)
             torch.cuda.current_stream(x.device).wait_stream(side)
             g = torch.cuda.CUDAGraph()
             with _runtime_env.capture_guard(), torch.cuda.graph(g), torch.no_grad():
-                out = self.unet(sx, st, encoder_hidden_states=sc)
+                out = self.unet(sx, st, encoder_hidden_states=sc, **kw)
             entry = self._unet_graphs[key] = (g, sx, st, sc, out)
         g, sx, st, sc, out = entry
         sx.copy_(x)
@@ -212,9 +219,13 @@
                 if noise is None:
                     noise = torch.randn_like(latents)
                 latents_noisy = self.scheduler.add_noise(latents, noise, t)
+                share = self._shared_reps(4)
                 with nn_ops.route_batch(4, 4 * batch_size):
-                    noise_pred = self.forward_unet(torch.cat([latents_noisy] * 4, dim=0), torch.cat([t] * 4),
-                                                   encoder_hidden_states=text_embeddings)
+                    if share:
+                        noise_pred = self.forward_unet(latents_noisy, t, encoder_hidden_states=text_embeddings, **share)
+                    else:
+                        noise_pred = self.forward_unet(torch.cat([latents_noisy] * 4, dim=0), torch.cat([t] * 4),
+                                                       encoder_hidden_states=text_embeddings)
             noise_pred_text = noise_pred[:batch_size]
             noise_pred_uncond = noise_pred[batch_size:batch_size * 2]
             noise_pred_neg = noise_pred[batch_size * 2:]
@@ -233,10 +244,13 @@
                 if noise is None:
                     noise = torch.randn_like(latents)
                 latents_noisy = self.scheduler.add_noise(latents, noise, t)
-                latent_model_input = torch.cat([latents_noisy] * 2, dim=0)
+                share = self._shared_reps(2)
                 with nn_ops.route_batch(2, 2 * batch_size):
-                    noise_pred = self.forward_unet(latent_model_input, torch.cat([t] * 2),
-                                                   encoder_hidden_states=text_embeddings)
+                    if share:
+                        noise_pred = self.forward_unet(latents_noisy, t, encoder_hidden_states=text_embeddings, **share)
+                    else:
+                        noise_pred = self.forward_unet(torch.cat([latents_noisy] * 2, dim=0), torch.cat([t] * 2),
+                                                       encoder_hidden_states=text_embeddings)
             noise_pred_text, noise_pred_uncond = noise_pred.chunk(2)
             noise_pred = noise_pred_text + self.cfg.guidance_scale * (noise_pred_text - noise_pred_uncond)
 
@@ -274,9 +288,13 @@
             y = latents
             zs = y + sigma * noise
             scaled_zs = zs / torch.sqrt(1 + sigma ** 2)
+            share = self._shared_reps(reps)
             with nn_ops.route_batch(reps, reps * batch_size):
-                noise_pred = self.forward_unet(torch.cat([scaled_zs] * reps, dim=0), torch.cat([t] * reps),
-                                               encoder_hidden_states=text_embeddings)
+                if share:
+                    noise_pred = self.forward_unet(scaled_zs, t, encoder_hidden_states=text_embeddings, **share)
+                else:
+                    noise_pred = self.forward_unet(torch.cat([scaled_zs] * reps, dim=0), torch.cat([t] * reps),
+                                                   encoder_hidden_states=text_embeddings)
         if use_perp_neg:
             noise_pred_text = noise_pred[:batch_size]
             noise_pred_uncond = noise_pred[batch_size:batch_size * 2]
@@ -362,10 +380,15 @@
         batch_size = latents_noisy.shape[0]
         reps = 4 if use_perp_neg else 2
         from .. import nn_ops
+        share = self._shared_reps(reps)
         with nn_ops.route_batch(reps, reps * batch_size):
-            noise_pred = self.forward_unet(torch.cat([latents_noisy] * reps, dim=0),
-                                           torch.cat([t.reshape(1)] * reps).to(self.device),
-                                           encoder_hidden_states=text_embeddings)
+            if share:
+                noise_pred = self.forward_unet(latents_noisy, t.reshape(1).to(self.device),
+                                               encoder_hidden_states=text_embeddings, **share)
+            else:
+                noise_pred = self.forward_unet(torch.cat([latents_noisy] * reps, dim=0),
+                                               torch.cat([t.reshape(1)] * reps).to(self.device),
+                                               encoder_hidden_states=text_embeddings)
         if use_perp_neg:
             noise_pred_text = noise_pred[:batch_size]
             noise_pred_uncond = noise_pred[batch_size:batch_size * 2]
diff --git a/garmentdreamer_amd/nn_ops.py b/garmentdreamer_amd/nn_ops.py
--- a/garmentdreamer_amd/nn_ops.py
+++ b/garmentdreamer_amd/nn_ops.py
@@ -88,6 +88,10 @@
     "gd_nn_softmax_rows_backward": (_i, [_vp, _vp, _vp, _vp, C.c_int64, _i]),
     "gd_nn_layernorm_backward": (_i, [_vp, _vp, _vp, _vp, _vp, _vp, C.c_int64, _i, C.c_float]),
     "gd_nn_add_layernorm_forward": (_i, [_vp, _vp, _vp, _vp, _vp, _f, _vp, _vp, C.c_int64, _i]),
+    "gd_nn_add_layernorm_forward_bcast": (_i, [_vp, _vp, _vp, _vp, _vp, _f, _vp, _vp, C.c_int64, _i, C.c_int64]),
+    "gd_nn_join_stat_rows": (C.c_size_t, [_i, _i, _i]),
+    "gd_nn_add_gn_partials": (_i, [_vp, _vp, _vp, _vp, _vp, _i, _i, _i, _i]),
+    "gd_nn_concat_gn_partials": (_i, [_vp, _vp, _vp, _vp, _vp, _i, _i, _i, _i, _i]),
     "gd_nn_attention_ws_bytes": (C.c_size_t, [_i, _i, _i]),
     "gd_nn_attention_d64_forward": (_i, [_vp, _vp, _vp, _vp, _vp, _vp, _i, _i, _i, _i, C.c_int64, _i, C.c_int64, _i,
                                          C.c_int64, _i, C.c_int64, _i, _f, _i]),
@@ -220,18 +224,19 @@
 
 class _GroupNormSiLU(torch.autograd.Function):
     @staticmethod
-    def forward(ctx, x, weight, bias, groups, eps, silu):
+    def forward(ctx, x, weight, bias, groups, eps, silu, mean_rstd=None):
         N, Cc, H, W = x.shape
         L = lib()
         y = torch.empty_like(x, memory_format=torch.channels_last)
-        ws = _gn_workspace(x, N, groups)
-        mr = torch.empty(N * groups * 2, dtype=torch.float32, device=x.device)
+        ws = _gn_workspace(x, N, groups) if mean_rstd is None else None
+        mr = torch.empty(N * groups * 2, dtype=torch.float32, device=x.device) if mean_rstd is None else mean_rstd
         w, b = weight.contiguous(), bias.contiguous()
         with torch.cuda.device(x.device):
             stream = torch.cuda.current_stream(x.device).cuda_stream
             _check(L.gd_nn_groupnorm_silu_forward(stream, x.data_ptr(), y.data_ptr(), w.data_ptr(), b.data_ptr(), N,
-                                                  H * W, Cc, groups, float(eps), int(silu), ws.data_ptr(),
-                                                  mr.data_ptr()), "gd_nn_groupnorm_silu_forward")
+                                                  H * W, Cc, groups, float(eps), int(silu),
+                                                  None if ws is None else ws.data_ptr(), mr.data_ptr()),
+                   "gd_nn_groupnorm_silu_forward")
         ctx.save_for_backward(x, w, b, mr)
         ctx.groups, ctx.silu = groups, silu
         return y
@@ -253,7 +258,7 @@
                                                    mr.data_ptr(), dx.data_ptr(), N, H * W, Cc, ctx.groups,
                                                    int(ctx.silu), ws.data_ptr(), sums.data_ptr(), None),
                    "gd_nn_groupnorm_silu_backward")
-        return dx, None, None, None, None, None
+        return dx, None, None, None, None, None, None
 
 
 _GN_FUSED_SMALL = os.environ.get("GD_NN_GN_SMALL", "1") != "0"
@@ -314,7 +319,14 @@
         return dx, None, None, None, None, None
 
 
-def group_norm_silu(x, weight, bias, groups: int, eps: float, silu: bool = True):
+def gn_stats_of(x, groups: int, eps: float):
+    tag = getattr(x, "_gd_gn_stats", None)
+    if tag is not None and tag[1:] == (groups, eps, x._version):
+        return tag[0]
+    return None
+
+
+def group_norm_silu(x, weight, bias, groups: int, eps: float, silu: bool = True, mean_rstd=None):
     if x.is_cuda:
         if weight.requires_grad or bias.requires_grad:
             raise RuntimeError("group_norm_silu HIP kernel computes input gradients only (frozen weights)")
@@ -327,10 +339,81 @@
                     return _GroupNormSiLUSmall.apply(x, weight, bias, groups, eps, silu)
             elif small and _GN_FUSED_SMALL:
                 return _gn_fused_small(x, weight, bias, groups, eps, silu)
-            return _GroupNormSiLU.apply(x, weight, bias, groups, eps, silu)
+            if mean_rstd is not None and (mean_rstd.dtype != torch.float32 or mean_rstd.numel() != x.shape[0] * groups * 2
+                                          or not mean_rstd.is_contiguous() or mean_rstd.device != x.device):
+                raise ValueError("group_norm_silu: mean_rstd must be contiguous fp32 [N * groups * 2] on x's device")
+            return _GroupNormSiLU.apply(x, weight, bias, groups, eps, silu, mean_rstd)
         _note_fallback("group_norm_silu", x, "needs a 4-D tensor with C % 8 == 0")
     y = F.group_norm(x, groups, weight, bias, eps)
     return F.silu(y) if silu else y
+
+
+
+_JOINS = os.environ.get("GD_NN_JOINS", "1") != "0"
+_JOIN_STATS = os.environ.get("GD_NN_JOIN_STATS", "0") == "1"
+
+
+def join_supported(a, b) -> bool:
+    return (_JOINS and not torch.is_grad_enabled() and _is_nhwc_bf16(a) and _is_nhwc_bf16(b) and a.device == b.device
+            and a.shape[2:] == b.shape[2:] and a.shape[1] % 8 == 0 and b.shape[1] % 8 == 0 and 0 < b.shape[0] <= a.shape[0]
+            and a.shape[0] % b.shape[0] == 0 and a.shape[0] <= 65535 and a.data_ptr() % 16 == 0 and b.data_ptr() % 16 == 0)
+
+
+def _join_wants_stats(N, HW, Cc, next_norm) -> bool:
+    if next_norm is None or not _JOIN_STATS or not _EPILOGUE_STATS or next_norm.num_channels != Cc:
+        return False
+    G = next_norm.num_groups
+    if Cc % G or (Cc // G) % 4:
+        return False
+    return not (_GN_FUSED_SMALL and lib().gd_nn_groupnorm_silu_fused_supported(N, HW, Cc, G))
+
+
+def _join(a, b, concat: bool, next_norm, stats=None):
+    N, C0, H, W = a.shape
+    C1 = b.shape[1]
+    Cc = C0 + C1 if concat else C0
+    L = lib()
+    out = torch.empty((N, Cc, H, W), dtype=torch.bfloat16, device=a.device, memory_format=torch.channels_last)
+    if stats is None:
+        stats = _join_wants_stats(N, H * W, Cc, next_norm)
+    elif stats:
+        G = next_norm.num_groups if next_norm is not None else 0
+        stats = G > 0 and next_norm.num_channels == Cc and Cc % G == 0 and (Cc // G) % 4 == 0
+    rows = L.gd_nn_join_stat_rows(N, H * W, Cc) if stats else 0
+    part = torch.empty(N * (Cc // 4) * rows * 2, dtype=torch.float32, device=a.device) if rows else None
+    with torch.cuda.device(a.device):
+        stream = torch.cuda.current_stream(a.device).cuda_stream
+        part_p = None if part is None else part.data_ptr()
+        if concat:
+            ret = L.gd_nn_concat_gn_partials(stream, a.data_ptr(), b.data_ptr(), out.data_ptr(), part_p, N, b.shape[0], H * W,
+                                             C0, C1)
+        else:
+            ret = L.gd_nn_add_gn_partials(stream, a.data_ptr(), b.data_ptr(), out.data_ptr(), part_p, N, b.shape[0], H * W, C0)
+        _check(ret, "gd_nn_concat_gn_partials" if concat else "gd_nn_add_gn_partials", "gd_nn_elementwise_last_error")
+        if part is not None:
+            G, eps = next_norm.num_groups, next_norm.eps
+            mr = torch.empty(N * G * 2, dtype=torch.float32, device=a.device)
+            _check(L.gd_nn_groupnorm_finish_partials(stream, part.data_ptr(), N, rows, Cc, G, H * W, float(eps), mr.data_ptr()),
+                   "gd_nn_groupnorm_finish_partials")
+            out._gd_gn_stats = (mr, G, eps, out._version)
+    return out
+
+
+def _shared_images(b, n: int):
+    return b if b.shape[0] == n else b.repeat(n // b.shape[0], *([1] * (b.dim() - 1)))
+
+
+def add_join(a, b, next_norm=None):
+    if join_supported(a, b) and a.shape[1] == b.shape[1] and \
+            (b.shape[0] != a.shape[0] or _join_wants_stats(a.shape[0], a.shape[2] * a.shape[3], a.shape[1], next_norm)):
+        return _join(a, b, False, next_norm)
+    return a + _shared_images(b, a.shape[0])
+
+
+def concat_join(a, b, next_norm=None):
+    if join_supported(a, b) and a.shape[1] + b.shape[1] <= 2560:
+        return _join(a, b, True, next_norm)
+    return torch.cat([a, _shared_images(b, a.shape[0])], dim=1)
 
 
 
@@ -381,6 +464,24 @@
     def __enter__(self):
         global _ROUTE_BATCH
         self.prev, _ROUTE_BATCH = _ROUTE_BATCH, self.value
+        return self
+
+    def __exit__(self, *exc):
+        global _ROUTE_BATCH
+        _ROUTE_BATCH = self.prev
+        return False
+
+
+class route_batch_shared:
+
+    def __init__(self, reps: int):
+        self.reps = int(reps)
+
+    def __enter__(self):
+        global _ROUTE_BATCH
+        self.prev = _ROUTE_BATCH
+        if self.prev is not None and self.reps > 1 and self.prev[0] % self.reps == 0 and self.prev[1] % self.reps == 0:
+            _ROUTE_BATCH = (self.prev[0] // self.reps, self.prev[1] // self.reps)
         return self
 
     def __exit__(self, *exc):
@@ -1232,14 +1333,19 @@
     x = x.contiguous()
     if residual is not None:
         residual = residual.contiguous()
-    s = torch.empty_like(x) if (residual is not None and want_sum) else None
-    y = torch.empty_like(x)
+    like = x if residual is None else residual
+    s = torch.empty_like(like) if (residual is not None and want_sum) else None
+    y = torch.empty_like(like)
     L = lib()
     with torch.cuda.device(x.device):
-        ret = L.gd_nn_add_layernorm_forward(
-            torch.cuda.current_stream(x.device).cuda_stream, x.data_ptr(),
-            None if residual is None else residual.data_ptr(), weight.data_ptr(), bias.data_ptr(),
-            float(eps), None if s is None else s.data_ptr(), y.data_ptr(), x.numel() // Cc, Cc)
+        stream = torch.cuda.current_stream(x.device).cuda_stream
+        res_p, s_p = None if residual is None else residual.data_ptr(), None if s is None else s.data_ptr()
+        if like.numel() == x.numel():
+            ret = L.gd_nn_add_layernorm_forward(stream, x.data_ptr(), res_p, weight.data_ptr(), bias.data_ptr(), float(eps), s_p,
+                                                y.data_ptr(), x.numel() // Cc, Cc)
+        else:
+            ret = L.gd_nn_add_layernorm_forward_bcast(stream, x.data_ptr(), res_p, weight.data_ptr(), bias.data_ptr(), float(eps),
+                                                      s_p, y.data_ptr(), like.numel() // Cc, Cc, x.numel() // Cc)
     if ret < 0:
         raise RuntimeError(f"gd_nn_add_layernorm_forward failed ({ret}): {L.gd_nn_elementwise_last_error().decode()}")
     return (x if residual is None else s), y
@@ -1273,8 +1379,11 @@
     Cc = x.shape[-1]
     ok = Cc % 8 == 0 and Cc <= 2048 and norm.weight.dtype == torch.bfloat16 and x.is_cuda and x.dtype == torch.bfloat16 and \
         (residual is None or (residual.is_cuda and residual.dtype == torch.bfloat16))
-    if ok and _rowwise_ok(x, residual, norm.weight, norm.bias):
+    shared = residual is not None and x.shape[0] != residual.shape[0]
+    if ok and _rowwise_ok(x, residual, norm.weight, norm.bias) and (not shared or want_sum):
         return _add_ln_fwd(x, residual, norm.weight, norm.bias, norm.eps, want_sum)
+    if shared:
+        x = _shared_images(x, residual.shape[0])
     if ok and _ROW_TRAIN and torch.is_grad_enabled() and not norm.weight.requires_grad and not norm.bias.requires_grad:
         if residual is None:
             return x, _AddLayerNormTrain.apply(x, None, norm.weight, norm.bias, float(norm.eps))
@@ -1388,18 +1497,21 @@
 
 
 def attention_d64_vt_strided(q, k, vt, kv_len: int):
-    B, S, H, _ = q.shape
-    Skv = vt.shape[2]
-    assert vt.shape[:2] == (B, H * 64) and vt.stride(2) == 1 and vt.stride(1) == Skv and vt.dtype == torch.bfloat16 and Skv % 64 == 0
+    Bq, S, H, _ = q.shape
+    B, Skv = vt.shape[0], vt.shape[2]
+    assert vt.shape[1] == H * 64 and vt.stride(2) == 1 and vt.stride(1) == Skv and vt.dtype == torch.bfloat16 and Skv % 64 == 0
+    assert k.shape[0] == B and B % Bq == 0
     L = lib()
     o = torch.empty((B, S, H * 64), dtype=torch.bfloat16, device=q.device)
     with torch.cuda.device(q.device):
-        ret = L.gd_nn_attention_d64_forward_vt_strided(torch.cuda.current_stream(q.device).cuda_stream, q.data_ptr(), k.data_ptr(),
-                                                       vt.data_ptr(), o.data_ptr(), B, S, Skv, H, q.stride(0), q.stride(1),
-                                                       k.stride(0), k.stride(1), vt.stride(0), o.stride(0), o.stride(1),
-                                                       64 ** -0.5, int(kv_len))
-    if ret < 0:
-        raise RuntimeError(f"gd_nn_attention_d64_forward_vt_strided failed ({ret}): {L.gd_nn_attention_last_error().decode()}")
+        stream = torch.cuda.current_stream(q.device).cuda_stream
+        for r in range(0, B, Bq):
+            ret = L.gd_nn_attention_d64_forward_vt_strided(stream, q.data_ptr(), k[r:r + Bq].data_ptr(), vt[r:r + Bq].data_ptr(),
+                                                           o[r:r + Bq].data_ptr(), Bq, S, Skv, H, q.stride(0), q.stride(1),
+                                                           k.stride(0), k.stride(1), vt.stride(0), o.stride(0), o.stride(1),
+                                                           64 ** -0.5, int(kv_len))
+            if ret < 0:
+                raise RuntimeError(f"gd_nn_attention_d64_forward_vt_strided failed ({ret}): {L.gd_nn_attention_last_error().decode()}")
     return o
 
 
diff --git a/include/gd_nn.h b/include/gd_nn.h
--- a/include/gd_nn.h
+++ b/include/gd_nn.h
@@ -131,6 +131,15 @@
 
 int gd_nn_add_layernorm_forward(void* stream, const void* x, const void* residual, const void* weight, const void* bias,
                                 float eps, void* sum_out, void* y, int64_t rows, int C);
+int gd_nn_add_layernorm_forward_bcast(void* stream, const void* x, const void* residual, const void* weight,
+                                      const void* bias, float eps, void* sum_out, void* y, int64_t rows, int C,
+                                      int64_t x_rows);
+
+size_t gd_nn_join_stat_rows(int N, int HW, int C);
+int gd_nn_add_gn_partials(void* stream, const void* a, const void* b, void* out, float* stat_part, int N, int Nb, int HW,
+                          int C);
+int gd_nn_concat_gn_partials(void* stream, const void* a, const void* b, void* out, float* stat_part, int N, int Nb, int HW,
+                             int C0, int C1);
 
 size_t gd_nn_attention_ws_bytes(int B, int Skv, int H);
 int gd_nn_attention_d64_forward(void* stream, const void* q, const void* k, const void* v, void* o, void* vt_ws, int B, int S,
```
